# arielmission-space/PAOS

Measured on AMD Instinct MI355X. Metric: wavefronts/sec (4096^2 c128, 20-surface chain) + achieved HBM GB/s, higher is better.
Workload: dtype c128 (f64); 1 GPU; SYN20 20-surface chain (SURVEY 8d: 43 2-D FFTs per wavefront as the reference runs it), 4096x4096 fp64, walked 512-wavelength sweep, 32 wavefronts/GPU/step, PSFs stay in HBM; separable pass programs + ptp identities ([24] passes/wavefront, parity 1e-15..2e-14 vs oracle); grid=4096, batch_per_gpu=32, parallelism=wavefront-sharded x1, transport=none (single process), ranks_seen=1, launcher=none

## Files before the change

include/paos_hip.h:

```cpp
#ifndef PAOS_HIP_H
#define PAOS_HIP_H

#ifdef __cplusplus
extern "C" {
#endif

typedef struct paos_ctx paos_ctx;

enum { PAOS_OK = 0, PAOS_EINVAL = 1, PAOS_EHIP = 2, PAOS_EUNSUPPORTED = 3 };
enum { PAOS_F64 = 0, PAOS_F32 = 1 };
enum { PAOS_SHAPE_ELLIPSE = 0, PAOS_SHAPE_RECT = 1 };
enum { PAOS_KERNEL_PASS_ROWS = 0, PAOS_KERNEL_PASS_COLS = 1, PAOS_KERNEL_PASS_ANY = 2 };
enum { PAOS_PW_SIGN = 1, PAOS_PW_QPHASE_CENTRED = 2, PAOS_PW_QPHASE_NATURAL = 3, PAOS_PW_SCALE = 4,
       PAOS_PW_MASK = 5 };
enum { PAOS_PWF_MUL2PI = 1,
       PAOS_PWF_X_ONLY = 2, PAOS_PWF_Y_ONLY = 4 };
enum { PAOS_MAX_PW = 6 };
enum { PAOS_NORM_SLOTS = 64 };
enum { PAOS_WHAT_FIELD = 0, PAOS_WHAT_AMPLITUDE = 1, PAOS_WHAT_PHASE = 2, PAOS_WHAT_INTENSITY = 3 };

enum { PAOS_PHASE_STRIDE = 5 };
enum { PAOS_APERTURE_STRIDE = 8 };
enum { PAOS_ZERNIKE_HEAD = 8 };

// ... 16 lines not shown
int paos_ctx_create(int device, int n, int batch, int precision, paos_ctx** out);
int paos_ctx_destroy(paos_ctx* ctx);
const char* paos_last_error(const paos_ctx* ctx);
int paos_sync(paos_ctx* ctx);
const char* paos_build_info(void);
const char* paos_source_hash(void);
void* paos_stream(paos_ctx* ctx);

int paos_profile_begin(paos_ctx* ctx, int kernel_kind, int max_launches);
int paos_profile_end(paos_ctx* ctx, int* launches, double* total_ms);
int paos_profile_end_split(paos_ctx* ctx, int* launches, double* total_ms, int* pruned_launches, double* pruned_ms);
int paos_profile_end_launches(paos_ctx* ctx, int capacity, double* ms_out, int* tag_out, int* count);
int paos_profile_planned_bytes(paos_ctx* ctx, int capacity, double* bytes_out, int* count);
int paos_profile_line_transforms(paos_ctx* ctx, int capacity, double* lines_out, int* count);

int paos_fill(paos_ctx* ctx, double re, double im);
int paos_start(paos_ctx* ctx, double re, double im, int shape, const double* aperture, const double* stop);
int paos_start_rows(paos_ctx* ctx, double re, double im, int shape, const double* aperture, const double* stop,
                    const double* write_rows);
int paos_zero_outside_rows(paos_ctx* ctx, const double* live_rows);
int paos_start_box(paos_ctx* ctx, double re, double im, int shape, const double* aperture, const double* stop,
                   const double* write_rows, const double* write_cols);
int paos_start_zernike_box(paos_ctx* ctx, double re, double im, int shape, const double* aperture, const double* stop,
                           const double* write_rows, const double* write_cols, int nmax, int kdim, const double* table,
                           const double* params, int param_stride, int* power_ticket);
int paos_zero_outside_box(paos_ctx* ctx, const double* live_rows, const double* live_cols);
int paos_import(paos_ctx* ctx, int item, const void* host_c128);
int paos_export(paos_ctx* ctx, int item, int what, void* host_out);

int paos_psf_keep(paos_ctx* ctx);
int paos_psf_keep_power(paos_ctx* ctx, int* ticket);
int paos_psf_fetch(paos_ctx* ctx, int item, double* host_out);
int paos_host_alloc(unsigned long long bytes, void** out);
int paos_host_free(void* p);
int paos_export_pinned(paos_ctx* ctx, int item, int what, void* pinned_out);

int paos_aperture(paos_ctx* ctx, int shape, const double* params);
int paos_aperture_render(paos_ctx* ctx, int shape, const double* params1, double* host_mask);
int paos_make_stop(paos_ctx* ctx, const double* enable);
int paos_stop_scale_last_power(paos_ctx* ctx, const double* enable);
int paos_stop_defer_last_power(paos_ctx* ctx, const double* enable);
int paos_norm2(paos_ctx* ctx, double* host_out);
int paos_norm2_enqueue(paos_ctx* ctx, int* ticket);
int paos_norm2_enqueue_rows(paos_ctx* ctx, const double* live_rows, int* ticket);
int paos_norm2_enqueue_rows_like(paos_ctx* ctx, const double* live_rows, const double* same_as, int* ticket);
int paos_norm2_enqueue_box(paos_ctx* ctx, const double* live_rows, const double* live_cols, const double* same_as, int* ticket);
int paos_norm2_fetch(paos_ctx* ctx, int ticket, double* host_out);
int paos_norm2_release(paos_ctx* ctx, int ticket);
int paos_psf_metrics(paos_ctx* ctx, int nr, const double* radii_px, double cx_px, double cy_px,
                     double* host_out);
int paos_phase(paos_ctx* ctx, const double* params, int mul2pi);
int paos_phase_map(paos_ctx* ctx, int item, const double* host_wfe, double wl);
int paos_phase_map_items(paos_ctx* ctx, const double* host_wfe, unsigned long long key, int n_items, const double* items,
                         const double* wl);
int paos_psd_screen(paos_ctx* ctx, const double* host_noise, const double* host_rough, const double* params,
                    unsigned long long key, double* host_out);
int paos_ptp(paos_ctx* ctx, const double* params);
int paos_stw(paos_ctx* ctx, const double* params, int inverse);
int paos_wts(paos_ctx* ctx, const double* params, int inverse);
int paos_focus_begin(paos_ctx* ctx);
int paos_focus_plane(paos_ctx* ctx, const double* params);
int paos_focus_end(paos_ctx* ctx);
enum { PAOS_OTF_MTF = 0, PAOS_OTF_COMPLEX = 1 };
int paos_otf_compute(paos_ctx* ctx);
int paos_otf_fetch(paos_ctx* ctx, int item, int what, void* host_out);
int paos_otf_cuts(paos_ctx* ctx, double* host_out);
int paos_blur_table(int n, double d, double sigma, double pixel, double* t);
enum { PAOS_BLUR_ITEM = 6 };
int paos_blur_apply(paos_ctx* ctx, const double* per_item);
enum { PAOS_EE_GIVEN = 0, PAOS_EE_CENTROID = 1, PAOS_EE_PEAK = 2 };
enum { PAOS_EE_ITEM = 4 };
enum { PAOS_EE_SUMMARY = 9 };
int paos_ee_compute(paos_ctx* ctx, int bins, int square, int centre_mode, const double* per_item);
int paos_ee_fetch(paos_ctx* ctx, double* summary, double* curves);
int paos_zoom_weights(int n, int s, double frac, double* w, int* carry);
enum { PAOS_ZOOM_PSF = 0, PAOS_ZOOM_FIELD = 1 };
int paos_zoom_compute(paos_ctx* ctx, int m, int s, const double* centres, int want_field);
int paos_zoom_tiles(int n, int batch, int m, int* pt_y, int* pt_x);
int paos_zoom_fetch(paos_ctx* ctx, int item, int what, void* host_out);
int paos_run_passes(paos_ctx* ctx, const paos_pass* passes, int n_passes, const double* blocks,
                    int n_blocks);
int paos_copy_yardstick(paos_ctx* ctx, int reps, double* ms_per_launch, double* bytes_per_launch);
int paos_record_set_stats(paos_ctx* ctx, unsigned long long* found, unsigned long long* rendered);
int paos_central_half_stats(paos_ctx* ctx, unsigned long long* central, unsigned long long* plain);
int paos_narrow_window_stats(paos_ctx* ctx, unsigned long long* narrow, unsigned long long* other);
int paos_record_block_stats(paos_ctx* ctx, unsigned long long* out);
int paos_frugal_built(int precision, int n, const int* record);
int paos_pass_builds(paos_ctx* ctx, int* records, int capacity, int* count);
int paos_deferred_stop_stats(paos_ctx* ctx, unsigned long long* rode, unsigned long long* settled);
int paos_ctx_set_pruning(paos_ctx* ctx, int on);
int paos_run_passes_live(paos_ctx* ctx, const paos_pass* passes, int n_passes, const double* blocks,
                         int n_blocks, const double* live_rows);
int paos_run_program(paos_ctx* ctx, const paos_pass* passes, int n_passes, const double* blocks, int n_blocks,
                     const paos_program_opts* opts);
int paos_zernike(paos_ctx* ctx, int nmax, int kdim, const double* table, const double* params,
                 int param_stride, double* host_wfe);
int paos_zernike_like(paos_ctx* ctx, int nmax, int kdim, const double* table, const double* params,
                      int param_stride, const double* same_as, double* host_wfe);


int paos_pupil_aperture(paos_ctx* ctx, int shape, const double* params);
int paos_pupil_upload(paos_ctx* ctx, int item, const double* host_weights);
int paos_zernike_gram(paos_ctx* ctx, int nmax, int kdim, const double* table, const double* params,
                      int param_stride, int K, const double* poly, int use_pupil, double* host_out);
int paos_zernike_pupil(paos_ctx* ctx, int nmax, int kdim, const double* table, const double* params,
                       int param_stride, double* host_wfe);

enum { PAOS_WF_UNIFORM = 0, PAOS_WF_INTENSITY = 1 };
enum { PAOS_WF_SUMMARY = 10 };
int paos_wavefront_fit(paos_ctx* ctx, int nmax, int kdim, const double* table, const double* params, int param_stride,
                       int K, const double* poly, int weight_mode, int use_pupil, const double* min_intensity);
int paos_wavefront_fetch(paos_ctx* ctx, double* summary, double* sums);

enum { PAOS_DETECTOR_GEOM = 6 };
enum { PAOS_DETECTOR_ITEM = 3 };
enum { PAOS_DETECTOR_SCRATCH_MIB = 512 };
int paos_detector_begin(paos_ctx* ctx, const double* geom);
int paos_detector_add(paos_ctx* ctx, const double* per_item);
int paos_detector_images(paos_ctx* ctx, const double* per_item, double* host_out);
int paos_detector_fetch(paos_ctx* ctx, double* host_out);
enum { PAOS_DETECTOR_PLACED_ITEM = 5 };
int paos_detector_add_placed(paos_ctx* ctx, const double* per_item);
int paos_detector_images_placed(paos_ctx* ctx, const double* per_item, double* host_out);

#ifdef __cplusplus
}
#endif
#endif
```

paos_amd/_lib.py:

```python
import ctypes
import os
import threading
import weakref

import numpy as np

_HERE = os.path.dirname(os.path.abspath(__file__))
LIB_PATH = os.environ.get("PAOS_LIB") or os.path.join(_HERE, "libpaoship.so")

PAOS_F64, PAOS_F32 = 0, 1
SHAPE_ELLIPSE, SHAPE_RECT = 0, 1
WHAT_FIELD, WHAT_AMPLITUDE, WHAT_PHASE, WHAT_INTENSITY = 0, 1, 2, 3
KERNEL_PASS_ROWS, KERNEL_PASS_COLS, KERNEL_PASS_ANY = 0, 1, 2
PW_SIGN, PW_QPHASE_CENTRED, PW_QPHASE_NATURAL, PW_SCALE, PW_MASK = 1, 2, 3, 4, 5
PWF_MUL2PI = 1
PWF_X_ONLY, PWF_Y_ONLY = 2, 4
MAX_PW = 6
OTF_MTF, OTF_COMPLEX = 0, 1
EE_GIVEN, EE_CENTROID, EE_PEAK = 0, 1, 2
EE_ITEM, EE_SUMMARY, EE_MAX_BINS = 4, 9, 1024
WF_UNIFORM, WF_INTENSITY = 0, 1
WF_SUMMARY, WF_MAX_TERMS = 10, 63
ZOOM_PSF, ZOOM_FIELD = 0, 1
ZOOM_MAX_TABLES = 256
NORM_SLOTS = 64


class PwOp(ctypes.Structure):
    _fields_ = [("kind", ctypes.c_int), ("flags", ctypes.c_int), ("block", ctypes.c_int)]


class ProgramOpts(ctypes.Structure):
    _fields_ = [("live_rows", ctypes.POINTER(ctypes.c_double)), ("rows_stale", ctypes.c_int),
                ("final_intensity", ctypes.c_int), ("power_ticket", ctypes.POINTER(ctypes.c_int)),
                ("live_cols", ctypes.POINTER(ctypes.c_double))]


class Pass(ctypes.Structure):
    _fields_ = [("axis", ctypes.c_int), ("fft1", ctypes.c_int), ("fft2", ctypes.c_int),
                ("n_pre", ctypes.c_int), ("n_mid", ctypes.c_int), ("n_post", ctypes.c_int),
                ("pre", PwOp * MAX_PW), ("mid", PwOp * MAX_PW), ("post", PwOp * MAX_PW)]

PHASE_STRIDE = 5
APERTURE_STRIDE = 8
ZERNIKE_HEAD = 8

_c_ctx = ctypes.c_void_p
_dbl_p = ctypes.POINTER(ctypes.c_double)
SYMBOLS = {
    "paos_ctx_create": (ctypes.c_int, [ctypes.c_int, ctypes.c_int, ctypes.c_int, ctypes.c_int, ctypes.POINTER(_c_ctx)]),
    "paos_ctx_destroy": (ctypes.c_int, [_c_ctx]),
    "paos_last_error": (ctypes.c_char_p, [_c_ctx]),
    "paos_sync": (ctypes.c_int, [_c_ctx]),
    "paos_build_info": (ctypes.c_char_p, []),
    "paos_stream": (ctypes.c_void_p, [_c_ctx]),
    "paos_profile_begin": (ctypes.c_int, [_c_ctx, ctypes.c_int, ctypes.c_int]),
    "paos_profile_end": (ctypes.c_int, [_c_ctx, ctypes.POINTER(ctypes.c_int), _dbl_p]),
    "paos_profile_end_split": (ctypes.c_int, [_c_ctx, ctypes.POINTER(ctypes.c_int), _dbl_p, ctypes.POINTER(ctypes.c_int), _dbl_p]),
    "paos_source_hash": (ctypes.c_char_p, []),
    "paos_profile_planned_bytes": (ctypes.c_int, [_c_ctx, ctypes.c_int, _dbl_p, ctypes.POINTER(ctypes.c_int)]),
    "paos_profile_line_transforms": (ctypes.c_int, [_c_ctx, ctypes.c_int, _dbl_p, ctypes.POINTER(ctypes.c_int)]),
    "paos_profile_end_launches": (ctypes.c_int, [_c_ctx, ctypes.c_int, _dbl_p, ctypes.POINTER(ctypes.c_int),
                                                 ctypes.POINTER(ctypes.c_int)]),
    "paos_fill": (ctypes.c_int, [_c_ctx, ctypes.c_double, ctypes.c_double]),
    "paos_import": (ctypes.c_int, [_c_ctx, ctypes.c_int, ctypes.c_void_p]),
    "paos_export": (ctypes.c_int, [_c_ctx, ctypes.c_int, ctypes.c_int, ctypes.c_void_p]),
    "paos_aperture": (ctypes.c_int, [_c_ctx, ctypes.c_int, _dbl_p]),
    "paos_aperture_render": (ctypes.c_int, [_c_ctx, ctypes.c_int, _dbl_p, _dbl_p]),
    "paos_make_stop": (ctypes.c_int, [_c_ctx, _dbl_p]),
    "paos_stop_scale_last_power": (ctypes.c_int, [_c_ctx, _dbl_p]),
    "paos_stop_defer_last_power": (ctypes.c_int, [_c_ctx, _dbl_p]),
    "paos_norm2": (ctypes.c_int, [_c_ctx, _dbl_p]),
    "paos_norm2_enqueue": (ctypes.c_int, [_c_ctx, ctypes.POINTER(ctypes.c_int)]),
    "paos_norm2_fetch": (ctypes.c_int, [_c_ctx, ctypes.c_int, _dbl_p]),
    "paos_norm2_release": (ctypes.c_int, [_c_ctx, ctypes.c_int]),
    "paos_psf_metrics": (ctypes.c_int, [_c_ctx, ctypes.c_int, _dbl_p, ctypes.c_double, ctypes.c_double, _dbl_p]),
    "paos_phase": (ctypes.c_int, [_c_ctx, _dbl_p, ctypes.c_int]),
    "paos_phase_map": (ctypes.c_int, [_c_ctx, ctypes.c_int, _dbl_p, ctypes.c_double]),
    "paos_ptp": (ctypes.c_int, [_c_ctx, _dbl_p]),
    "paos_stw": (ctypes.c_int, [_c_ctx, _dbl_p, ctypes.c_int]),
    "paos_wts": (ctypes.c_int, [_c_ctx, _dbl_p, ctypes.c_int]),
    "paos_focus_begin": (ctypes.c_int, [_c_ctx]),
    "paos_focus_plane": (ctypes.c_int, [_c_ctx, _dbl_p]),
    "paos_focus_end": (ctypes.c_int, [_c_ctx]),
    "paos_otf_compute": (ctypes.c_int, [_c_ctx]),
    "paos_otf_fetch": (ctypes.c_int, [_c_ctx, ctypes.c_int, ctypes.c_int, ctypes.c_void_p]),
    "paos_otf_cuts": (ctypes.c_int, [_c_ctx, _dbl_p]),
    "paos_blur_table": (ctypes.c_int, [ctypes.c_int, ctypes.c_double, ctypes.c_double, ctypes.c_double, _dbl_p]),
    "paos_blur_apply": (ctypes.c_int, [_c_ctx, _dbl_p]),
    "paos_ee_compute": (ctypes.c_int, [_c_ctx, ctypes.c_int, ctypes.c_int, ctypes.c_int, _dbl_p]),
    "paos_ee_fetch": (ctypes.c_int, [_c_ctx, _dbl_p, _dbl_p]),
    "paos_wavefront_fit": (ctypes.c_int, [_c_ctx, ctypes.c_int, ctypes.c_int, _dbl_p, _dbl_p, ctypes.c_int, ctypes.c_int, _dbl_p,
                                          ctypes.c_int, ctypes.c_int, _dbl_p]),
    "paos_wavefront_fetch": (ctypes.c_int, [_c_ctx, _dbl_p, _dbl_p]),
    "paos_zoom_weights": (ctypes.c_int, [ctypes.c_int, ctypes.c_int, ctypes.c_double, _dbl_p, ctypes.POINTER(ctypes.c_int)]),
    "paos_zoom_compute": (ctypes.c_int, [_c_ctx, ctypes.c_int, ctypes.c_int, _dbl_p, ctypes.c_int]),
    "paos_zoom_fetch": (ctypes.c_int, [_c_ctx, ctypes.c_int, ctypes.c_int, ctypes.c_void_p]),
    "paos_zoom_tiles": (ctypes.c_int, [ctypes.c_int, ctypes.c_int, ctypes.c_int, ctypes.POINTER(ctypes.c_int),
                                       ctypes.POINTER(ctypes.c_int)]),
    "paos_run_passes": (ctypes.c_int, [_c_ctx, ctypes.POINTER(Pass), ctypes.c_int, _dbl_p, ctypes.c_int]),
    "paos_copy_yardstick": (ctypes.c_int, [_c_ctx, ctypes.c_int, _dbl_p, _dbl_p]),
    "paos_record_set_stats": (ctypes.c_int, [_c_ctx, ctypes.POINTER(ctypes.c_ulonglong), ctypes.POINTER(ctypes.c_ulonglong)]),
    "paos_central_half_stats": (ctypes.c_int, [_c_ctx, ctypes.POINTER(ctypes.c_ulonglong), ctypes.POINTER(ctypes.c_ulonglong)]),
    "paos_narrow_window_stats": (ctypes.c_int, [_c_ctx, ctypes.POINTER(ctypes.c_ulonglong), ctypes.POINTER(ctypes.c_ulonglong)]),
    "paos_record_block_stats": (ctypes.c_int, [_c_ctx, ctypes.POINTER(ctypes.c_ulonglong)]),
    "paos_frugal_built": (ctypes.c_int, [ctypes.c_int, ctypes.c_int, ctypes.POINTER(ctypes.c_int)]),
    "paos_pass_builds": (ctypes.c_int, [_c_ctx, ctypes.POINTER(ctypes.c_int), ctypes.c_int, ctypes.POINTER(ctypes.c_int)]),
    "paos_deferred_stop_stats": (ctypes.c_int, [_c_ctx, ctypes.POINTER(ctypes.c_ulonglong), ctypes.POINTER(ctypes.c_ulonglong)]),
    "paos_ctx_set_pruning": (ctypes.c_int, [_c_ctx, ctypes.c_int]),
    "paos_run_passes_live": (ctypes.c_int, [_c_ctx, ctypes.POINTER(Pass), ctypes.c_int, _dbl_p, ctypes.c_int, _dbl_p]),
    "paos_zernike": (ctypes.c_int, [_c_ctx, ctypes.c_int, ctypes.c_int, _dbl_p, _dbl_p, ctypes.c_int, _dbl_p]),
    "paos_psf_keep": (ctypes.c_int, [_c_ctx]),
    "paos_psf_keep_power": (ctypes.c_int, [_c_ctx, ctypes.POINTER(ctypes.c_int)]),
    "paos_psf_fetch": (ctypes.c_int, [_c_ctx, ctypes.c_int, _dbl_p]),
    "paos_host_alloc": (ctypes.c_int, [ctypes.c_ulonglong, ctypes.POINTER(ctypes.c_void_p)]),
    "paos_host_free": (ctypes.c_int, [ctypes.c_void_p]),
    "paos_export_pinned": (ctypes.c_int, [_c_ctx, ctypes.c_int, ctypes.c_int, ctypes.c_void_p]),
    "paos_start": (ctypes.c_int, [_c_ctx, ctypes.c_double, ctypes.c_double, ctypes.c_int, _dbl_p, _dbl_p]),
    "paos_pupil_aperture": (ctypes.c_int, [_c_ctx, ctypes.c_int, _dbl_p]),
    "paos_pupil_upload": (ctypes.c_int, [_c_ctx, ctypes.c_int, _dbl_p]),
    "paos_zernike_like": (ctypes.c_int, [_c_ctx, ctypes.c_int, ctypes.c_int, _dbl_p, _dbl_p, ctypes.c_int, _dbl_p, _dbl_p]),
    "paos_zernike_gram": (ctypes.c_int, [_c_ctx, ctypes.c_int, ctypes.c_int, _dbl_p, _dbl_p, ctypes.c_int,
                                         ctypes.c_int, _dbl_p, ctypes.c_int, _dbl_p]),
    "paos_zernike_pupil": (ctypes.c_int, [_c_ctx, ctypes.c_int, ctypes.c_int, _dbl_p, _dbl_p, ctypes.c_int, _dbl_p]),
    "paos_start_rows": (ctypes.c_int, [_c_ctx, ctypes.c_double, ctypes.c_double, ctypes.c_int, _dbl_p, _dbl_p, _dbl_p]),
    "paos_zero_outside_rows": (ctypes.c_int, [_c_ctx, _dbl_p]),
    "paos_phase_map_items": (ctypes.c_int, [_c_ctx, _dbl_p, ctypes.c_ulonglong, ctypes.c_int, _dbl_p, _dbl_p]),
    "paos_psd_screen": (ctypes.c_int, [_c_ctx, _dbl_p, _dbl_p, _dbl_p, ctypes.c_ulonglong, _dbl_p]),
    "paos_start_box": (ctypes.c_int, [_c_ctx, ctypes.c_double, ctypes.c_double, ctypes.c_int, _dbl_p, _dbl_p, _dbl_p, _dbl_p]),
    "paos_start_zernike_box": (ctypes.c_int, [_c_ctx, ctypes.c_double, ctypes.c_double, ctypes.c_int, _dbl_p, _dbl_p, _dbl_p, _dbl_p,
                                              ctypes.c_int, ctypes.c_int, _dbl_p, _dbl_p, ctypes.c_int, ctypes.POINTER(ctypes.c_int)]),
    "paos_zero_outside_box": (ctypes.c_int, [_c_ctx, _dbl_p, _dbl_p]),
    "paos_norm2_enqueue_box": (ctypes.c_int, [_c_ctx, _dbl_p, _dbl_p, _dbl_p, ctypes.POINTER(ctypes.c_int)]),
    "paos_norm2_enqueue_rows": (ctypes.c_int, [_c_ctx, _dbl_p, ctypes.POINTER(ctypes.c_int)]),
    "paos_norm2_enqueue_rows_like": (ctypes.c_int, [_c_ctx, _dbl_p, _dbl_p, ctypes.POINTER(ctypes.c_int)]),
    "paos_run_program": (ctypes.c_int, [_c_ctx, ctypes.POINTER(Pass), ctypes.c_int, _dbl_p, ctypes.c_int,
                                        ctypes.POINTER(ProgramOpts)]),
    "paos_detector_begin": (ctypes.c_int, [_c_ctx, _dbl_p]),
    "paos_detector_add": (ctypes.c_int, [_c_ctx, _dbl_p]),
    "paos_detector_images": (ctypes.c_int, [_c_ctx, _dbl_p, _dbl_p]),
    "paos_detector_fetch": (ctypes.c_int, [_c_ctx, _dbl_p]),
    "paos_detector_add_placed": (ctypes.c_int, [_c_ctx, _dbl_p]),
    "paos_detector_images_placed": (ctypes.c_int, [_c_ctx, _dbl_p, _dbl_p]),
}

_lib = None


class PaosHipError(RuntimeError):
    pass


def load():
    global _lib
    if _lib is not None:
        return _lib
    if not os.path.exists(LIB_PATH):
        raise PaosHipError(
            f"{LIB_PATH} not found: build it with `make` or "
            "`python -c 'import __graft_entry__ as g; g.build()'` (there is no CPU fallback)"
        )
    lib = ctypes.CDLL(LIB_PATH)
    if os.environ.get("PAOS_LIB"):
        import sys

        print(f"paos_amd: using the library variant {LIB_PATH} (PAOS_LIB)", file=sys.stderr)
    for name, (res, args) in SYMBOLS.items():
        fn = getattr(lib, name)
        fn.restype = res
        fn.argtypes = args
    _lib = lib
    return lib


def _dptr(arr):
    return arr.ctypes.data_as(_dbl_p)


def as_blocks(blocks, batch, stride):
    arr = np.ascontiguousarray(blocks, dtype=np.float64)
    if arr.shape != (batch, stride):
        raise ValueError(f"expected parameter blocks of shape {(batch, stride)}, got {arr.shape}")
    return arr


BUILD_FIELDS = ("axis", "kpre", "kmid", "nfft", "store", "tab", "fuse", "one_line", "central")


def frugal_built(precision, n, record):
    if len(record) != len(BUILD_FIELDS):
        raise ValueError("a build record has nine fields")
    rec = (ctypes.c_int * 9)(*[int(v) for v in record])
    code = {"fp64": PAOS_F64, "fp32": PAOS_F32}.get(precision, -1)
    rc = load().paos_frugal_built(code, int(n), rec)
    if rc < 0:
        raise ValueError(f"no family of pass-kernel builds for {precision} at n = {n}")
    return bool(rc)


def zoom_check(size, oversample, n):
    if isinstance(size, bool) or not isinstance(size, (int, np.integer)) or size < 16 or size > 1024 or size % 16:
        raise ValueError(f"a zoomed window's size must be an integer multiple of 16 in 16 .. 1024, got {size!r}")
    if isinstance(oversample, bool) or not isinstance(oversample, (int, np.integer)) or not 1 <= oversample <= 64:
        raise ValueError(f"a zoomed window's oversampling must be an integer in 1 .. 64, got {oversample!r}")
    if size > oversample * n:
        raise ValueError(f"a zoomed window of {size} samples at oversampling {oversample} is wider than the {n}-pixel grid")


def zoom_tiles(n, batch, size):
    pty, ptx = ctypes.c_int(0), ctypes.c_int(0)
    if load().paos_zoom_tiles(int(n), int(batch), int(size), ctypes.byref(pty), ctypes.byref(ptx)) != 0:
        raise ValueError(f"paos_zoom_tiles refused n={n!r}, batch={batch!r}, size={size!r}")
    return pty.value, ptx.value


def blur_table(n, d, sigma, pixel=0.0):
    if isinstance(n, bool) or not isinstance(n, (int, np.integer)) or n < 2:
        raise ValueError(f"paos_blur_table refused n={n!r}")
    out = np.empty(int(n) // 2 + 1, dtype=np.float64)
    if load().paos_blur_table(int(n), float(d), float(sigma), float(pixel), _dptr(out)) != 0:
# ... 425 lines not shown
    def energy_compute(self, bins, deltas, aspects, centre_mode, centres=None, square=False):
        per_item = np.empty((self.batch, EE_ITEM), dtype=np.float64)
        try:
            per_item[:, 0] = np.broadcast_to(np.asarray(deltas, dtype=np.float64), (self.batch,))
            per_item[:, 1] = np.broadcast_to(np.asarray(aspects, dtype=np.float64), (self.batch,))
            per_item[:, 2:] = self.n / 2 if centres is None else np.asarray(centres, dtype=np.float64)
        except ValueError:
            raise ValueError(f"energy_compute takes scalars or one value per item ({self.batch}) and (batch, 2) centres") from None
        self._check(self._lib.paos_ee_compute(self._ctx, int(bins), int(bool(square)), int(centre_mode), _dptr(per_item)),
                    "paos_ee_compute")
        self._ee_shape = (self.batch, 2 if square else 1, int(bins))

    def energy_fetch(self, curves=True):
        shape = getattr(self, "_ee_shape", None)
        if shape is None:
            raise PaosHipError("paos_ee_fetch failed (1): no energy profiles computed (paos_ee_compute)")
        summary = np.empty((self.batch, EE_SUMMARY), dtype=np.float64)
        out = np.empty(shape, dtype=np.float64) if curves else None
        self._check(self._lib.paos_ee_fetch(self._ctx, _dptr(summary), _dptr(out) if curves else None), "paos_ee_fetch")
        return summary, out

    def wavefront_fit(self, nmax, kdim, table, blocks, poly, weight=WF_UNIFORM, min_intensity=None, pupil=False):
        t = np.ascontiguousarray(table, dtype=np.float64).reshape(-1)
        b = np.ascontiguousarray(blocks, dtype=np.float64)
        q = np.ascontiguousarray(poly, dtype=np.float64)
        if b.ndim != 2 or b.shape[0] != self.batch:
            raise ValueError("zernike blocks must be [batch][stride]")
        if q.ndim != 2 or q.shape[1] != 4:
            raise ValueError("poly must be [K][4]")
        floors = None
        if min_intensity is not None:
            try:
                floors = np.ascontiguousarray(np.broadcast_to(np.asarray(min_intensity, dtype=np.float64), (self.batch,)))
            except ValueError:
                raise ValueError(f"wavefront_fit takes a scalar floor or one per item ({self.batch})") from None
        self._check(self._lib.paos_wavefront_fit(self._ctx, int(nmax), int(kdim), _dptr(t), _dptr(b), int(b.shape[1]), int(q.shape[0]),
                                                 _dptr(q), int(weight), 1 if pupil else 0,
                                                 _dptr(floors) if floors is not None else None), "paos_wavefront_fit")
        self._wf_terms = int(q.shape[0])

    def wavefront_fetch(self):
        k = getattr(self, "_wf_terms", None)
        if k is None:
            raise PaosHipError("paos_wavefront_fetch failed (1): no wavefront fit computed (paos_wavefront_fit)")
        summary = np.empty((self.batch, WF_SUMMARY), dtype=np.float64)
        sums = np.empty((self.batch, (k + 1) * (k + 2) // 2), dtype=np.float64)
        self._check(self._lib.paos_wavefront_fetch(self._ctx, _dptr(summary), _dptr(sums)), "paos_wavefront_fetch")
        return summary, sums

    def zoom_compute(self, size, oversample, centres=None, field=False):
        ctr = None if centres is None else zoom_centres(centres, self.batch, self.n)
        zoom_check(size, oversample, self.n)
        self._check(self._lib.paos_zoom_compute(self._ctx, int(size), int(oversample), _dptr(ctr) if ctr is not None else None,
                                                1 if field else 0), "paos_zoom_compute")
        self._zoom_size = int(size)

    def zoom_fetch(self, item=0, what="psf"):
        if what not in ("psf", "field"):
            raise ValueError(f"what must be 'psf' or 'field', got {what!r}")
        m = getattr(self, "_zoom_size", 1)
        out = np.empty((m, m), dtype=np.float64 if what == "psf" else np.complex128)
        self._check(self._lib.paos_zoom_fetch(self._ctx, int(item), ZOOM_PSF if what == "psf" else ZOOM_FIELD,
                                              out.ctypes.data_as(ctypes.c_void_p)), "paos_zoom_fetch")
        return out

    def copy_yardstick(self, reps=10):
        ms, nbytes = ctypes.c_double(0.0), ctypes.c_double(0.0)
        self._check(self._lib.paos_copy_yardstick(self._ctx, int(reps), ctypes.byref(ms), ctypes.byref(nbytes)),
                    "paos_copy_yardstick")
        return ms.value, nbytes.value

    def record_set_stats(self):
        found, rendered = ctypes.c_ulonglong(0), ctypes.c_ulonglong(0)
        self._check(self._lib.paos_record_set_stats(self._ctx, ctypes.byref(found), ctypes.byref(rendered)),
                    "paos_record_set_stats")
        return int(found.value), int(rendered.value)

    def central_half_stats(self):
        central, plain = ctypes.c_ulonglong(0), ctypes.c_ulonglong(0)
        self._check(self._lib.paos_central_half_stats(self._ctx, ctypes.byref(central), ctypes.byref(plain)),
                    "paos_central_half_stats")
        return int(central.value), int(plain.value)

    def record_block_stats(self):
        out = (ctypes.c_ulonglong * 3)()
        self._check(self._lib.paos_record_block_stats(self._ctx, out), "paos_record_block_stats")
        return int(out[0]), int(out[1]), int(out[2])

    def pass_builds(self, capacity=64):
        count = ctypes.c_int(0)
        buf = (ctypes.c_int * (9 * capacity))()
        self._check(self._lib.paos_pass_builds(self._ctx, buf, capacity, ctypes.byref(count)), "paos_pass_builds")
        if count.value > capacity:
            return self.pass_builds(count.value)
        return [tuple(buf[9 * i:9 * i + 9]) for i in range(count.value)]

    def deferred_stop_stats(self):
        rode, settled = ctypes.c_ulonglong(0), ctypes.c_ulonglong(0)
        self._check(self._lib.paos_deferred_stop_stats(self._ctx, ctypes.byref(rode), ctypes.byref(settled)),
                    "paos_deferred_stop_stats")
        return int(rode.value), int(settled.value)

    def set_pruning(self, on):
        self._check(self._lib.paos_ctx_set_pruning(self._ctx, 1 if on else 0), "paos_ctx_set_pruning")

    def run_passes(self, passes, blocks, live_rows=None, rows_stale=False, final_intensity=False, live_cols=None):
        b = np.ascontiguousarray(blocks, dtype=np.float64)
        if b.ndim != 3 or b.shape[1:] != (self.batch, PHASE_STRIDE):
            raise ValueError("blocks must be [n_blocks][batch][5]")
        arr = (Pass * len(passes))()
        for dst, src in zip(arr, passes):
            dst.axis, dst.fft1, dst.fft2 = src["axis"], src.get("fft1", -1), src.get("fft2", -1)
            for name in ("pre", "mid", "post"):
                ops = src.get(name, ())
                if len(ops) > MAX_PW:
                    raise ValueError("too many operators in one pass slot")
                setattr(dst, "n_" + name, len(ops))
                lst = getattr(dst, name)
                for i, (kind, flags, block) in enumerate(ops):
                    lst[i].kind, lst[i].flags, lst[i].block = kind, flags, block
        if rows_stale or final_intensity:
            lr = self._rows(live_rows) if live_rows is not None else None
            lc = self._rows(live_cols) if (live_cols is not None and rows_stale and lr is not None) else None
            ticket = ctypes.c_int(-1)
            opts = ProgramOpts(_dptr(lr) if lr is not None else None, 1 if (rows_stale and lr is not None) else 0,
                               int(final_intensity), ctypes.pointer(ticket), _dptr(lc) if lc is not None else None)
            self._check(self._lib.paos_run_program(self._ctx, arr, len(passes), _dptr(b), b.shape[0], ctypes.byref(opts)),
                        "paos_run_program")
            return ticket.value if final_intensity else None
        if live_rows is not None:
            lr = self._rows(live_rows)
            self._check(self._lib.paos_run_passes_live(self._ctx, arr, len(passes), _dptr(b), b.shape[0], _dptr(lr)),
                        "paos_run_passes_live")
            return None
        self._check(self._lib.paos_run_passes(self._ctx, arr, len(passes), _dptr(b), b.shape[0]),
                    "paos_run_passes")
        return None

    def zernike(self, nmax, kdim, table, blocks, want_wfe=False, pupil=False, same_as=None):
        t = np.ascontiguousarray(table, dtype=np.float64).reshape(-1)
        b = np.ascontiguousarray(blocks, dtype=np.float64)
        if b.ndim != 2 or b.shape[0] != self.batch:
            raise ValueError("zernike blocks must be [batch][stride]")
        out = np.empty((self.n, self.n), dtype=np.float64) if want_wfe else None
        if same_as is not None and not pupil:
            like = np.ascontiguousarray(same_as, dtype=np.float64).reshape(-1)
            if like.size != self.batch:
                raise ValueError("same_as must name an item per item")
            self._check(self._lib.paos_zernike_like(self._ctx, int(nmax), int(kdim), _dptr(t), _dptr(b), int(b.shape[1]),
                                                    _dptr(like), _dptr(out) if want_wfe else None), "paos_zernike_like")
            return out
        fn = self._lib.paos_zernike_pupil if pupil else self._lib.paos_zernike
        self._check(fn(self._ctx, int(nmax), int(kdim), _dptr(t), _dptr(b), int(b.shape[1]),
                       _dptr(out) if want_wfe else None),
                    "paos_zernike_pupil" if pupil else "paos_zernike")
        return out

    def start(self, value, shape, blocks, stop=None, write_rows=None, write_cols=None):
        b = np.ascontiguousarray(blocks, dtype=np.float64)
        if b.shape != (self.batch, APERTURE_STRIDE):
            raise ValueError("aperture blocks must be [batch][8]")
        st = None if stop is None else np.ascontiguousarray(stop, dtype=np.float64)
        if st is not None and st.shape != (self.batch,):
            raise ValueError("stop flags must be [batch]")
        v = complex(value)
        if write_rows is not None and write_cols is not None:
            self._check(self._lib.paos_start_box(self._ctx, v.real, v.imag, int(shape), _dptr(b),
                                                 _dptr(st) if st is not None else None, _dptr(self._rows(write_rows)),
                                                 _dptr(self._rows(write_cols))), "paos_start_box")
            return
        if write_rows is not None:
            self._check(self._lib.paos_start_rows(self._ctx, v.real, v.imag, int(shape), _dptr(b),
                                                  _dptr(st) if st is not None else None, _dptr(self._rows(write_rows))),
                        "paos_start_rows")
            return
        self._check(self._lib.paos_start(self._ctx, v.real, v.imag, int(shape), _dptr(b),
                                         _dptr(st) if st is not None else None), "paos_start")

    def start_zernike(self, value, shape, blocks, stop, write_rows, write_cols, nmax, kdim, table, zblocks, power=False):
        b = np.ascontiguousarray(blocks, dtype=np.float64)
        if b.shape != (self.batch, APERTURE_STRIDE):
            raise ValueError("aperture blocks must be [batch][8]")
        st = None if stop is None else np.ascontiguousarray(stop, dtype=np.float64)
        if st is not None and st.shape != (self.batch,):
            raise ValueError("stop flags must be [batch]")
        t = np.ascontiguousarray(table, dtype=np.float64).reshape(-1)
        zb = np.ascontiguousarray(zblocks, dtype=np.float64)
        if zb.ndim != 2 or zb.shape[0] != self.batch:
            raise ValueError("zernike blocks must be [batch][stride]")
        v = complex(value)
        ticket = ctypes.c_int(-1)
        self._check(self._lib.paos_start_zernike_box(self._ctx, v.real, v.imag, int(shape), _dptr(b),
                                                     _dptr(st) if st is not None else None, _dptr(self._rows(write_rows)),
                                                     _dptr(self._rows(write_cols)), int(nmax), int(kdim), _dptr(t), _dptr(zb),
                                                     int(zb.shape[1]), ctypes.byref(ticket) if power else None),
                    "paos_start_zernike_box")
        return ticket.value if power else None

    def pupil_aperture(self, shape, blocks):
        b = np.ascontiguousarray(blocks, dtype=np.float64)
        if b.shape != (self.batch, APERTURE_STRIDE):
            raise ValueError("aperture blocks must be [batch][8]")
        self._check(self._lib.paos_pupil_aperture(self._ctx, int(shape), _dptr(b)), "paos_pupil_aperture")

    def pupil_upload(self, item, weights):
        w = np.ascontiguousarray(weights, dtype=np.float64)
        if w.shape != (self.n, self.n):
            raise ValueError("pupil weights must be [n][n]")
        self._check(self._lib.paos_pupil_upload(self._ctx, int(item), _dptr(w)), "paos_pupil_upload")

    def zernike_gram(self, nmax, kdim, table, blocks, poly, pupil=True):
        t = np.ascontiguousarray(table, dtype=np.float64).reshape(-1)
        b = np.ascontiguousarray(blocks, dtype=np.float64)
        q = np.ascontiguousarray(poly, dtype=np.float64)
        if b.ndim != 2 or b.shape[0] != self.batch:
            raise ValueError("zernike blocks must be [batch][stride]")
        if q.ndim != 2 or q.shape[1] != 4:
            raise ValueError("poly must be [K][4]")
        k = q.shape[0]
        out = np.empty((self.batch, k * (k + 1) // 2 + 1), dtype=np.float64)
        self._check(self._lib.paos_zernike_gram(self._ctx, int(nmax), int(kdim), _dptr(t), _dptr(b),
                                                int(b.shape[1]), int(k), _dptr(q), 1 if pupil else 0, _dptr(out)),
                    "paos_zernike_gram")
        return out[:, :-1], out[:, -1]
```

paos_amd/csrc/arena_layout.h:

```cpp
#pragma once
#include <cstddef>

#pragma GCC visibility push(hidden)

constexpr size_t kArenaAlign = 16;
inline size_t arena_rounded(size_t count) { return (count + kArenaAlign - 1) & ~(kArenaAlign - 1); }
constexpr size_t kArenaSlack = 64;

enum ArenaRoom {
  ARENA_FITS,
  ARENA_SWITCH,
  ARENA_GROW
};

struct ArenaLayout {
  size_t cap = 0;
  size_t head = 0;
  size_t sent = 0;

  ArenaRoom room(size_t total) const {
    total += kArenaSlack;
    if (total > cap) return ARENA_GROW;
    return head + total > cap ? ARENA_SWITCH : ARENA_FITS;
  }
  size_t grown(size_t total) const {
    size_t c = cap ? cap : kArenaAlign;
    while (c < total + kArenaSlack) c *= 2;
    return c;
  }
  bool fits(size_t count) const { return count <= cap && head + count <= cap; }
  size_t place(size_t count) {
    const size_t at = head;
    head += arena_rounded(count);
    return at;
  }
  bool pending() const { return sent < head; }
  bool take(size_t* first, size_t* count) {
    if (!pending()) return false;
    *first = sent;
    *count = head - sent;
    sent = head;
    return true;
  }
  void drop() { sent = head; }
  void rewind() { head = sent = 0; }
};

struct ArenaBatchState {
  bool reserved = false, closed = false;
  bool may_add() const { return !closed; }
  bool may_switch() const { return !reserved; }
};

#pragma GCC visibility pop
```

paos_amd/csrc/context.hip:

```cpp
#include "host.h"

#include <cmath>
#include <complex>
#include <cstdio>
#include <cstring>
#include <mutex>
#include <set>
#include <utility>

namespace {

thread_local std::string g_err;

}

int fail(paos_ctx* c, int code, const std::string& msg) {
  if (c) c->err = msg;
  g_err = msg;
  return code;
}

namespace {

bool dump_arena() {
// ... 198 lines not shown
  return out;
}

namespace {

template <typename T>
std::vector<std::complex<T>> twiddles(int n) {
  std::vector<std::complex<T>> tw(n);
  const long double two_pi = 6.283185307179586476925286766559005768L;
  for (int m = 0; m < n; ++m) {
    const long double a = two_pi * (long double)m / (long double)n;
    tw[m] = std::complex<T>((T)cosl(a), (T)-sinl(a));
  }
  return tw;
}


int profile_end(paos_ctx* c, int* launches, double* total_ms, int* pruned_launches, double* pruned_ms) {
  if (c) (void)hipSetDevice(c->device);
  if (!c || !launches || !total_ms) return fail(c, PAOS_EINVAL, "null argument");
  HIPCHK(c, hipStreamSynchronize(c->stream));
  double sum = 0.0, psum = 0.0;
  int pcount = 0;
  for (size_t i = 0; i + 1 < c->prof_used; i += 2) {
    float ms = 0.f;
    HIPCHK(c, hipEventElapsedTime(&ms, c->prof_events[i], c->prof_events[i + 1]));
    sum += ms;
    if (i / 2 < c->prof_tags.size() && c->prof_tags[i / 2]) { psum += ms; ++pcount; }
  }
  *launches = (int)(c->prof_used / 2);
  *total_ms = sum;
  if (pruned_launches) *pruned_launches = pcount;
  if (pruned_ms) *pruned_ms = psum;
  c->prof_kind = -1;
  c->prof_used = 0;
  return PAOS_OK;
}

}

extern "C" {

const char* paos_last_error(const paos_ctx* ctx) { return ctx ? ctx->err.c_str() : g_err.c_str(); }

const char* paos_build_info(void) {
  static const std::string info = std::string("libpaoship gfx950 layout=") + std::to_string(BR) + "(c64 at N>=2048: " + std::to_string(PAOS_F32_BR) + ")x(" +
                                  std::to_string(Lay<double>::BC) + "|" + std::to_string(Lay<float>::BC) +
                                  ") pad_blocks=" + std::to_string(PAOS_PAD_BLOCKS);
  return info.c_str();
}

void* paos_stream(paos_ctx* ctx) { return ctx ? (void*)ctx->stream : nullptr; }

int paos_ctx_create(int device, int n, int batch, int precision, paos_ctx** out) {
  if (!out) return fail(nullptr, PAOS_EINVAL, "out is null");
  *out = nullptr;
  if (n < 64 || n > 4096 || (n & (n - 1))) return fail(nullptr, PAOS_EUNSUPPORTED, "grid size must be a power of two in 64..4096");
  if (batch < 1) return fail(nullptr, PAOS_EINVAL, "batch must be >= 1");
  if (precision != PAOS_F64 && precision != PAOS_F32) return fail(nullptr, PAOS_EINVAL, "precision must be PAOS_F64 or PAOS_F32");
  int ndev = 0;
  if (hipGetDeviceCount(&ndev) != hipSuccess || ndev == 0)
    return fail(nullptr, PAOS_EHIP, "no HIP device available: libpaoship has no CPU fallback");
  if (device < 0 || device >= ndev) return fail(nullptr, PAOS_EINVAL, "device index out of range");
  paos_ctx* c = new paos_ctx();
  c->device = device; c->n = n; c->batch = batch; c->precision = precision;
  const int bc = precision == PAOS_F64 ? Lay<double>::BC : Lay<float>::BC;
  c->br = (precision == PAOS_F32 && n >= 2048) ? PAOS_F32_BR : PAOS_BR;
  c->pitch = (unsigned)n * c->br + (unsigned)PAOS_PAD_BLOCKS * c->br * bc;
  c->item_stride = c->pitch * (unsigned)(n / c->br);
  const size_t eb = elem_bytes(c);
  auto bail = [&](hipError_t e, const char* what) {
    std::string msg = std::string(what) + ": " + hipGetErrorString(e);
    paos_ctx_destroy(c);
    return fail(nullptr, PAOS_EHIP, msg);
  };
  hipError_t e;
  if ((e = hipSetDevice(device)) != hipSuccess) return bail(e, "hipSetDevice");
  if ((e = hipStreamCreateWithFlags(&c->stream, hipStreamNonBlocking)) != hipSuccess) return bail(e, "hipStreamCreate");
  if (const char* pad = getenv("PAOS_LDS_PAD")) c->lds_pad = (size_t)std::max(0, std::atoi(pad));
  if (env_is("PAOS_CENTRAL_HALF", '0')) c->central_half = false;
  if (env_is("PAOS_CENTRAL_HALF", '1')) c->central_half = true;
  if (env_is("PAOS_NARROW_WINDOWS", '0')) c->narrow_windows = false;
  if (env_is("PAOS_NARROW_WINDOWS", '1')) c->narrow_windows = true;
  if ((e = hipMalloc(&c->dyn_scale, (size_t)batch * sizeof(double))) != hipSuccess) return bail(e, "hipMalloc(dyn_scale)");
  {
    std::vector<double> ones((size_t)batch, 1.0);
    if ((e = hipMemcpy(c->dyn_scale, ones.data(), ones.size() * sizeof(double), hipMemcpyHostToDevice)) != hipSuccess) return bail(e, "hipMemcpy(dyn_scale)");
  }
  if ((e = hipMalloc(&c->field, (size_t)c->item_stride * batch * eb)) != hipSuccess) return bail(e, "hipMalloc(field)");
  if ((e = hipMemsetAsync(c->field, 0, (size_t)c->item_stride * batch * eb, c->stream)) != hipSuccess) return bail(e, "hipMemset(field)");
  if ((e = hipMalloc(&c->tw, (size_t)n * eb)) != hipSuccess) return bail(e, "hipMalloc(tw)");
  if ((e = hipMalloc(&c->staging, (size_t)n * n * 16)) != hipSuccess) return bail(e, "hipMalloc(staging)");
  c->nparts = 1024;
  if ((e = hipMalloc(&c->partial, (size_t)batch * c->nparts * sizeof(double))) != hipSuccess) return bail(e, "hipMalloc(partial)");
  if ((e = hipMalloc(&c->norm2, (size_t)batch * sizeof(double))) != hipSuccess) return bail(e, "hipMalloc(norm2)");
  if ((e = hipHostMalloc(&c->norm2_host, (size_t)kNormSlots * batch * sizeof(double))) != hipSuccess) return bail(e, "hipHostMalloc(norm2)");
  c->arena.lay.cap = (size_t)1 << 18;
  if (c->arena.lay.cap < (size_t)batch * 2048) c->arena.lay.cap = (size_t)batch * 2048;
  if (const char* cap = getenv("PAOS_ARENA_DOUBLES")) c->arena.lay.cap = arena_rounded((size_t)std::max(1LL, std::atoll(cap)));
  if ((e = hipHostMalloc(&c->arena.host, kArenaSlabs * c->arena.lay.cap * sizeof(double))) != hipSuccess) return bail(e, "hipHostMalloc(arena)");
  if ((e = hipMalloc(&c->arena.dev, kArenaSlabs * c->arena.lay.cap * sizeof(double))) != hipSuccess) return bail(e, "hipMalloc(arena)");
  for (int k = 0; k < kArenaSlabs; ++k)
    if ((e = hipEventCreateWithFlags(&c->arena.fence[k], hipEventDisableTiming)) != hipSuccess) return bail(e, "hipEventCreate(arena fence)");
  c->arena.used[0] = true;
  e = dispatch_layout(c, [&](auto t, auto) {
    auto tw = twiddles<decltype(t)>(n);
    return hipMemcpy(c->tw, tw.data(), (size_t)n * eb, hipMemcpyHostToDevice);
  });
  if (e != hipSuccess) return bail(e, "hipMemcpy(tw)");
  *out = c;
  return PAOS_OK;
}

int paos_profile_begin(paos_ctx* c, int kernel_kind, int max_launches) {
  if (c) (void)hipSetDevice(c->device);
  if (!c || max_launches < 0) return fail(c, PAOS_EINVAL, "bad profile request");
  HIPCHK(c, hipStreamSynchronize(c->stream));
  while (c->prof_events.size() < (size_t)2 * max_launches) {
    hipEvent_t e;
    HIPCHK(c, hipEventCreate(&e));
    c->prof_events.push_back(e);
  }
  c->prof_kind = kernel_kind;
  c->prof_used = 0;
  c->prof_tags.clear();
  c->prof_bytes.clear();
  c->prof_lines.clear();
  return PAOS_OK;
}

int paos_profile_end_launches(paos_ctx* c, int capacity, double* ms_out, int* tag_out, int* count) {
  if (c) (void)hipSetDevice(c->device);
  if (!c || !ms_out || !tag_out || !count || capacity < 0) return fail(c, PAOS_EINVAL, "null argument");
  HIPCHK(c, hipStreamSynchronize(c->stream));
  const int n = (int)(c->prof_used / 2);
  if (n > capacity) return fail(c, PAOS_EINVAL, "more launches were timed than the caller's arrays hold");
  for (int i = 0; i < n; ++i) {
    float ms = 0.f;
    HIPCHK(c, hipEventElapsedTime(&ms, c->prof_events[2 * i], c->prof_events[2 * i + 1]));
    ms_out[i] = ms;
    tag_out[i] = (size_t)i < c->prof_tags.size() ? c->prof_tags[i] : 0;
  }
  *count = n;
  c->prof_kind = -1;
  c->prof_used = 0;
  return PAOS_OK;
}

int paos_profile_planned_bytes(paos_ctx* c, int capacity, double* bytes_out, int* count) {
  if (!c || !bytes_out || !count || capacity < 0) return fail(c, PAOS_EINVAL, "null argument");
  const int n = (int)(c->prof_used / 2);
  if (n > capacity) return fail(c, PAOS_EINVAL, "more launches were timed than the caller's array holds");
  for (int i = 0; i < n; ++i) bytes_out[i] = (size_t)i < c->prof_bytes.size() ? c->prof_bytes[i] : 0.0;
  *count = n;
  return PAOS_OK;
}

int paos_profile_line_transforms(paos_ctx* c, int capacity, double* lines_out, int* count) {
  if (!c || !lines_out || !count || capacity < 0) return fail(c, PAOS_EINVAL, "bad profile request");
  const int n = (int)(c->prof_used / 2);
  if (n > capacity) return fail(c, PAOS_EINVAL, "profile buffer too small");
  for (int i = 0; i < n; ++i) lines_out[i] = (size_t)i < c->prof_lines.size() ? c->prof_lines[i] : 0.0;
  *count = n;
  return PAOS_OK;
}

int paos_profile_end(paos_ctx* c, int* launches, double* total_ms) {
  return profile_end(c, launches, total_ms, nullptr, nullptr);
}

int paos_profile_end_split(paos_ctx* c, int* launches, double* total_ms, int* pruned_launches, double* pruned_ms) {
  if (!pruned_launches || !pruned_ms) return fail(c, PAOS_EINVAL, "null argument");
  return profile_end(c, launches, total_ms, pruned_launches, pruned_ms);
}

int paos_ctx_destroy(paos_ctx* c) {
  if (!c) return PAOS_OK;
  (void)hipSetDevice(c->device);
  if (c->stream) (void)hipStreamSynchronize(c->stream);
  for (hipEvent_t e : c->prof_events) (void)hipEventDestroy(e);
  if (c->field) (void)hipFree(c->field);
  if (c->tw) (void)hipFree(c->tw);
  if (c->staging) (void)hipFree(c->staging);
  if (c->tables) (void)hipFree(c->tables);
  if (c->mask) (void)hipFree(c->mask);
  if (c->metric_partial) (void)hipFree(c->metric_partial);
  if (c->metric_out) (void)hipFree(c->metric_out);
  if (c->metric_host) (void)hipHostFree(c->metric_host);
  for (auto& ms : c->mask_sets) {
    if (ms.lines) (void)hipFree(ms.lines);
    if (ms.vals) (void)hipFree(ms.vals);
  }
  if (c->mask_overflow) (void)hipFree(c->mask_overflow);
  if (c->block_stats) (void)hipFree(c->block_stats);
  if (c->partial) (void)hipFree(c->partial);
  if (c->norm2) (void)hipFree(c->norm2);
  if (c->norm2_host) (void)hipHostFree(c->norm2_host);
  if (c->psf) (void)hipFree(c->psf);
  if (c->focus_spec) (void)hipFree(c->focus_spec);
  if (c->otf_spec) (void)hipFree(c->otf_spec);
  if (c->otf_cuts) (void)hipFree(c->otf_cuts);
  if (c->zoom_t) (void)hipFree(c->zoom_t);
  if (c->zoom_psf) (void)hipFree(c->zoom_psf);
  if (c->zoom_field) (void)hipFree(c->zoom_field);
  if (c->zoom_tabs) (void)hipFree(c->zoom_tabs);
  if (c->map_dev) (void)hipFree(c->map_dev);
  if (c->psd_scratch) (void)hipFree(c->psd_scratch);
  if (c->start_norm2) (void)hipFree(c->start_norm2);
  if (c->start_partial) (void)hipFree(c->start_partial);
  if (c->psd_bad) (void)hipFree(c->psd_bad);
  if (c->pow_partial) (void)hipFree(c->pow_partial);
  if (c->dyn_scale) (void)hipFree(c->dyn_scale);
  if (c->ptab) (void)hipFree(c->ptab);
  if (c->psf_partial) (void)hipFree(c->psf_partial);
  if (c->det_img) (void)hipFree(c->det_img);
  if (c->det_rows) (void)hipFree(c->det_rows);
  if (c->det_out) (void)hipFree(c->det_out);
  if (c->ee_buf) (void)hipFree(c->ee_buf);
  if (c->wf_buf) (void)hipFree(c->wf_buf);
  for (int i = 0; i < 2; ++i) {
    if (c->bounce[i]) (void)hipHostFree(c->bounce[i]);
    if (c->bounce_ev[i]) (void)hipEventDestroy(c->bounce_ev[i]);
  }
  if (c->arena.host) (void)hipHostFree(c->arena.host);
  if (c->arena.dev) (void)hipFree(c->arena.dev);
  for (int k = 0; k < kArenaSlabs; ++k)
    if (c->arena.fence[k]) (void)hipEventDestroy(c->arena.fence[k]);
  if (c->stream) (void)hipStreamDestroy(c->stream);
  delete c;
  return PAOS_OK;
}

int paos_sync(paos_ctx* c) {
  if (c) (void)hipSetDevice(c->device);
  if (!c) return fail(c, PAOS_EINVAL, "null context");
  HIPCHK(c, hipStreamSynchronize(c->stream));
  return check_mask_overflow(c);
}

int paos_host_alloc(unsigned long long bytes, void** out) {
  if (!out || bytes == 0) return fail(nullptr, PAOS_EINVAL, "null argument");
  *out = nullptr;
  const hipError_t e = hipHostMalloc(out, (size_t)bytes);
  if (e != hipSuccess) {
    *out = nullptr;
    return fail(nullptr, PAOS_EHIP, std::string("hipHostMalloc: ") + hipGetErrorString(e));
  }
  return PAOS_OK;
}

int paos_host_free(void* p) {
  if (!p) return PAOS_OK;
  const hipError_t e = hipHostFree(p);
  if (e != hipSuccess) return fail(nullptr, PAOS_EHIP, std::string("hipHostFree: ") + hipGetErrorString(e));
  return PAOS_OK;
}

int paos_norm2_fetch(paos_ctx* c, int ticket, double* host_out) {
  if (c) (void)hipSetDevice(c->device);
  if (!c || !host_out || ticket < 0 || ticket >= kNormSlots) return fail(c, PAOS_EINVAL, "bad ticket");
  if (!c->norm_busy[ticket]) return fail(c, PAOS_EINVAL, "ticket is not outstanding (already fetched, or never issued)");
  HIPCHK(c, hipStreamSynchronize(c->stream));
  c->norm_busy[ticket] = false;
  std::memcpy(host_out, c->norm2_host + (size_t)ticket * c->batch, (size_t)c->batch * sizeof(double));
  return check_mask_overflow(c);
}

int paos_norm2_release(paos_ctx* c, int ticket) {
  if (!c || ticket < 0 || ticket >= kNormSlots) return fail(c, PAOS_EINVAL, "bad ticket");
  c->norm_busy[ticket] = false;
  return PAOS_OK;
}

int paos_record_set_stats(paos_ctx* c, unsigned long long* found, unsigned long long* rendered) {
  if (!c || !found || !rendered) return fail(c, PAOS_EINVAL, "bad record-set request");
  *found = c->mask_hits;
  *rendered = c->mask_rendered;
  return PAOS_OK;
}

int paos_central_half_stats(paos_ctx* c, unsigned long long* central, unsigned long long* plain) {
  if (!c || !central || !plain) return fail(c, PAOS_EINVAL, "bad central-half request");
  *central = c->central_launches;
  *plain = c->plain_launches;
  return PAOS_OK;
}

int paos_narrow_window_stats(paos_ctx* c, unsigned long long* narrow, unsigned long long* other) {
  if (!c || !narrow || !other) return fail(c, PAOS_EINVAL, "bad narrow-window request");
  *narrow = c->narrow_launches;
  *other = c->other_launches;
  return PAOS_OK;
}

int paos_record_block_stats(paos_ctx* c, unsigned long long* out) {
  if (!c || !out) return fail(c, PAOS_EINVAL, "bad record-block request");
  out[0] = out[1] = out[2] = 0ull;
  if (!c->block_stats) return PAOS_OK;
  HIPCHK(c, hipStreamSynchronize(c->stream));
  HIPCHK(c, hipMemcpy(out, c->block_stats, 3 * sizeof(unsigned long long), hipMemcpyDeviceToHost));
  return PAOS_OK;
}

int paos_deferred_stop_stats(paos_ctx* c, unsigned long long* rode, unsigned long long* settled) {
  if (!c || !rode || !settled) return fail(c, PAOS_EINVAL, "bad deferred-stop request");
  *rode = c->deferred_rode;
  *settled = c->deferred_settled;
  return PAOS_OK;
}

int paos_ctx_set_pruning(paos_ctx* c, int on) {
  if (!c) return fail(c, PAOS_EINVAL, "null context");
  c->prune = on != 0;
  return PAOS_OK;
}

}
```

paos_amd/csrc/host.h:

```cpp
#pragma once
#include "../../include/paos_hip.h"

#include <hip/hip_runtime.h>

#include <cstdlib>
#include <string>
#include <type_traits>
#include <vector>

#include "arena_layout.h"
#include "frugal_pass.h"
#include "pass_records.h"

using namespace paos;

#ifndef PAOS_BR
#define PAOS_BR 4
#endif
#ifndef PAOS_PAD_BLOCKS
#define PAOS_PAD_BLOCKS 3
#endif
inline constexpr int BR = PAOS_BR;
#ifndef PAOS_F32_BR
#define PAOS_F32_BR 8
#endif
template <typename T, int N>
constexpr int block_rows() { return (sizeof(T) == 4 && N >= 2048) ? PAOS_F32_BR : PAOS_BR; }
inline constexpr int kNormSlots = PAOS_NORM_SLOTS;
template <typename T>
struct Lay {
  static constexpr int BC = 2;
};

constexpr int kArenaSlabs = 4;
struct Arena {
  double* host = nullptr;
  double* dev = nullptr;
  ArenaLayout lay;
  int cur = 0;
  int left = -1;
  hipEvent_t fence[kArenaSlabs] = {};
  bool fenced[kArenaSlabs] = {};
  bool used[kArenaSlabs] = {};
};

struct paos_ctx {
  int device = 0, n = 0, batch = 0, precision = 0;
  int br = PAOS_BR;
  unsigned pitch = 0, item_stride = 0;
  hipStream_t stream = nullptr;
  double* psf = nullptr;
  void* focus_spec = nullptr;
  bool focus_open = false;
  void* otf_spec = nullptr;
  bool otf_computed = false, otf_valid = false;
  double* otf_cuts = nullptr;
  std::vector<double> blur_tabs, blur_key;
  cx<double>* zoom_t = nullptr;
  double* zoom_psf = nullptr;
  cx<double>* zoom_field = nullptr;
  int zoom_m = 0;
  bool zoom_done = false, zoom_has_field = false;
  double* zoom_tabs = nullptr;
  int zoom_s = 0, zoom_cap = 0;
  std::vector<double> zoom_fracs;
  std::vector<std::vector<int>> zoom_carry;
  double* map_dev = nullptr;
  unsigned long long map_key = 0;
  double map_max = 0.0;
  std::vector<double> start_key;
  double* start_norm2 = nullptr;
  std::vector<double> start_partial_key;
  double* start_partial = nullptr;
  cx<double>* psd_scratch = nullptr;
  int* psd_bad = nullptr;
  double* psf_partial = nullptr;
  int psf_nparts = 0;
  double* pow_partial = nullptr;
  int pow_nparts = 0;
  cx<double>* ptab = nullptr;
  int ptab_slots = 0;
  double* dyn_scale = nullptr;
  bool dyn_pending = false;
  unsigned long long deferred_rode = 0, deferred_settled = 0;
  bool norm2_of_field = false;
  int psf_zero_axis = -1;
  std::vector<double> psf_zero_lo, psf_zero_hi;
  bool det_set = false;
  int det_nx = 0, det_ny = 0;
  double det_geom[4] = {};
  double* det_img = nullptr;
  double* det_rows = nullptr;
  size_t det_rows_bytes = 0;
  double* det_out = nullptr;
  size_t det_out_bytes = 0;
  double* ee_buf = nullptr;
  size_t ee_bytes = 0;
  int ee_bins = 0, ee_curves = 0;
  bool ee_computed = false, ee_valid = false;
  double* wf_buf = nullptr;
  size_t wf_bytes = 0;
  int wf_pairs = 0;
  bool wf_fitted = false;
  void* bounce[2] = {nullptr, nullptr};
  hipEvent_t bounce_ev[2] = {nullptr, nullptr};
  void* field = nullptr;
  void* tw = nullptr;
  void* staging = nullptr;
  cx<double>* tables = nullptr;
  double* mask = nullptr;
  double* metric_partial = nullptr;
  double* metric_out = nullptr;
  double* metric_host = nullptr;
  struct MaskSet {
    MaskLine* lines = nullptr;
    double* vals = nullptr;
    std::vector<double> key;
    unsigned long long used = 0;
    int line_lo = 0, line_hi = 0;
  };
  static constexpr int kMaskSets = 8;
  MaskSet mask_sets[kMaskSets];
  unsigned long long mask_clock = 0;
  unsigned long long mask_hits = 0, mask_rendered = 0;
  size_t lds_pad = 0;
  bool central_half = true;
  unsigned long long central_launches = 0, plain_launches = 0;
  bool narrow_windows = true;
  unsigned long long narrow_launches = 0, other_launches = 0;
  std::vector<int> pass_builds;
  int* mask_overflow = nullptr;
  unsigned long long* block_stats = nullptr;
  double* partial = nullptr;
// ... 46 lines not shown
  static constexpr int COL_LINES = BC;
  static constexpr int ROW_THREADS = ROW_LINES * N / E, COL_THREADS = COL_LINES * N / E;
  static constexpr int ROW_TILES = (ROW_THREADS >= 128) ? 1 : 128 / ROW_THREADS;
  static constexpr int COL_TILES = (COL_THREADS >= 128) ? 1 : 128 / COL_THREADS;
  static constexpr bool ROW_SPLIT = (size_t)ROW_LINES * ROW_TILES * line_lds_bytes<T, N, false>() > 144 * 1024;
  static constexpr bool COL_SPLIT = (size_t)COL_LINES * COL_TILES * line_lds_bytes<T, N, false>() > 144 * 1024;
  static constexpr int MINW = 1;
};
inline int frugal_tile_lines(const paos_ctx* c, int axis) { return axis == 0 ? (c->n >= 2048 ? c->br / 2 : c->br) : 2; }

int arena_reserve(paos_ctx* c, size_t total);
int arena_push(paos_ctx* c, const double* src, size_t count, const double** dev);
class ArenaBatch {
 public:
  explicit ArenaBatch(paos_ctx* c) : c_(c) {}
  int begin(size_t total);
  int add(const double* src, size_t count, const double** dev);
  int commit();

 private:
  paos_ctx* c_;
  ArenaBatchState st_;
};
int arena_settled(paos_ctx* c, int rc);
int copy_to_host(paos_ctx* c, void* host, const void* dev, size_t bytes);
int next_norm_slot(paos_ctx* c);
int check_mask_overflow(paos_ctx* c);
int check_rows(paos_ctx* c, const double* rows);
std::vector<double> rounded_cols(const paos_ctx* c, const double* cols);
int opt_in_lds(paos_ctx* c, const void* kern, size_t lds);
bool timed_launch_begin(paos_ctx* c, int kind);
hipError_t timed_launch_end(paos_ctx* c, int tag);

int launch_failed(paos_ctx* c, const char* call, hipError_t e, const char* file, int line);
#define TIMED_LAUNCH(c, ...) timed_launch(__FILE__, __LINE__, (c), __VA_ARGS__)
template <typename Kern, typename... Args>
int timed_launch(const char* file, int line, paos_ctx* c, Kern kern, dim3 grid, dim3 block, size_t lds, size_t lds_opt_in, int kind,
                 int tag, Args... args) {
  if (lds_opt_in) {
    int rc = opt_in_lds(c, (const void*)kern, lds_opt_in);
    if (rc) return rc;
  }
  const bool timed = timed_launch_begin(c, kind);
  hipLaunchKernelGGL(kern, grid, block, lds, c->stream, args...);
  hipError_t e = hipGetLastError();
  if (e != hipSuccess) return launch_failed(c, "hipGetLastError()", e, file, line);
  if (timed && (e = timed_launch_end(c, tag)) != hipSuccess) return launch_failed(c, "timed_launch_end(c, tag)", e, file, line);
  return PAOS_OK;
}
inline size_t generic_lds_opt_in(size_t lds) { return lds > 48 * 1024 ? lds : 0; }

template <typename F>
int dispatch_n(paos_ctx* c, F&& f) {
  switch (c->n) {
#define PAOS_N_CASE(N) case N: return f(std::integral_constant<int, N>{})
    PAOS_N_CASE(64);
    PAOS_N_CASE(128);
    PAOS_N_CASE(256);
    PAOS_N_CASE(512);
    PAOS_N_CASE(1024);
    PAOS_N_CASE(2048);
    PAOS_N_CASE(4096);
#undef PAOS_N_CASE
  }
  return fail(c, PAOS_EUNSUPPORTED, "grid size must be a power of two in 64..4096");
}

template <typename F>
auto dispatch_block_rows(const paos_ctx* c, F&& f) {
  if (c->br == PAOS_F32_BR) return f(std::integral_constant<int, PAOS_F32_BR>{});
  return f(std::integral_constant<int, PAOS_BR>{});
}
template <typename F>
auto dispatch_layout(const paos_ctx* c, F&& f) {
  if (c->precision == PAOS_F64) return f(double{}, std::integral_constant<int, PAOS_BR>{});
  return dispatch_block_rows(c, [&](auto br) { return f(float{}, br); });
}
template <int A, int B, typename F>
auto dispatch_either(bool first, F&& f) {
  if (first) return f(std::integral_constant<int, A>{});
  return f(std::integral_constant<int, B>{});
}

int run_passes(paos_ctx* c, const paos_pass* passes, int n_passes, const double* blocks, int n_blocks,
               const double* entry_rows = nullptr, bool entry_stale = false, int* final_ticket = nullptr, int final_mode = 1,
               const double* entry_cols = nullptr);
int mask_render_mode();
bool mask_rect_blocks();

int generic_pass(paos_ctx* c, int axis, const PassArgs& a, int feat);

template <typename T, int N>
int frugal_family(paos_ctx* c, const FrugalBuild& b, const FrugalArgs& a, bool narrow);

int settle_scale(paos_ctx* c, bool field_is_overwritten = false);
int dyn_scale_reset(paos_ctx* c);
int zero_outside_rows(paos_ctx* c, const double* live_rows);
int zero_outside_box(paos_ctx* c, const double* live_rows, const double* live_cols);
int power_ring_full(paos_ctx* c);
int take_power_ticket(paos_ctx* c, const double* partial, int nparts, const double* source, int* ticket);
int psf_keep_power_impl(paos_ctx* c, int* ticket);
struct MaskRender {
  const double *params, *shared;
  int set, axis, line0, line_end, shapes;
};
constexpr int kMaskRenders = 8;
int render_mask_records(paos_ctx* c, const MaskRender* jobs, int count);
int render_mask_weights(paos_ctx* c, const double* ap);
int pointwise_pass(paos_ctx* c, const PassArgs& a);

#define SETTLE_SCALE(c) do { if (c) { (c)->norm2_of_field = false; if ((c)->dyn_pending) { int rc_ = settle_scale(c); if (rc_) return rc_; } } } while (0)
#define DROP_SCALE(c) do { if (c) { (c)->norm2_of_field = false; if ((c)->dyn_pending) { int rc_ = settle_scale(c, true); if (rc_) return rc_; } } } while (0)

#pragma GCC visibility pop
```

paos_amd/csrc/paos_hip.hip:

```cpp
#include "host.h"

#include <algorithm>
#include <cmath>
#include <cstring>

#include "item_groups.h"
#include "pointwise.h"

namespace {

int pw_blocks(const paos_ctx* c) {
  const size_t total = (size_t)c->item_stride;
  size_t b = (total + kPwThreads - 1) / kPwThreads;
  return (int)(b < 2048 ? b : 2048);
}

__global__ void dyn_scale_set_kernel(double* dyn, const double* norm2, const double* enable, int batch) {
  const int i = blockIdx.x * blockDim.x + threadIdx.x;
  if (i < batch) dyn[i] = (!enable || enable[i] != 0.0) ? 1.0 / sqrt(norm2[i]) : 1.0;
}
__global__ void dyn_scale_reset_kernel(double* dyn, int batch) {
  const int i = blockIdx.x * blockDim.x + threadIdx.x;
  if (i < batch) dyn[i] = 1.0;
}
// ... 31 lines not shown

static_assert(kMaskRenders == kMaskJobs, "a call's renderings go out in one launch per shape");
int render_mask_records(paos_ctx* c, const MaskRender* renders, int count) {
  MaskJobs jobs{};
  for (int j = 0; j < count; ++j) {
    const MaskRender& r = renders[j];
    const paos_ctx::MaskSet& ms = c->mask_sets[r.set];
    jobs.job[j] = MaskJob{r.params, r.shared, ms.lines, ms.vals, r.axis, r.line0, r.line_end, r.shapes};
  }
  jobs.batch_stride = c->batch * (int)FP_STRIDE; jobs.param_stride = (int)FP_STRIDE; jobs.n = c->n; jobs.overflow = c->mask_overflow;
  const int mode = mask_render_mode();
  jobs.windows = mode != 0 ? 1 : 0;
  jobs.pairs = mode >= 2 ? std::min(mode, 3) - 1 : 0;
  jobs.rect_blocks = mask_rect_blocks() ? 1 : 0;
  int widest = 0, shapes = 0;
  for (int j = 0; j < count; ++j) {
    widest = std::max(widest, jobs.job[j].line_end - jobs.job[j].line0);
    shapes |= jobs.job[j].shapes;
  }
  const dim3 block(256);
  const int per_wg = 4 * (jobs.pairs >= 2 ? 4 : (jobs.pairs ? 2 : 1));
  constexpr int block_per_wg = kMaskBlockLines * kMaskWaves;
  if ((shapes & 1) && mode == 4)
    hipLaunchKernelGGL(mask_blocks_kernel, dim3((widest + block_per_wg - 1) / block_per_wg, c->batch, count), block, 0, c->stream, jobs, c->block_stats);
  else if (shapes & 1)
    hipLaunchKernelGGL(mask_lines_kernel<0>, dim3((widest + per_wg - 1) / per_wg, c->batch, count), block, 0, c->stream, jobs);
  const int rect_per_wg = 4 * (jobs.rect_blocks ? 64 : 1);
  if (shapes & 2) hipLaunchKernelGGL(mask_lines_kernel<1>, dim3((widest + rect_per_wg - 1) / rect_per_wg, c->batch, count), block, 0, c->stream, jobs);
  HIPCHK(c, hipGetLastError());
  return PAOS_OK;
}

int render_mask_weights(paos_ctx* c, const double* ap) {
  if (!c->mask) HIPCHK(c, hipMalloc(&c->mask, (size_t)c->batch * c->item_stride * sizeof(double)));
  const dim3 grid(pw_blocks(c), c->batch), block(kPwThreads);
  const double* ap2 = ap + (size_t)c->batch * FP_STRIDE;
  dispatch_layout(c, [&](auto t, auto br) {
    using T = decltype(t);
    constexpr int BRV = decltype(br)::value;
    hipLaunchKernelGGL((aperture_kernel<T, BRV, Lay<T>::BC, 0>), grid, block, 0, c->stream, (cx<T>*)nullptr, ap, ap2, FP_STRIDE, c->n, c->pitch, c->item_stride, c->mask, 1);
    hipLaunchKernelGGL((aperture_kernel<T, BRV, Lay<T>::BC, 1>), grid, block, 0, c->stream, (cx<T>*)nullptr, ap, ap2, FP_STRIDE, c->n, c->pitch, c->item_stride, c->mask, 1);
  });
  HIPCHK(c, hipGetLastError());
  return PAOS_OK;
}

int pointwise_pass(paos_ctx* c, const PassArgs& a) {
  const dim3 grid(pw_blocks(c), c->batch), block(kPwThreads);
  dispatch_layout(c, [&](auto t, auto br) {
    hipLaunchKernelGGL((pointwise_kernel<decltype(t), decltype(br)::value, Lay<decltype(t)>::BC>), grid, block, 0, c->stream, a, c->n);
  });
  HIPCHK(c, hipGetLastError());
  return PAOS_OK;
}

namespace {

const char* const kPhaseMapOverflow = "the phase argument 2 pi w / wl of the map's largest value is not finite";
bool phase_map_argument_finite(double wmax, double wl) { return std::isfinite((6.283185307179586 * wmax) / wl); }

bool share_wfe_maps() {
  static const bool on = !env_is("PAOS_SHARE_WFE", '0');
  return on;
}

void norm2_partial_launch(paos_ctx* c, const double* enable, const double* rows = nullptr, const double* cols = nullptr) {
  dispatch_layout(c, [&](auto t, auto br) {
    using T = decltype(t);
    hipLaunchKernelGGL((norm2_partial_kernel<T, decltype(br)::value, Lay<T>::BC>), dim3(c->nparts, c->batch), dim3(kPwThreads), 0, c->stream,
                       (const cx<T>*)c->field, c->partial, c->n, c->pitch, c->item_stride, enable, 1, rows, cols);
  });
}

void stop_scale_launch(paos_ctx* c, const double* enable) {
  dispatch_layout(c, [&](auto t, auto) {
    using T = decltype(t);
    hipLaunchKernelGGL(stop_scale_kernel<T>, dim3(pw_blocks(c), c->batch), dim3(kPwThreads), 0, c->stream, (cx<T>*)c->field, c->norm2,
                       c->item_stride, enable, 1);
  });
}

}

int power_ring_full(paos_ctx* c) {
  if (c->norm_busy[next_norm_slot(c)])
    return fail(c, PAOS_EINVAL, "64 power reductions outstanding: fetch earlier tickets (paos_norm2_fetch) first");
  return PAOS_OK;
}

int take_power_ticket(paos_ctx* c, const double* partial, int nparts, const double* source, int* ticket) {
  if (int rc = power_ring_full(c)) return rc;
  const int slot = next_norm_slot(c);
  hipLaunchKernelGGL(norm2_final_kernel, dim3(c->batch), dim3(kPwThreads), 0, c->stream, partial, c->norm2, nparts, (const double*)nullptr, 1, source);
  HIPCHK(c, hipGetLastError());
  c->norm_busy[slot] = true;
  c->norm_slot = (slot + 1) % kNormSlots;
  HIPCHK(c, hipMemcpyAsync(c->norm2_host + (size_t)slot * c->batch, c->norm2, (size_t)c->batch * sizeof(double),
                           hipMemcpyDeviceToHost, c->stream));
  *ticket = slot;
  return PAOS_OK;
}

extern "C" {

int paos_fill(paos_ctx* c, double re, double im) {
  DROP_SCALE(c);
  if (c) (void)hipSetDevice(c->device);
  if (!c) return fail(c, PAOS_EINVAL, "null context");
  const size_t total = (size_t)c->item_stride * c->batch;
  dispatch_layout(c, [&](auto t, auto) {
    using T = decltype(t);
    hipLaunchKernelGGL(fill_kernel<T>, dim3(2048), dim3(kPwThreads), 0, c->stream, (cx<T>*)c->field, total, (T)re, (T)im);
  });
  HIPCHK(c, hipGetLastError());
  return PAOS_OK;
}

struct StartZernike {
  int nmax, kdim, param_stride;
  const double *table, *params;
  int* power_ticket;
};
static int zernike_check(paos_ctx* c, int nmax, int kdim, const double* table, const double* params, int param_stride);

static bool start_memo_on() {
  static const bool memo = !env_is("PAOS_START_POWER_MEMO", '0');
  return memo;
}
static bool same_key(const std::vector<double>& a, const std::vector<double>& b) {
  return a.size() == b.size() && !std::memcmp(a.data(), b.data(), a.size() * sizeof(double));
}
static void start_forget(paos_ctx* c) {
  c->start_key.clear();
  c->start_partial_key.clear();
}

static int start_body(paos_ctx* c, double re, double im, int shape, const double* aperture, const double* stop,
                      const double* write_rows, const double* write_cols, const StartZernike* zk) {
  if (c) (void)hipSetDevice(c->device);
  if (!c || !aperture) return fail(c, PAOS_EINVAL, "null argument");
  if (shape != PAOS_SHAPE_ELLIPSE && shape != PAOS_SHAPE_RECT) return fail(c, PAOS_EINVAL, "unknown aperture shape");
  int rc;
  if (zk) {
    if ((rc = zernike_check(c, zk->nmax, zk->kdim, zk->table, zk->params, zk->param_stride))) return rc;
    if (zk->power_ticket && (rc = power_ring_full(c))) return rc;
  }
  const int batch = c->batch;
  std::vector<double> flags(batch, 0.0);
  bool any_stop = false;
  if (stop)
    for (int i = 0; i < batch; ++i) { flags[i] = stop[i] != 0.0 ? 1.0 : 0.0; any_stop |= flags[i] != 0.0; }
  std::vector<double> power_of, compute;
  power_representatives(batch, aperture, AP_STRIDE, flags.data(), power_of, compute);
  if (write_rows && (rc = check_rows(c, write_rows))) return rc;
  std::vector<double> wc;
  if (write_cols) {
    if (!write_rows) return fail(c, PAOS_EINVAL, "a column window needs a row window");
    if ((rc = check_rows(c, write_cols))) return rc;
    wc = rounded_cols(c, write_cols);
  }
  static const bool share_start = !env_is("PAOS_SHARE_START", '0');
  ItemGroups groups = group_items(
      batch,
      [&](int j, int i) {
        return share_start && flags[j] == flags[i] && same_record(aperture + (size_t)j * AP_STRIDE, aperture + (size_t)i * AP_STRIDE, AP_STRIDE) &&
               (!write_rows || same_record(write_rows + 2 * j, write_rows + 2 * i, 2)) &&
               (!write_cols || same_record(write_cols + 2 * j, write_cols + 2 * i, 2));
      },
      [](int) { return true; });
  std::vector<double> lead, same, subs;
  const bool want_power = zk && zk->power_ticket;
  if (zk) {
    group_leaders(groups, lead, same);
    subs = split_by_map(groups, zk->params, zk->param_stride, ZP_ENABLE, ZP_INV_WL, share_wfe_maps());
  }
  const size_t zt_count = zk ? (size_t)(zk->nmax + 1) * zk->kdim * 3 : 0, zp_count = zk ? (size_t)batch * zk->param_stride : 0;
  size_t total = arena_rounded((size_t)batch * AP_STRIDE) + 3 * arena_rounded(batch) + arena_rounded(groups.goff.size()) +
                 arena_rounded(groups.glen.size()) + arena_rounded(groups.members.size());
  if (write_rows) total += arena_rounded((size_t)2 * batch);
  if (write_cols) total += arena_rounded(wc.size());
  if (zk) total += arena_rounded(zt_count) + arena_rounded(zp_count) + arena_rounded(subs.size());
  if (want_power) total += 2 * arena_rounded(batch);
  ArenaBatch ab(c);
  if ((rc = ab.begin(total))) return rc;
  const double *dp = nullptr, *ds = nullptr, *dcompute = nullptr, *dpower_of = nullptr, *drows = nullptr, *dcols = nullptr;
  if ((rc = ab.add(aperture, (size_t)batch * AP_STRIDE, &dp))) return rc;
  if ((rc = ab.add(flags.data(), flags.size(), &ds))) return rc;
  if ((rc = ab.add(compute.data(), compute.size(), &dcompute))) return rc;
  if ((rc = ab.add(power_of.data(), power_of.size(), &dpower_of))) return rc;
  if (write_rows && (rc = ab.add(write_rows, (size_t)2 * batch, &drows))) return rc;
  if (write_cols && (rc = ab.add(wc.data(), wc.size(), &dcols))) return rc;
  const double *dzt = nullptr, *dzp = nullptr, *dsubs = nullptr, *dlead = nullptr, *dsame = nullptr;
  if (zk) {
    if ((rc = ab.add(zk->table, zt_count, &dzt))) return rc;
    if ((rc = ab.add(zk->params, zp_count, &dzp))) return rc;
    if ((rc = ab.add(subs.data(), subs.size(), &dsubs))) return rc;
    if (want_power) {
      if ((rc = ab.add(lead.data(), lead.size(), &dlead))) return rc;
      if ((rc = ab.add(same.data(), same.size(), &dsame))) return rc;
    }
  }
  const double *dgoff = nullptr, *dglen = nullptr, *dmembers = nullptr;
  if ((rc = ab.add(groups.goff.data(), groups.goff.size(), &dgoff))) return rc;
  if ((rc = ab.add(groups.glen.data(), groups.glen.size(), &dglen))) return rc;
  if ((rc = ab.add(groups.members.data(), groups.members.size(), &dmembers))) return rc;
  if ((rc = ab.commit())) return rc;
  const bool memo = start_memo_on();
  std::vector<double> key, pkey;
  if (memo && (any_stop || want_power)) {
    key.reserve(3 + (size_t)batch * (AP_STRIDE + 1));
    key.push_back((double)shape); key.push_back(re); key.push_back(im);
    key.insert(key.end(), aperture, aperture + (size_t)batch * AP_STRIDE);
    key.insert(key.end(), flags.begin(), flags.end());
  }
  bool power_found = false;
  if (any_stop) {
    power_found = memo && c->start_norm2 && same_key(key, c->start_key);
    if (power_found) HIPCHK(c, hipMemcpyAsync(c->norm2, c->start_norm2, (size_t)batch * sizeof(double), hipMemcpyDeviceToDevice, c->stream));
    else c->start_key.clear();
  }
  bool partial_found = false;
  double* partial = c->partial;
  if (want_power && memo) {
    pkey = key;
    pkey.insert(pkey.end(), write_rows, write_rows + (size_t)2 * batch);
    pkey.insert(pkey.end(), wc.begin(), wc.end());
    pkey.insert(pkey.end(), lead.begin(), lead.end());
    pkey.insert(pkey.end(), same.begin(), same.end());
    partial_found = c->start_partial && same_key(pkey, c->start_partial_key);
    if (!partial_found) c->start_partial_key.clear();
    if (!c->start_partial) HIPCHK(c, hipMalloc(&c->start_partial, (size_t)batch * c->nparts * sizeof(double)));
    partial = c->start_partial;
  }
  const dim3 block(kPwThreads), sweep(pw_blocks(c), batch), parts(c->nparts, batch);
  dispatch_layout(c, [&](auto t, auto br) {
    using T = decltype(t);
    constexpr int BRV = decltype(br)::value, BC = Lay<T>::BC;
    dispatch_either<0, 1>(shape == PAOS_SHAPE_ELLIPSE, [&](auto s) {
      constexpr int S = decltype(s)::value;
      if (any_stop && !power_found) {
        hipLaunchKernelGGL((start_power_kernel<T, BRV, BC, S>), parts, block, 0, c->stream, dp, c->n, c->pitch, c->item_stride, re, im,
                           c->partial, dcompute);
        hipLaunchKernelGGL(norm2_final_kernel, dim3(batch), block, 0, c->stream, c->partial, c->norm2, c->nparts, ds, 1, dpower_of);
      }
      if (!zk) {
        hipLaunchKernelGGL((start_write_kernel<T, BRV, BC, S>), sweep, block, 0, c->stream, (cx<T>*)c->field, dp, c->n, c->pitch,
                           c->item_stride, re, im, (const double*)c->norm2, ds, drows, dgoff, dglen, dmembers, dcols);
        return;
      }
      dispatch_either<8, 0>(zk->nmax <= 8, [&](auto nc) {
        hipLaunchKernelGGL((zernike_start_write_kernel<T, BRV, BC, S, decltype(nc)::value>), sweep, block, 0, c->stream, (cx<T>*)c->field,
                           dp, c->n, c->pitch, c->item_stride, re, im, (const double*)c->norm2, ds, drows, dcols, dgoff, dglen, dsubs,
                           dmembers, dzt, dzp, zk->param_stride, zk->nmax, zk->kdim);
      });
      if (want_power && !partial_found)
        hipLaunchKernelGGL((start_norm2_partial_kernel<T, BRV, BC, S>), parts, block, 0, c->stream, partial, dp, c->n, c->pitch,
                           c->item_stride, re, im, (const double*)c->norm2, ds, dlead, drows, dcols);
    });
  });
  HIPCHK(c, hipGetLastError());
  if (any_stop && !power_found && memo) {
    if (!c->start_norm2) HIPCHK(c, hipMalloc(&c->start_norm2, (size_t)batch * sizeof(double)));
    HIPCHK(c, hipMemcpyAsync(c->start_norm2, c->norm2, (size_t)batch * sizeof(double), hipMemcpyDeviceToDevice, c->stream));
    c->start_key = std::move(key);
  }
  if (want_power && !partial_found && memo) c->start_partial_key = std::move(pkey);
  if (want_power) return take_power_ticket(c, partial, c->nparts, dsame, zk->power_ticket);
  return PAOS_OK;
}

static int start_impl(paos_ctx* c, double re, double im, int shape, const double* aperture, const double* stop,
                      const double* write_rows, const double* write_cols = nullptr, const StartZernike* zk = nullptr) {
  const int rc = arena_settled(c, start_body(c, re, im, shape, aperture, stop, write_rows, write_cols, zk));
  if (rc != PAOS_OK && c) start_forget(c);
  return rc;
}

int paos_start(paos_ctx* c, double re, double im, int shape, const double* aperture, const double* stop) {
  return paos_start_box(c, re, im, shape, aperture, stop, nullptr, nullptr);
}

int paos_start_rows(paos_ctx* c, double re, double im, int shape, const double* aperture, const double* stop,
                    const double* write_rows) {
  return paos_start_box(c, re, im, shape, aperture, stop, write_rows, nullptr);
}

int paos_start_box(paos_ctx* c, double re, double im, int shape, const double* aperture, const double* stop,
                   const double* write_rows, const double* write_cols) {
  DROP_SCALE(c);
  return start_impl(c, re, im, shape, aperture, stop, write_rows, write_cols);
}

int paos_start_zernike_box(paos_ctx* c, double re, double im, int shape, const double* aperture, const double* stop,
                           const double* write_rows, const double* write_cols, int nmax, int kdim, const double* table,
                           const double* params, int param_stride, int* power_ticket) {
  DROP_SCALE(c);
  if (c && (!write_rows || !write_cols)) return fail(c, PAOS_EINVAL, "paos_start_zernike_box: null window");
  const StartZernike zk{nmax, kdim, param_stride, table, params, power_ticket};
  return start_impl(c, re, im, shape, aperture, stop, write_rows, write_cols, &zk);
}

int paos_zero_outside_box(paos_ctx* c, const double* live_rows, const double* live_cols) {
  SETTLE_SCALE(c);
  if (c) (void)hipSetDevice(c->device);
  if (!c || !live_rows) return fail(c, PAOS_EINVAL, "null argument");
  int rc = check_rows(c, live_rows);
  if (rc) return rc;
  if (live_cols && (rc = check_rows(c, live_cols))) return rc;
  return arena_settled(c, zero_outside_box(c, live_rows, live_cols));
}

int paos_zero_outside_rows(paos_ctx* c, const double* live_rows) { return paos_zero_outside_box(c, live_rows, nullptr); }

int paos_import(paos_ctx* c, int item, const void* host) {
  SETTLE_SCALE(c);
  if (c) (void)hipSetDevice(c->device);
  if (!c || !host || item < 0 || item >= c->batch) return fail(c, PAOS_EINVAL, "bad item or null buffer");
  const size_t bytes = (size_t)c->n * c->n * 16;
  HIPCHK(c, hipMemcpyAsync(c->staging, host, bytes, hipMemcpyHostToDevice, c->stream));
  dispatch_layout(c, [&](auto t, auto br) {
    using T = decltype(t);
    hipLaunchKernelGGL((import_kernel<T, decltype(br)::value, Lay<T>::BC>), dim3(pw_blocks(c)), dim3(kPwThreads), 0, c->stream,
                       (cx<T>*)c->field + (size_t)item * c->item_stride, (const cx<double>*)c->staging, c->n, c->pitch);
  });
  HIPCHK(c, hipGetLastError());
  HIPCHK(c, hipStreamSynchronize(c->stream));
  return PAOS_OK;
}

static int export_impl(paos_ctx* c, int item, int what, void* host_out, bool pinned) {
  if (!c || !host_out || item < 0 || item >= c->batch || what < 0 || what > 3)
    return fail(c, PAOS_EINVAL, "bad item/what or null buffer");
  dispatch_layout(c, [&](auto t, auto br) {
    using T = decltype(t);
    hipLaunchKernelGGL((export_kernel<T, decltype(br)::value, Lay<T>::BC>), dim3(pw_blocks(c)), dim3(kPwThreads), 0, c->stream,
                       (const cx<T>*)c->field + (size_t)item * c->item_stride, (double*)c->staging, c->n, c->pitch, what);
  });
  HIPCHK(c, hipGetLastError());
  const size_t bytes = (size_t)c->n * c->n * (what == PAOS_WHAT_FIELD ? 16 : 8);
  if (pinned) {
    HIPCHK(c, hipMemcpyAsync(host_out, c->staging, bytes, hipMemcpyDeviceToHost, c->stream));
    HIPCHK(c, hipStreamSynchronize(c->stream));
  } else {
    int rc = copy_to_host(c, host_out, c->staging, bytes);
    if (rc) return rc;
  }
  return check_mask_overflow(c);
}

int paos_export(paos_ctx* c, int item, int what, void* host_out) {
  SETTLE_SCALE(c);
  if (c) (void)hipSetDevice(c->device);
  return export_impl(c, item, what, host_out, false);
}

int paos_export_pinned(paos_ctx* c, int item, int what, void* pinned_out) {
  SETTLE_SCALE(c);
  if (c) (void)hipSetDevice(c->device);
  return export_impl(c, item, what, pinned_out, true);
}

int paos_psf_keep(paos_ctx* c) {
  SETTLE_SCALE(c);
  if (c) (void)hipSetDevice(c->device);
  if (!c) return fail(c, PAOS_EINVAL, "null context");
  if (!c->psf) HIPCHK(c, hipMalloc(&c->psf, (size_t)c->batch * c->item_stride * sizeof(double)));
  c->psf_zero_axis = -1;
  c->otf_valid = c->ee_valid = false;
  const dim3 grid(pw_blocks(c), c->batch), block(kPwThreads);
  dispatch_layout(c, [&](auto t, auto br) {
    using T = decltype(t);
    hipLaunchKernelGGL((intensity_kernel<T, decltype(br)::value, Lay<T>::BC>), grid, block, 0, c->stream, (const cx<T>*)c->field,
                       c->psf, c->n, c->pitch, c->item_stride);
  });
  HIPCHK(c, hipGetLastError());
  return PAOS_OK;
}

int paos_psf_fetch(paos_ctx* c, int item, double* host_out) {
  if (c) (void)hipSetDevice(c->device);
  if (!c || !host_out || item < 0 || item >= c->batch) return fail(c, PAOS_EINVAL, "bad item or null buffer");
// ... 629 lines not shown
```

paos_amd/csrc/passes.hip:

```cpp
#include "frugal_launch.h"

#include <algorithm>
#include <cmath>
#include <cstdio>
#include <cstring>

#include "pass_program.h"
#include "phase_tables.h"

namespace {

int check_ops(paos_ctx* c, const paos_pw_op* ops, int count, int n_blocks) {
  if (count < 0 || count > PAOS_MAX_PW) return fail(c, PAOS_EINVAL, "too many pointwise operators in a pass");
  for (int o = 0; o < count; ++o) {
    if (ops[o].kind < PAOS_PW_SIGN || ops[o].kind > PAOS_PW_MASK) return fail(c, PAOS_EINVAL, "unknown pointwise operator");
    if (ops[o].block < 0 || ops[o].block >= n_blocks) return fail(c, PAOS_EINVAL, "operator block index out of range");
    if (ops[o].kind == PAOS_PW_MASK && ops[o].block + 1 >= n_blocks) return fail(c, PAOS_EINVAL, "an aperture operator needs two parameter blocks");
  }
  return PAOS_OK;
}

bool use_tables() {
  static const bool on = env_is("PAOS_PHASE_TABLES", '1');
  return on;
// ... 173 lines not shown
  c->prof_next_lines = g.lines;
  const FrugalBuild& b = g.build;
  {
    int rec[kBuildFields];
    build_to_ints(b, rec);
    c->pass_builds.insert(c->pass_builds.end(), rec, rec + kBuildFields);
  }
  static const bool dump = env_is("PAOS_DUMP_PASSES", '1');
  if (dump) {
    std::fprintf(stderr, "build axis %d kpre %d kmid %d nfft %d store %d tab %d fuse %d one_line %d central %d n %d %s\n", b.axis, b.kpre, b.kmid,
                 b.nfft, b.store, b.tab, b.fuse, b.one_line, b.central, c->n, c->precision == PAOS_F64 ? "fp64" : "fp32");
    for (int k = 0; k < g.count; ++k) {
      const LoweredPass* l = g.lp[k];
      if (l->items.empty()) continue;
      const FrugalItem& f = l->items[0];
      std::fprintf(stderr, "%spass axis %d kpre %d kmid %d nfft %d | pre: sign %g scale %g mask %g | fft1 on %g inv %g | mid: sign %g scale %g mask %g | "
                   "fft2 on %g inv %g | lines [%g, %g) fill %g loads [%g, %g) stores [%g, %g)\n", k == 0 ? "" : "+", g.axis, l->kpre, l->kmid, l->nfft,
                   f.pre.sign_on, f.pre.scale, f.pre.mask_on, f.fft1_on, f.fft1_inv, f.mid.sign_on, f.mid.scale, f.mid.mask_on, f.fft2_on, f.fft2_inv,
                   f.line_lo, f.line_hi, f.line_fill, f.pos_lo, f.pos_hi, f.spos_lo, f.spos_hi);
    }
  }
  return dispatch_family(c->precision, c->n, (int)PAOS_EUNSUPPORTED,
                         [&](auto t, auto n) { return frugal_family<decltype(t), decltype(n)::value>(c, b, a, g.narrow != 0); });
}

int launch_one_pass(paos_ctx* c, const paos_pass& p, const double* dblocks, int n_blocks,
                    const int* table_of_op ) {
  int rc;
  for (int l = 0; l < 3; ++l)
    if ((rc = check_ops(c, op_list(p, l).ops, op_list(p, l).count, n_blocks))) return rc;
  if (p.fft1 >= n_blocks || p.fft2 >= n_blocks) return fail(c, PAOS_EINVAL, "transform control block out of range");
  int nmask = 0;
  for (int l = 0; l < 3; ++l) {
    const OpList ol = op_list(p, l);
    for (int o = 0; o < ol.count; ++o)
      if (ol.ops[o].kind == PAOS_PW_MASK) {
        if (++nmask > 1) return fail(c, PAOS_EINVAL, "one aperture operator per pass");
        int rcm = render_mask_weights(c, dblocks + (size_t)ol.ops[o].block * c->batch * FP_STRIDE);
        if (rcm) return rcm;
      }
  }
  PassArgs a{};
  a.field = c->field; a.tw = c->tw; a.blocks = dblocks; a.tables = c->tables; a.mask = c->mask; a.batch = c->batch;
  a.fft1 = p.fft1; a.fft2 = p.fft2; a.n_pre = p.n_pre; a.n_mid = p.n_mid; a.n_post = p.n_post;
  static_assert(sizeof(PwOp) == sizeof(paos_pw_op), "ABI op layout");
  std::memcpy(a.pre, p.pre, sizeof(a.pre));
  std::memcpy(a.mid, p.mid, sizeof(a.mid));
  std::memcpy(a.post, p.post, sizeof(a.post));
  PwOp* lists[3] = {a.pre, a.mid, a.post};
  int feat = 0;
  for (int l = 0; l < 3; ++l)
    for (int o = 0; o < PAOS_MAX_PW; ++o) {
      lists[l][o].flags &= (1 << kTableShift) - 1;
      const int t = table_of_op[l * PAOS_MAX_PW + o];
      if (t >= 0) { lists[l][o].flags |= (t + 1) << kTableShift; feat = 3; }
      if (o < op_list(p, l).count && lists[l][o].kind == PWK_MASK) feat = 3;
    }
  a.pitch = c->pitch; a.item_stride = c->item_stride;
  if (p.axis == 0 || p.axis == 1) return generic_pass(c, p.axis, a, feat);
  if (p.axis != -1) return fail(c, PAOS_EINVAL, "pass axis must be 0, 1 or -1");
  if (p.fft1 >= 0 || p.fft2 >= 0 || p.n_mid || p.n_post)
    return fail(c, PAOS_EINVAL, "a transform-free pass carries its operators in the pre list");
  return pointwise_pass(c, a);
}

struct ProgramRun {
  paos_ctx* c;
  const paos_pass* passes;
  int n_passes;
  const double* blocks;
  int n_blocks;
  PlanDims d;
  PlanSwitches sw;
  ArenaBatch ab;
  const double* dblocks = nullptr;
  std::vector<LoweredPass> low;
  bool all_frugal = false, pruned = false;
  int store = 0;
  int power_groups = 0;
  std::vector<MaskRender> renderings;
  std::vector<Launch> launches;
  std::vector<int> launch_of;
  StagedTables staged;
  ProgramRun(paos_ctx* c_, const paos_pass* passes_, int n_passes_, const double* blocks_, int n_blocks_)
      : c(c_), passes(passes_), n_passes(n_passes_), blocks(blocks_), n_blocks(n_blocks_), d(plan_dims(c_)), sw(plan_switches(c_)), ab(c_) {}
};

int validate_program(paos_ctx* c, const paos_pass* passes, int n_passes, const double* blocks, int n_blocks, const int* final_ticket) {
  if (c) c->pass_builds.clear();
  if (!c || !passes || !blocks || n_passes < 0 || n_blocks < 1) return fail(c, PAOS_EINVAL, "bad pass program");
  c->norm2_of_field = false;
  if (int rcr = final_ticket ? power_ring_full(c) : PAOS_OK) return rcr;
  switch (check_phase_args(plan_dims(c), passes, n_passes, blocks, n_blocks)) {
    case PHASE_BLOCK_OUT_OF_RANGE: return fail(c, PAOS_EINVAL, "operator block index out of range");
    case PHASE_TOO_LARGE: return fail(c, PAOS_EUNSUPPORTED, "quadratic phase exceeds 1e12 rad at the grid corner (or is not finite)");
    default: return PAOS_OK;
  }
}

int open_batch(ProgramRun& r) {
  paos_ctx* c = r.c;
  const size_t per_pass = (((size_t)c->batch * sizeof(FrugalItem) / sizeof(double) + 15) & ~size_t(15)) +
                          (((size_t)c->batch + 15) & ~size_t(15)) + 16;
  int rc = r.ab.begin((size_t)r.n_blocks * c->batch * FP_STRIDE + 16 + (size_t)r.n_passes * per_pass + 2 * arena_rounded((size_t)2 * c->batch));
  if (rc) return rc;
  return r.ab.add(r.blocks, (size_t)r.n_blocks * c->batch * FP_STRIDE, &r.dblocks);
}

int lower_and_assign_sets(ProgramRun& r) {
  paos_ctx* c = r.c;
  r.low.resize(r.n_passes);
  r.all_frugal = !use_tables() && frugal_sizes(c) && r.n_passes > 0;
  if (use_tables() || !frugal_sizes(c)) return PAOS_OK;
  int rc = ensure_mask_store(c);
  if (rc) return rc;
  for (int q = 0; q < r.n_passes; ++q) {
    LoweredPass& lp = r.low[q];
    lp.ok = lower_frugal(r.d, r.passes[q], r.blocks, lp);
    if (lp.ok && lp.mask_block >= 0 && (rc = assign_mask_set(c, r.passes[q], lp, r.blocks))) return rc;
    r.all_frugal = r.all_frugal && lp.ok;
  }
  return PAOS_OK;
}

int settle_stop(ProgramRun& r) {
  paos_ctx* c = r.c;
  if (!c->dyn_pending) return PAOS_OK;
  bool ride = r.n_passes > 0 && r.low[0].ok;
  if (ride)
    for (const FrugalItem& fi : r.low[0].items) ride = ride && fi.active != 0.0;
  if (ride) ++c->deferred_rode;
  return ride ? PAOS_OK : settle_scale(c);
}

void plan_lines(ProgramRun& r, const double* entry_rows, bool entry_stale, const double* entry_cols) {
  paos_ctx* c = r.c;
  r.pruned = r.all_frugal && r.sw.env_prune && r.sw.ctx_prune;
  if (r.pruned) plan_pruning(r.d, r.passes, r.n_passes, r.blocks, r.low, entry_rows, entry_stale, entry_cols);
  for (LoweredPass& lp : r.low) {
    if (!lp.ok || lp.mask_block < 0) continue;
    record_window(r.d, lp);
    paos_ctx::MaskSet& ms = c->mask_sets[lp.mask_set];
    if (!lp.mask_render && !(ms.line_lo <= lp.mask_lo && ms.line_hi >= lp.mask_hi)) {
      lp.mask_render = true;
      --c->mask_hits; ++c->mask_rendered;
    }
    if (lp.mask_render) { ms.line_lo = lp.mask_lo; ms.line_hi = lp.mask_hi; }
  }
}

int prepare_store(ProgramRun& r, int final_mode) {
  paos_ctx* c = r.c;
  r.store = last_pass_store(r.low, final_mode);
  if (final_mode == 2 && r.store == 2) {
    r.power_groups = c->n / frugal_tile_lines(c, r.passes[r.n_passes - 1].axis);
    if (c->pow_nparts < c->n / 2) {
      if (c->pow_partial) (void)hipFree(c->pow_partial);
      c->pow_partial = nullptr; c->pow_nparts = 0;
      HIPCHK(c, hipMalloc(&c->pow_partial, (size_t)c->batch * (c->n / 2) * sizeof(double)));
      c->pow_nparts = c->n / 2;
    }
    HIPCHK(c, hipMemsetAsync(c->pow_partial, 0, (size_t)c->batch * r.power_groups * sizeof(double), c->stream));
  }
  if (final_mode != 1) return PAOS_OK;
  if (!c->psf) HIPCHK(c, hipMalloc(&c->psf, (size_t)c->batch * c->item_stride * sizeof(double)));
  c->otf_valid = c->ee_valid = false;
  if (r.store != 1) return PAOS_OK;
  const int axis = r.passes[r.n_passes - 1].axis, groups = c->n / frugal_tile_lines(c, axis);
  if (c->psf_nparts < groups) {
    if (c->psf_partial) (void)hipFree(c->psf_partial);
    c->psf_partial = nullptr; c->psf_nparts = 0;
    c->psf_zero_axis = -1;
    HIPCHK(c, hipMalloc(&c->psf_partial, (size_t)c->batch * groups * sizeof(double)));
    c->psf_nparts = groups;
  }
  psf_zero_fill(r.d, r.sw, axis, r.low[r.n_passes - 1].items, c->psf_zero_axis, c->psf_zero_lo, c->psf_zero_hi);
  c->psf_zero_axis = -1;
  return PAOS_OK;
}

int batch_renderings(ProgramRun& r) {
  for (int q : batched_renderings(r.sw, r.all_frugal, r.low)) {
    LoweredPass& lp = r.low[q];
    const double* dshared = nullptr;
    int rc = r.ab.add(lp.mask_shared.data(), lp.mask_shared.size(), &dshared);
    if (rc) return rc;
    r.renderings.push_back(mask_job(r.c, r.passes[q].axis, lp, r.dblocks + (size_t)lp.mask_block * r.c->batch * FP_STRIDE, dshared));
    lp.mask_render = false;
// ... 2 lines not shown
}

int plan_and_stage_launches(ProgramRun& r) {
  r.launches = form_launches(r.d, r.sw, r.passes, r.n_passes, r.low, r.all_frugal && r.pruned, r.launch_of);
  for (Launch& g : r.launches) {
    if (!g.lp[0]->ok) continue;
    decide_tables(r.d, r.sw, g);
    finish_launch(r.d, r.sw, g, g.q + g.count == r.n_passes ? r.store : 0);
  }
  if (!stage_whole_program(r.d, r.sw, r.all_frugal, r.n_passes)) return PAOS_OK;
  return stage_groups(r.c, r.ab, r.launches, &r.staged);
}

int launch_chunks(ProgramRun& r) {
  paos_ctx* c = r.c;
  int rc;
  int i = 0;
  while (i < r.n_passes) {
    TableArgs ta{};
    ta.blocks = r.dblocks; ta.tables = c->tables; ta.batch = c->batch; ta.n = c->n; ta.count = 0;
    std::vector<int> assign;
    int j = i;
    for (; j < r.n_passes; ++j) {
      const paos_pass& p = r.passes[j];
      int need = 0;
      for (int l = 0; l < 3; ++l)
        for (int o = 0; o < op_list(p, l).count && o < PAOS_MAX_PW; ++o) need += is_phase(op_list(p, l).ops[o]);
      if (use_tables() && ta.count + need > kMaxTables) {
        if (j == i) return fail(c, PAOS_EINVAL, "one pass needs more phase tables than the store holds");
        break;
      }
      const size_t base = assign.size();
      assign.resize(base + 3 * PAOS_MAX_PW, -1);
      if (!use_tables()) continue;
      for (int l = 0; l < 3; ++l)
        for (int o = 0; o < op_list(p, l).count && o < PAOS_MAX_PW; ++o) {
          const paos_pw_op& op = op_list(p, l).ops[o];
          if (!is_phase(op)) continue;
          if (op.block < 0 || op.block >= r.n_blocks) return fail(c, PAOS_EINVAL, "operator block index out of range");
          ta.jobs[ta.count] = {op.block, op.kind, op.flags & PAOS_PWF_MUL2PI};
          assign[base + l * PAOS_MAX_PW + o] = ta.count++;
        }
    }
    if (ta.count > 0) {
      if (!c->tables) {
        HIPCHK(c, hipMalloc(&c->tables, (size_t)kMaxTables * c->batch * 2 * c->n * sizeof(cx<double>)));
        ta.tables = c->tables;
      }
      const dim3 grid((2 * c->n + 255) / 256, c->batch, ta.count);
      hipLaunchKernelGGL(phase_table_kernel, grid, dim3(256), 0, c->stream, ta);
      HIPCHK(c, hipGetLastError());
    }
    for (int q = i; q < j; ++q) {
      if (!r.low[q].ok) {
        if ((rc = launch_one_pass(c, r.passes[q], r.dblocks, r.n_blocks, &assign[(size_t)(q - i) * 3 * PAOS_MAX_PW]))) return rc;
        continue;
      }
      const Launch& g = r.launches[r.launch_of[q]];
      const int last = q + g.count - 1;
      if (last >= j) return fail(c, PAOS_EINVAL, "a fused group crosses a table chunk");
      if ((rc = launch_lowered(c, g, r.dblocks, r.staged.items ? r.staged.items + g.item_base : nullptr))) return rc;
      q = last;
      if (c->dyn_pending) {
        if ((rc = dyn_scale_reset(c))) return rc;
      }
    }
    i = j;
  }
  return PAOS_OK;
}

int hand_out_ticket(ProgramRun& r, int final_mode, int* final_ticket) {
  paos_ctx* c = r.c;
  if (final_mode == 2) {
    const int rcp = r.store == 2 ? take_power_ticket(c, c->pow_partial, r.power_groups, nullptr, final_ticket) : paos_norm2_enqueue(c, final_ticket);
    if (rcp == PAOS_OK) c->norm2_of_field = true;
    return rcp;
  }
  if (r.store != 1) return psf_keep_power_impl(c, final_ticket);
  c->psf_zero_axis = r.passes[r.n_passes - 1].axis;
  return take_power_ticket(c, c->psf_partial, c->n / frugal_tile_lines(c, r.passes[r.n_passes - 1].axis), nullptr, final_ticket);
}

int run_passes_impl(paos_ctx* c, const paos_pass* passes, int n_passes, const double* blocks, int n_blocks,
                    const double* entry_rows, bool entry_stale, int* final_ticket, int final_mode, const double* entry_cols) {
  int rc = validate_program(c, passes, n_passes, blocks, n_blocks, final_ticket);
  if (rc) return rc;
  final_mode = final_ticket ? (final_mode == 2 ? 2 : 1) : 0;
  ProgramRun r(c, passes, n_passes, blocks, n_blocks);
  if ((rc = open_batch(r)) || (rc = lower_and_assign_sets(r)) || (rc = settle_stop(r))) return rc;
  plan_lines(r, entry_rows, entry_stale, entry_cols);
  if (entry_stale && entry_rows && entry_zero_first(r.d, r.pruned, r.low, entry_rows, entry_cols)) {
    if ((rc = entry_cols ? zero_outside_box(c, entry_rows, entry_cols) : zero_outside_rows(c, entry_rows))) return rc;
  }
  if ((rc = prepare_store(r, final_mode)) || (rc = batch_renderings(r)) || (rc = plan_and_stage_launches(r))) return rc;
  if ((rc = r.ab.commit())) return rc;
  for (size_t at = 0; at < r.renderings.size(); at += kMaskRenders)
    if ((rc = render_mask_records(c, r.renderings.data() + at, (int)std::min<size_t>(kMaskRenders, r.renderings.size() - at)))) return rc;
  if ((rc = launch_staged_tables(c, r.staged)) || (rc = launch_chunks(r))) return rc;
  return final_mode ? hand_out_ticket(r, final_mode, final_ticket) : PAOS_OK;
}

}

int run_passes(paos_ctx* c, const paos_pass* passes, int n_passes, const double* blocks, int n_blocks, const double* entry_rows,
               bool entry_stale, int* final_ticket, int final_mode, const double* entry_cols) {
  const int rc = arena_settled(c, run_passes_impl(c, passes, n_passes, blocks, n_blocks, entry_rows, entry_stale, final_ticket, final_mode, entry_cols));
  if (rc != PAOS_OK && c) forget_mask_sets(c);
  return rc;
}

int mask_render_mode() {
  if (env_is("PAOS_MASK_SCAN", '1')) return 0;
  if (env_is("PAOS_MASK_PAIRS", '0')) return 1;
  if (env_is("PAOS_MASK_PAIRS", '1')) return 2;
  return env_is("PAOS_MASK_BLOCKS", '0') ? 3 : 4;
}
bool mask_rect_blocks() {
  return !env_is("PAOS_MASK_RECT_BLOCKS", '0');
}

namespace {

struct Program {
  std::vector<paos_pass> passes;
  std::vector<double> blocks;
  int batch;
  explicit Program(int b) : batch(b) {}
  int add_block(const double* src, double v1, double v2, double v3, double v4, bool copy) {
    const int id = (int)(blocks.size() / ((size_t)batch * FP_STRIDE));
    for (int i = 0; i < batch; ++i) {
      const double* s = src + (size_t)i * FP_STRIDE;
      if (copy) blocks.insert(blocks.end(), s, s + FP_STRIDE);
      else blocks.insert(blocks.end(), {s[FP_ENABLE], v1, v2, v3, v4});
    }
    return id;
  }
  paos_pass& add_pass(int axis, int fft1, int fft2) {
    paos_pass p{};
    p.axis = axis; p.fft1 = fft1; p.fft2 = fft2;
    passes.push_back(p);
    return passes.back();
  }
};
void push(paos_pw_op* list, int& count, int kind, int block, int flags = 0) { list[count++] = {kind, flags, block}; }

enum FftOp { OP_PTP, OP_STW, OP_WTS };

int fft_op(paos_ctx* c, FftOp op, const double* params, int inverse) {
  if (!c || !params) return fail(c, PAOS_EINVAL, "null argument");
  Program g(c->batch);
  const double inv_n = 1.0 / c->n;
  const int par = g.add_block(params, 0, 0, 0, 0, true);
  const int scl = g.add_block(params, 0, 0, inv_n, 0, false);
  if (op == OP_PTP) {
    const int fwd = g.add_block(params, 0, 0, 0, 0, false), inv = g.add_block(params, 1, 0, 0, 0, false);
    g.add_pass(0, fwd, -1);
    { paos_pass& p = g.add_pass(1, fwd, inv); push(p.mid, p.n_mid, PAOS_PW_QPHASE_NATURAL, par); push(p.mid, p.n_mid, PAOS_PW_SCALE, scl); }
    { paos_pass& p = g.add_pass(0, inv, -1); push(p.mid, p.n_mid, PAOS_PW_SCALE, scl); }
  } else {
    const int ctl = g.add_block(params, inverse ? 1.0 : 0.0, 0, 0, 0, false);
    paos_pass& r = g.add_pass(0, ctl, -1);
    push(r.pre, r.n_pre, PAOS_PW_SIGN, par);
    if (op == OP_WTS) push(r.pre, r.n_pre, PAOS_PW_QPHASE_CENTRED, par);
    paos_pass& q = g.add_pass(1, ctl, -1);
    push(q.mid, q.n_mid, PAOS_PW_SIGN, par);
    if (op == OP_STW) push(q.mid, q.n_mid, PAOS_PW_QPHASE_CENTRED, par);
    push(q.mid, q.n_mid, PAOS_PW_SCALE, scl);
  }
  return run_passes(c, g.passes.data(), (int)g.passes.size(), g.blocks.data(),
                    (int)(g.blocks.size() / ((size_t)c->batch * FP_STRIDE)));
}

}

extern "C" {

int paos_run_program(paos_ctx* c, const paos_pass* passes, int n_passes, const double* blocks, int n_blocks,
                     const paos_program_opts* opts) {
  if (c) (void)hipSetDevice(c->device);
  if (!opts) return run_passes(c, passes, n_passes, blocks, n_blocks);
  if (c && opts->live_rows) {
    int rc = check_rows(c, opts->live_rows);
    if (rc) return rc;
  }
  if (opts->final_intensity && !opts->power_ticket) return fail(c, PAOS_EINVAL, "final_intensity needs a place for the power ticket");
  if (opts->final_intensity < 0 || opts->final_intensity > 2) return fail(c, PAOS_EINVAL, "final_intensity: 0, 1 (PSF instead of the field) or 2 (field + its power)");
  const bool stale = opts->live_rows && opts->rows_stale != 0;
  if (c && opts->live_cols && stale) {
    int rc = check_rows(c, opts->live_cols);
    if (rc) return rc;
  }
  return run_passes(c, passes, n_passes, blocks, n_blocks, opts->live_rows, stale,
                    opts->final_intensity ? opts->power_ticket : nullptr, opts->final_intensity == 2 ? 2 : 1,
                    stale ? opts->live_cols : nullptr);
}

int paos_frugal_built(int precision, int n, const int* record) {
  if (!record) return -PAOS_EINVAL;
  const FrugalBuild b = build_from_ints(record);
  return dispatch_family(precision, n, -(int)PAOS_EINVAL, [&](auto t, auto size) { return frugal_built<decltype(t), decltype(size)::value>(b) ? 1 : 0; });
}

int paos_pass_builds(paos_ctx* c, int* records, int capacity, int* count) {
  if (!c || !count || capacity < 0 || (capacity > 0 && !records)) return fail(c, PAOS_EINVAL, "bad pass-builds request");
  const int have = (int)(c->pass_builds.size() / kBuildFields);
  *count = have;
  if (have > 0 && capacity > 0) std::memcpy(records, c->pass_builds.data(), (size_t)(have < capacity ? have : capacity) * kBuildFields * sizeof(int));
  return PAOS_OK;
}

int paos_phase(paos_ctx* c, const double* params, int mul2pi) {
  SETTLE_SCALE(c);
  if (c) (void)hipSetDevice(c->device);
  if (!c || !params) return fail(c, PAOS_EINVAL, "null argument");
  Program g(c->batch);
  const int par = g.add_block(params, 0, 0, 0, 0, true);
  paos_pass& p = g.add_pass(-1, -1, -1);
  push(p.pre, p.n_pre, PAOS_PW_QPHASE_CENTRED, par, mul2pi ? PAOS_PWF_MUL2PI : 0);
  return run_passes(c, g.passes.data(), 1, g.blocks.data(), 1);
}

int paos_run_passes(paos_ctx* c, const paos_pass* passes, int n_passes, const double* blocks, int n_blocks) {
  if (c) (void)hipSetDevice(c->device);
  return run_passes(c, passes, n_passes, blocks, n_blocks);
}

int paos_run_passes_live(paos_ctx* c, const paos_pass* passes, int n_passes, const double* blocks, int n_blocks,
                         const double* live_rows) {
  if (c) (void)hipSetDevice(c->device);
  if (c && live_rows)
    for (int i = 0; i < c->batch; ++i)
      if (!(live_rows[2 * i] >= 0.0) || !(live_rows[2 * i + 1] <= (double)c->n) || !(live_rows[2 * i] <= live_rows[2 * i + 1]))
        return fail(c, PAOS_EINVAL, "live row range must satisfy 0 <= lo <= hi <= n");
  return run_passes(c, passes, n_passes, blocks, n_blocks, live_rows);
}

int paos_ptp(paos_ctx* c, const double* params) {
  if (c) (void)hipSetDevice(c->device);
  return fft_op(c, OP_PTP, params, 0);
}
int paos_stw(paos_ctx* c, const double* params, int inverse) {
  if (c) (void)hipSetDevice(c->device);
  return fft_op(c, OP_STW, params, inverse);
}
int paos_wts(paos_ctx* c, const double* params, int inverse) {
  if (c) (void)hipSetDevice(c->device);
  return fft_op(c, OP_WTS, params, inverse);
}

}
```

paos_amd/passes.py:

```python
import numpy as np

from . import _lib

import os

_OFF = [0.0, 0.0, 0.0, 0.0, 0.0]
MAX_MERGED_PTP = 3
PTP_ALGEBRA = os.environ.get("PAOS_PTP_ALGEBRA", "1") != "0"
PARITY_GATE = 1.0e-10
UNDO_MAX_RESIDUAL = 1.0e-11
UNDO_COMPENSATE_MAX = 1.0e-6
FIRST_AXIS = 1 if os.environ.get("PAOS_FIRST_AXIS", "0") == "1" else 0


def _rows(rows, batch):
    if isinstance(rows, np.ndarray):
        if rows.shape != (batch, 5):
            raise ValueError(f"expected blocks of shape {(batch, 5)}, got {rows.shape}")
        return rows
    if len(rows) != batch:
        raise ValueError("one block (or None) per batch item is required")
    return np.array([r if r is not None else _OFF for r in rows], dtype=np.float64).reshape(batch, 5)


# ... 159 lines not shown
        else:
            zero = np.zeros_like(rx)
            out.append(np.stack([on.astype(float), np.sqrt(np.abs(rx)), zero, np.ones_like(rx), np.where(rx < 0.0, -1.0, 1.0)], axis=1))
            out.append(np.stack([on.astype(float), zero, np.sqrt(np.abs(ry)), np.ones_like(rx), np.where(ry < 0.0, -1.0, 1.0)], axis=1))
        return [b for b in out if np.any(b[:, 0] != 0.0) and np.any((b[:, 1] != 0.0) | (b[:, 2] != 0.0))]

    def stw(self, rows, inverse):
        self._single(rows, inverse, "stw")

    def wts(self, rows, inverse):
        self._single(rows, inverse, "wts")

    def ptp(self, rows):
        arr = _rows(rows, self.batch)
        if not arr[:, 0].any():
            return
        lp = self.last_ptp if PTP_ALGEBRA else None
        if (lp is not None and self.open is lp["tail"] and not self.tail and lp["tail"]["mid"] == lp["tail_mid"] and
                sum(op[0] == _lib.PW_QPHASE_NATURAL for op in lp["middle"]["mid"]) < MAX_MERGED_PTP):
            first = self.blocks[lp["par"]]
            on = arr[:, 0] != 0.0
            if (lp["single"] and np.array_equal(first[:, 0] != 0.0, on) and
                    np.array_equal(first[on, 1:3], arr[on, 1:3]) and np.array_equal(first[on, 3], -arr[on, 3]) and
                    np.array_equal(first[on, 4], arr[on, 4])):
                self._restore(lp["undo"])
                return
            par = self._block(arr)
            for blk, col, val in ((lp["fwd"], 1, 0.0), (lp["inv"], 1, 1.0), (lp["scl"], 3, 1.0 / self.n)):
                b = self.blocks[blk]
                new = on & (b[:, 0] == 0.0)
                b[new, :] = 0.0
                b[new, 0] = 1.0
                b[new, col] = val
            mid = lp["middle"]["mid"]
            mid.insert(len(mid) - 1, (_lib.PW_QPHASE_NATURAL, 0, par))
            lp["single"] = False
            return
        undo = self._snapshot()
        par = self._block(arr)
        fwd = self._derived(arr, v1=0.0)
        inv = self._derived(arr, v1=1.0)
        scl = self._derived(arr, v3=1.0 / self.n)
        axis = self._first_pass([], fwd)
        middle = {"axis": 1 - axis, "fft1": fwd, "fft2": inv, "pre": [], "post": [],
                  "mid": [(_lib.PW_QPHASE_NATURAL, 0, par), (_lib.PW_SCALE, 0, scl)]}
        self.passes.append(middle)
        self.open = None
        self._open_pass(axis, inv, [(_lib.PW_SCALE, 0, scl)])
        self.last_ptp = {"middle": middle, "tail": self.open, "tail_mid": list(self.open["mid"]), "fwd": fwd, "inv": inv,
                         "scl": scl, "par": par, "single": True, "undo": undo}

    def _snapshot(self):
        o = self.open
        return {"n_blocks": len(self.blocks), "n_passes": len(self.passes), "open": o, "tail": list(self.tail),
                "open_state": None if o is None else (list(o["mid"]), o.get("fft2", -1)), "last_ptp": self.last_ptp,
                "last_single": self.last_single}

    def _restore(self, snap):
        del self.blocks[snap["n_blocks"]:]
        del self.passes[snap["n_passes"]:]
        self.open, self.tail, self.last_ptp = snap["open"], list(snap["tail"]), snap["last_ptp"]
        self.last_single = snap["last_single"]
        if self.open is not None:
            self.open["mid"], self.open["fft2"] = list(snap["open_state"][0]), snap["open_state"][1]

    def open_takes_mask(self):
        o = self.open
        if o is None or self.tail:
            return False
        if any(op[0] == _lib.PW_MASK for op in o["mid"]):
            return False
        return len(o["mid"]) + 1 <= _lib.MAX_PW

    def pending(self):
        return bool(self.passes or self.tail or self.open)

    def program(self):
        self._close_open()
        passes = self.passes
        blocks = np.stack(self.blocks) if self.blocks else np.zeros((0, self.batch, 5), dtype=np.float64)
        self._reset()
        return passes, blocks

    def flush(self, dev, live_rows=None, rows_stale=False, final_intensity=False, live_cols=None):
        if not self.pending():
            return (0, None) if final_intensity else 0
        passes, blocks = self.program()
        ticket = None
        if passes:
            if rows_stale and live_cols is not None:
                ticket = dev.run_passes(passes, blocks, live_rows=live_rows, rows_stale=True, final_intensity=final_intensity,
                                        live_cols=live_cols)
            elif rows_stale or final_intensity:
                ticket = dev.run_passes(passes, blocks, live_rows=live_rows, rows_stale=rows_stale,
                                        final_intensity=final_intensity)
            elif live_rows is None:
                dev.run_passes(passes, blocks)
            else:
                dev.run_passes(passes, blocks, live_rows=live_rows)
        elif final_intensity and final_intensity != 2:
            raise RuntimeError("a program without passes cannot store the PSF")
        return (len(passes), ticket) if final_intensity else len(passes)


SEPARABLE = os.environ.get("PAOS_SEPARABLE", "1") != "0"


class SeparableCompiler(PassCompiler):

    def _reset(self):
        super()._reset()
        self.ops = []

    def aperture(self, records):
        rows = _aperture_rows(records, self.batch)
        if rows is None:
            return
        self.ops.append({"k": "mask", "first": rows[0], "second": rows[1]})

    def lens(self, rows):
        arr = _rows(rows, self.batch)
        if arr[:, 0].any():
            self.ops.append({"k": "diag", "kind": _lib.PW_QPHASE_CENTRED, "flags": _lib.PWF_MUL2PI, "arr": arr.copy()})

    def _single(self, rows, inverse, kind):
        arr = _rows(rows, self.batch)
        if not arr[:, 0].any():
            return
        inv = np.where(np.asarray(inverse, dtype=bool), 1.0, 0.0) * np.ones(self.batch)
        last = self.ops[-1] if self.ops else None
        if PTP_ALGEBRA and kind == "stw" and last is not None and last["k"] == "single" and last["kind"] == "wts":
            if self._undoes(last["arr"], last["inv"], arr, inv):
                self.ops.pop()
                return
            if self._undoes(last["arr"], last["inv"], arr, inv, max_residual=UNDO_COMPENSATE_MAX):
                leftovers = self._residual_phase(last["arr"], arr)
                self.ops.pop()
                for blk in leftovers:
                    self.ops.append({"k": "diag", "kind": _lib.PW_QPHASE_CENTRED, "flags": 0, "arr": blk})
                return
        self.ops.append({"k": "single", "kind": kind, "arr": arr.copy(), "inv": inv})

    def ptp(self, rows):
        arr = _rows(rows, self.batch)
        if not arr[:, 0].any():
            return
        on = arr[:, 0] != 0.0
        last = self.ops[-1] if self.ops else None
        if PTP_ALGEBRA and last is not None and last["k"] == "ptp" and len(last["H"]) < MAX_MERGED_PTP:
            first = last["H"][0]
            if (len(last["H"]) == 1 and np.array_equal(first[:, 0] != 0.0, on) and
                    np.array_equal(first[on, 1:3], arr[on, 1:3]) and np.array_equal(first[on, 3], -arr[on, 3]) and
                    np.array_equal(first[on, 4], arr[on, 4])):
                self.ops.pop()
                return
            last["H"].append(arr.copy())
            last["on"] = last["on"] | on
            return
        self.ops.append({"k": "ptp", "H": [arr.copy()], "on": on.copy()})

    def open_takes_mask(self):
        count = 0
        for op in reversed(self.ops):
            if op["k"] == "mask":
                return False if count == 0 else count % 2 == 1
            count += {"ptp": 2, "single": 1}.get(op["k"], 0)
        return count % 2 == 1

    def pending(self):
        return bool(self.ops)

    def _axis_block(self, arr, axis):
# ... 126 lines not shown
```

paos_amd/run.py:

```python
import atexit
import gc
import math
import threading
from collections.abc import Mapping, Sequence
from copy import deepcopy
from numbers import Real

import numpy as np

from . import _lib
from . import abcd as _abcd
from .abcd import ABCD
from .aperture import EllipticalAperture, RectangularAperture, make_aperture
from .coordinate_break import coordinate_break
from . import passes as _passes
from .passes import PassCompiler, SeparableCompiler
from . import phase_maps as _phase_maps
from .phase_maps import MAP_SERIAL as _MAP_SERIAL, PsdScreen, grid_sag_map
from .planner import (BeamBatch, gram_polynomials, jacobi_recurrence, orthonorm_matrix,
                      zernike_block)
from .zernike import zernike_tables

import os as _os

FUSE_APERTURES = {"0": False, "1": True}.get(_os.environ.get("PAOS_FUSE_APERTURES", "auto"), "auto")
POWER_ON_STORE = _os.environ.get("PAOS_POWER_ON_STORE", "1") != "0"
STOP_FROM_PROGRAM = _os.environ.get("PAOS_STOP_FROM_PROGRAM", "1") != "0"
INERT_TAIL = _os.environ.get("PAOS_INERT_TAIL", "1") != "0"
STOP_DEFERRED = _os.environ.get("PAOS_STOP_DEFERRED", "1") != "0"
START_BOX = _os.environ.get("PAOS_START_BOX", "1") != "0"
TWIN_FIELDS = _os.environ.get("PAOS_TWIN_FIELDS", "1") != "0"
FUSE_START = _os.environ.get("PAOS_FUSE_START", "1") != "0"
_MASK_RUN = 192




class _Reduction:

    __slots__ = ("dev", "slot", "raw", "released")

    def __init__(self, dev, slot):
        self.dev, self.slot, self.raw, self.released = dev, int(slot), None, False

    def values(self):
        if self.raw is None:
            if self.released:
                raise RuntimeError("this power was given back unread (PowerTicket.release)")
            self.raw = self.dev.norm2_fetch(self.slot)
        return self.raw

    def release(self):
        if self.raw is None and not self.released:
            self.dev.norm2_release(self.slot)
            self.released = True


class PowerTicket:

    __slots__ = ("_red", "_post")

    def __init__(self, reduction, post=None):
        self._red, self._post = reduction, post

    def fetch(self):
        v = self._red.values()
        return self._post(v) if self._post is not None else v

    def release(self):
        self._red.release()

    def __int__(self):
        return self._red.slot

    def __repr__(self):
        state = "fetched" if self._red.raw is not None else ("released" if self._red.released else "outstanding")
        return f"PowerTicket(slot {self._red.slot}, {state}{', derived' if self._post is not None else ''})"


class _PowerLedger:

    def __init__(self, dev):
        self.dev, self.entries, self.drained, self._final, self.offered = dev, [], 0, {}, None

    def final(self, ticket):
        return self._final.setdefault(ticket, _Reduction(self.dev, ticket))

    def record(self, ticket, pending, post=None, final=False):
        red = self.final(ticket) if final else _Reduction(self.dev, ticket)
        self.entries.append((red, pending, post))
        return red

    def offer(self, ticket, post=None):
        self.offered = (ticket, post)

    def claim(self, pending):
        (ticket, post), self.offered = self.offered, None
        self.record(ticket, pending, post)

    def decline(self):
        if self.offered is not None:
            self.dev.norm2_release(self.offered[0])
            self.offered = None

    def outstanding(self):
        return sum(1 for e in self.entries[self.drained:] if e[0].raw is None and not e[0].released)

    def drain(self):
        for red, pending, post in self.entries[self.drained:]:
            values = red.values()
            if post is not None:
                values = post(values)
            for i, rec in pending:
                rec["power"] = float(values[i])
        self.drained = len(self.entries)
# ... 472 lines not shown
            groups.setdefault(id(m), (m, [], []))
            groups[id(m)][1].append(i)
            groups[id(m)][2].append(wl)
            if len(plans) == 1:
                wfe = m.copy() if any(hit[2] is m for hit in _SAG_MAPS.values()) else m
    for m, idx, wls in groups.values():
        if len(idx) > 1 and hasattr(dev, "phase_map_items"):
            filled = _FILLED_MAPS.get(id(m))
            if filled is None or filled[0] is not m:
                if len(_FILLED_MAPS) >= 2:
                    _FILLED_MAPS.pop(next(iter(_FILLED_MAPS)))
                filled = _FILLED_MAPS[id(m)] = (m, np.ascontiguousarray(np.ma.filled(m, 0.0), dtype=np.float64), next(_MAP_SERIAL))
            dev.phase_map_items(filled[1], idx, wls, key=filled[2])
        else:
            for i, wl in zip(idx, wls):
                dev.phase_map(i, np.ma.filled(m, 0.0), wl)
    return wfe


_FILLED_MAPS = {}


def _queue_apertures(comp, plans):
    if plans.ap is not None:
        comp.aperture(plans.ap.blocks())


def _queue_steps(comp, lens, stw, ptp, wts, inv_stw, inv_wts):
    comp.lens(lens)
    comp.stw(stw, inv_stw != 0.0)
    comp.ptp(ptp)
    comp.wts(wts, inv_wts != 0.0)


def _given(**kw):
    return {k: v for k, v in kw.items() if v is not None}


def _enqueue_power(dev, rows=None, like=None, cols=None):
    if rows is None:
        return dev.norm2_enqueue()
    if cols is not None:
        return dev.norm2_enqueue(rows, same_as=like, live_cols=cols)
    return dev.norm2_enqueue(rows, **_given(same_as=like))


def _start_field(dev, fs, plans, value, lean, may_defer):
    code = plans.ap.start_shape() if plans.ap is not None else None
    if code is None:
        dev.fill(value)
        return False, None
    rows = cols = None
    if lean is not None and hasattr(dev, "zero_outside_rows"):
        trial = [[0, dev.n] for _ in plans]
        plans.ap.narrow_rows(trial, dev.n)
        if all(r[0] > 0 or r[1] < dev.n for r in trial) and all(r[0] < r[1] for r in trial):
            rows = trial
            if START_BOX:
                cols = plans.ap.live_cols(dev.n)
    blocks = plans.ap.blocks()[0].tolist()
    stops = [1.0 if p["stop"] else 0.0 for p in plans]
    seen, same_as = {}, []
    for i, (b, st) in enumerate(zip(blocks, stops)):
        key = (tuple(float(x) for x in b), st, tuple(rows[i]) if rows is not None else None,
               tuple(cols[i]) if cols is not None else None)
        same_as.append(seen.setdefault(key, i))
    copies = same_as if len(set(same_as)) < len(same_as) else None
    if may_defer and cols is not None:
        lean.deferred_start = dict(value=value, code=code, blocks=blocks, stops=stops, rows=rows, cols=cols, like=copies)
    else:
        dev.start(value, code, blocks, stops, **_given(write_rows=rows, write_cols=cols))
    _live_rows_after(plans, fs.live, dev.n)
    fs.stale, fs.stale_cols = rows is not None, cols if rows is not None else None
    return True, copies


class _WalkState:

    def __init__(self):
        self.rows, self.psf_ticket, self.same_as = None, None, None
        self.cols = None
        self.final_ticket = None
        self.deferred_start = None


class _FieldState:

    def __init__(self, n, batch):
        self.n, self.live = n, [[0, n] for _ in range(batch)]
        self.stale, self.stale_cols, self.dead, self.twins, self.power = False, None, False, None, None

    def known_rows(self):
        return [list(r) for r in self.live] if any(r[0] > 0 or r[1] < self.n for r in self.live) else None

    def stale_cols_for(self, rows):
        return self.stale_cols if (self.stale and rows is not None) else None

    def settle(self, dev):
        if self.stale:
            if self.stale_cols is not None:
                dev.zero_outside_rows(self.live, self.stale_cols)
            else:
                dev.zero_outside_rows(self.live)
            self.stale, self.stale_cols = False, None

    def flush(self, dev, comp, lean, ledger, final_intensity=False, final_power=False):
        if self.dead:
            comp.program()
            return 0
        rows = self.known_rows()
        if not comp.pending():
            return 0
        store = True if final_intensity else (2 if final_power else False)
        if store == 2 and ledger is not None:
            ledger.make_room()
        out = comp.flush(dev, live_rows=rows, rows_stale=self.stale and rows is not None, final_intensity=store,
                         live_cols=self.stale_cols_for(rows))
        done, ticket = out if store else (out, None)
        if final_intensity:
            lean.psf_ticket = lean.final_ticket = ticket
            self.dead = True
        elif final_power:
            self.power = ticket if done else None
        if done:
            self.stale, self.stale_cols = False, None
            for r in self.live:
                r[0], r[1] = 0, self.n
        return done


def _zernike_rides(d, plans, items, n, pending):
    any_stop, any_zern, _, any_ap = plans.summary()
    if not any_zern or any_stop or any_ap or pending or (len(plans) == 1 and bool(items[0]["save"])):
        return False
    for p, rows, cols in zip(plans, d["rows"], d["cols"]):
        z = p["zernike"]
        if z is None or z["pupil"] is not None or not (z["radius"] > 0 and z["dx"] > 0 and z["dy"] > 0):
            return False
        hx, hy = z["radius"] / z["dx"], z["radius"] / z["dy"]
        if not (cols[0] <= n // 2 - hx and n // 2 + hx <= cols[1] - 1 and
                rows[0] <= n // 2 - hy and n // 2 + hy <= rows[1] - 1):
            return False
    return True


def _launch_start(dev, lean, plans=None, items=None, pending=True):
    d, lean.deferred_start = lean.deferred_start, None
    power = d.get("power")
    if plans is not None and _zernike_rides(d, plans, items, dev.n, pending):
        zs, nmax, kdim, table, build = _zernike_tables(plans)
        slot = dev.start_zernike(d["value"], d["code"], d["blocks"], d["stops"], d["rows"], d["cols"], nmax, kdim, table,
                                 build([z["Z"] for z in zs]), power=power is not None)
        if power is not None:
            power.slot = int(slot)
        return True
    dev.start(d["value"], d["code"], d["blocks"], d["stops"], write_rows=d["rows"], write_cols=d["cols"])
    if power is not None:
        power.slot = int(_enqueue_power(dev, d["rows"], d["like"], d["cols"]))
    return False


def _walk(dev, states, chains, on_saved, stats=None, fresh=None, lean=None, psf_at=None, ledger=None):
    _SAG_SEEN.clear()
    keys = [list(c.keys()) for c in chains]
    if any(k != keys[0] for k in keys[1:]):
        raise ValueError("batched chains must list the same surfaces (same keys, same order)")
    st0 = states[0]
    if any((st.pupil_diameter, st.gridsize, st.zoom) != (st0.pupil_diameter, st0.gridsize, st0.zoom) for st in states):
        raise ValueError("the wavefronts of a batch share beam diameter, grid and zoom")
    beams = BeamBatch(st0.pupil_diameter, [st.wavelength for st in states], st0.gridsize, st0.zoom)
    state, n = beams.state, beams.n
    comp = (SeparableCompiler if _passes.SEPARABLE else PassCompiler)(len(states), dev.n)
    fs = _FieldState(dev.n, len(states))
    npass = fused_start = 0
    factor_cols_t, factor_cols_s = [], []
    rays = _Rays([st.field for st in states])

    order = keys[0]
    inert_from = len(order)
    while inert_from > 0 and all(_inert(c[order[inert_from - 1]]) for c in chains):
        inert_from -= 1
    for pos, key in enumerate(order):
        items = [c[key] for c in chains]
        if ledger is not None:
            ledger.decline()
        dxs, dys, wls = state[:, beams.DX].tolist(), state[:, beams.DY].tolist(), state[:, beams.WL].tolist()
        readout = []

        def wz_dtf():
            if not readout:
                readout.extend(beams.readout())
            return readout

        plans = _plan_surface(items, n, dxs, dys, wls, lambda i: wz_dtf()[0][i], rays)
        col_t, col_s = [it["ABCDt"] for it in items], [it["ABCDs"] for it in items]
        factor_cols_t.append(col_t)
        factor_cols_s.append(col_s)
        saved = any(it["save"] for it in items)
        if saved:
            plans.chief_ray = rays.chief()
            wz, dtf = wz_dtf()
            fr, props, ext = state[:, beams.FRATIO].tolist(), beams.propagators(), beams.extents()
            for i, (it, p) in enumerate(zip(items, plans)):
                if it["save"]:
                    p["scalars"] = {"wz": float(wz[i]), "distancetofocus": float(dtf[i]), "fratio": fr[i],
                                    "dx": dxs[i], "dy": dys[i], "wl": wls[i], "extent": ext[i],
                                    "propagator": props[i]}
                    p["ABCDt"] = ABCDProduct(tuple(col[i] for col in factor_cols_t))
                    p["ABCDs"] = ABCDProduct(tuple(col[i] for col in factor_cols_s))
        lens, stw, ptp, wts, inv_stw, inv_wts = beams.surface(*_gate_arrays(col_t, col_s))
        rays.advance(col_t, col_s)
        zernike_done = (lean is not None and lean.deferred_start is not None
                        and _launch_start(dev, lean, plans, items, comp.pending()))
        fused_start += zernike_done
        if fresh is not None and not saved and all(_inert(it) for it in items):
            continue
        any_stop, any_zern, any_map, any_ap = plans.summary()
        started, like = False, None
        if fresh is not None:
            value, fresh = fresh, None
            untouched = not (any_zern or any_map)
            may_defer = (FUSE_START and untouched and hasattr(dev, "start_zernike") and pos + 1 < len(order)
                         and not (psf_at is not None and key == psf_at) and all(_identity_gates(it) for it in items))
            started, copies = _start_field(dev, fs, plans, value, lean, may_defer)
            if started:
                like, fs.twins = (copies if untouched else None), (copies if TWIN_FIELDS else None)
        if not started:
            fuse_ap = FUSE_APERTURES
            own_breaker = saved or any_stop or any_zern or any_map
            if fuse_ap == "auto":
                fuse_ap = (plans.ap is not None and (not own_breaker or comp.open_takes_mask()) and
                           plans.ap.fits_line_records(dev.n, dev.precision))
            if fuse_ap:
                _queue_apertures(comp, plans)
            breaker = own_breaker or (any_ap and not fuse_ap)
            if breaker:
                only_saved = (saved and all(it["save"] for it in items) and
                              not (any_stop or any_zern or any_map or (any_ap and not fuse_ap)))
                ends_here = key == psf_at or (INERT_TAIL and pos + 1 >= inert_from and psf_at == order[-1] and
                                              all(_identity_gates(it) for it in items))
                as_psf = (lean is not None and psf_at is not None and ends_here and only_saved and comp.pending()
                          and not fs.dead)
                stop_rides = (STOP_FROM_PROGRAM and any_stop and comp.pending() and not fs.dead and
                              not (any_ap and not fuse_ap))
                npass += fs.flush(dev, comp, lean, ledger, final_intensity=as_psf,
                                  final_power=(not as_psf and comp.pending() and not fs.dead and
                                               (stop_rides or (ledger is not None and only_saved))))
            if not fuse_ap and any_ap:
                _launch_apertures(dev, plans)
                if not comp.pending():
                    _live_rows_after(plans, fs.live, dev.n)
            post = None
            if any_stop:
                fs.settle(dev)
                flags = [1.0 if p["stop"] else 0.0 for p in plans]
                if fs.power is not None:
                    dev.make_stop(flags, power_known=True, defer=STOP_DEFERRED)
                    post = lambda v, f=np.array(flags): np.where(f != 0.0, v * (1.0 / np.sqrt(v)) ** 2, v)
                else:
                    dev.make_stop(flags)
            if fs.power is not None:
                if ledger is not None:
                    ledger.offer(fs.power, post)
                else:
                    dev.norm2_release(fs.power)
                fs.power = None
            if fs.twins is not None and (comp.pending() or fuse_ap or any_ap or any_stop):
                fs.twins = None
        wfe = None if zernike_done else _launch_zernike(dev, plans, want_wfe=len(plans) == 1 and bool(items[0]["save"]),
                                                        same_as=fs.twins)
        if any_zern or any_map:
            fs.twins = None
        wfe = _launch_phase_maps(dev, plans, wfe)
        if saved:
            if lean is None:
                fs.settle(dev)
            else:
                if psf_at is not None and key == psf_at and lean.psf_ticket is None:
                    fs.settle(dev)
                lean.rows = fs.known_rows() if not comp.pending() else None
                lean.cols, lean.same_as = fs.stale_cols_for(lean.rows), like
            on_saved(key, items, plans, wfe)
            if lean is not None:
                lean.rows, lean.psf_ticket, lean.cols, lean.same_as = None, None, None, None
        _queue_steps(comp, lens, stw, ptp, wts, inv_stw, inv_wts)
        if comp.pending():
            fs.twins = None
            if lean is not None and lean.deferred_start is not None:
                _launch_start(dev, lean)
    if ledger is not None:
        ledger.decline()
    if lean is not None and lean.deferred_start is not None:
        _launch_start(dev, lean)
    if fresh is not None:
        dev.fill(fresh)
    npass += fs.flush(dev, comp, lean, ledger)
    fs.settle(dev)
    if stats is not None:
        stats["fused_passes"] = npass
        stats["fused_start"] = fused_start


_IDLE_CONTEXTS = {}
_IDLE_LOCK = threading.Lock()


def _borrow_context(n, precision, device):
    with _IDLE_LOCK:
        dev = _IDLE_CONTEXTS.pop((n, precision, device), None)
    return dev if dev is not None else _lib.DeviceFields(n, 1, precision, device)


def _return_context(dev, n, precision, device):
    with _IDLE_LOCK:
        if (n, precision, device) not in _IDLE_CONTEXTS:
            _IDLE_CONTEXTS[(n, precision, device)] = dev
            return
    dev.close()


def release_contexts():
    with _IDLE_LOCK:
        devs = list(_IDLE_CONTEXTS.values())
        _IDLE_CONTEXTS.clear()
    for dev in devs:
        dev.close()


atexit.register(release_contexts)


def run(pupil_diameter, wavelength, gridsize, zoom, field, opt_chain, precision="fp64", device=0):
    assert isinstance(opt_chain, dict), "opt_chain must be a dict"
    retval = {}
    state = _Item(pupil_diameter, wavelength, gridsize, zoom, field)
    dev = _borrow_context(int(gridsize), precision, device)

    def on_saved(key, items, plans, wfe):
        item, plan = items[0], plans[0]
        rec = {"aperture": plans.aperture(0)}
        if isinstance(wfe, np.ma.MaskedArray):
            rec["wfe"] = wfe
        elif wfe is not None:
            outside = np.isnan(wfe)
            rec["wfe"] = np.ma.MaskedArray(data=np.where(outside, 0.0, wfe), mask=outside,
                                           fill_value=0.0)
        s = plan["scalars"]
        rec.update({
            "amplitude": dev.download(0, _lib.WHAT_AMPLITUDE),
            "wz": s["wz"], "distancetofocus": s["distancetofocus"], "fratio": s["fratio"],
            "phase": dev.download(0, _lib.WHAT_PHASE),
            "dx": s["dx"], "dy": s["dy"],
            "wfo": dev.download(0, _lib.WHAT_FIELD),
            "wl": s["wl"], "extent": s["extent"], "propagator": s["propagator"],
        })
        rec["_plan"] = plan
        retval[item["num"]] = rec

    try:
        _walk(dev, [state], [opt_chain], on_saved, fresh=1.0 + 0.0j)
        dev.sync()
    except BaseException:
        dev.close()
        raise
    _return_context(dev, int(gridsize), precision, device)
    for rec in retval.values():
        plan = rec.pop("_plan")
        rec["ABCDt"] = deepcopy(plan["ABCDt"])
        rec["ABCDs"] = deepcopy(plan["ABCDs"])
    return retval


def _need_saved_last(chains, last_key, who):
    if last_key is None or not all(chain[last_key]["save"] for chain in chains):
        raise ValueError(f"{who} the last surface of the chain to be saved")


def _plan_wavefront(wavefront, chains, nb, sync):
    if wavefront is None:
# ... 335 lines not shown
```

Before: 2529 wavefronts/s.

## Hold the Zernike start and launch it fused with the next pass program

Adds a combined entry point that runs the start-of-chain aperture/Zernike setup inside the same native call as the following pass program. The Python driver holds the deferred start and releases it either into that program or standalone when a stop, aperture, map or save needs it first. It also adds a side stream with fork/join events for a front fork, which is off by default. The aim is to cut host round trips, per-launch overhead and arena uploads at the start of each chain, at the cost of more complex ordering logic and a multi-ticket power-ring check.

```diff
diff --git a/include/paos_hip.h b/include/paos_hip.h
--- a/include/paos_hip.h
+++ b/include/paos_hip.h
@@ -122,6 +122,8 @@
                     int n_blocks);
 int paos_copy_yardstick(paos_ctx* ctx, int reps, double* ms_per_launch, double* bytes_per_launch);
 int paos_record_set_stats(paos_ctx* ctx, unsigned long long* found, unsigned long long* rendered);
+int paos_record_sets_poison(paos_ctx* ctx);
+int paos_record_set_fetch(paos_ctx* ctx, int set, void* lines_out, double* vals_out, unsigned long long* bytes);
 int paos_central_half_stats(paos_ctx* ctx, unsigned long long* central, unsigned long long* plain);
 int paos_narrow_window_stats(paos_ctx* ctx, unsigned long long* narrow, unsigned long long* other);
 int paos_record_block_stats(paos_ctx* ctx, unsigned long long* out);
@@ -133,6 +135,18 @@
                          int n_blocks, const double* live_rows);
 int paos_run_program(paos_ctx* ctx, const paos_pass* passes, int n_passes, const double* blocks, int n_blocks,
                      const paos_program_opts* opts);
+typedef struct {
+  double re, im;
+  int shape;
+  const double *aperture, *stop, *write_rows, *write_cols;
+  int nmax, kdim;
+  const double *table, *params;
+  int param_stride;
+  int* power_ticket;
+} paos_start_desc;
+int paos_run_started_program(paos_ctx* ctx, const paos_start_desc* start, const paos_pass* passes, int n_passes,
+                             const double* blocks, int n_blocks, const paos_program_opts* opts);
+int paos_front_fork_stats(paos_ctx* ctx, unsigned long long* forked, unsigned long long* in_line);
 int paos_zernike(paos_ctx* ctx, int nmax, int kdim, const double* table, const double* params,
                  int param_stride, double* host_wfe);
 int paos_zernike_like(paos_ctx* ctx, int nmax, int kdim, const double* table, const double* params,
diff --git a/paos_amd/_lib.py b/paos_amd/_lib.py
--- a/paos_amd/_lib.py
+++ b/paos_amd/_lib.py
@@ -34,6 +34,15 @@
     _fields_ = [("live_rows", ctypes.POINTER(ctypes.c_double)), ("rows_stale", ctypes.c_int),
                 ("final_intensity", ctypes.c_int), ("power_ticket", ctypes.POINTER(ctypes.c_int)),
                 ("live_cols", ctypes.POINTER(ctypes.c_double))]
+
+
+class StartDesc(ctypes.Structure):
+    _fields_ = [("re", ctypes.c_double), ("im", ctypes.c_double), ("shape", ctypes.c_int),
+                ("aperture", ctypes.POINTER(ctypes.c_double)), ("stop", ctypes.POINTER(ctypes.c_double)),
+                ("write_rows", ctypes.POINTER(ctypes.c_double)), ("write_cols", ctypes.POINTER(ctypes.c_double)),
+                ("nmax", ctypes.c_int), ("kdim", ctypes.c_int),
+                ("table", ctypes.POINTER(ctypes.c_double)), ("params", ctypes.POINTER(ctypes.c_double)),
+                ("param_stride", ctypes.c_int), ("power_ticket", ctypes.POINTER(ctypes.c_int))]
 
 
 class Pass(ctypes.Structure):
@@ -136,6 +145,11 @@
     "paos_norm2_enqueue_rows_like": (ctypes.c_int, [_c_ctx, _dbl_p, _dbl_p, ctypes.POINTER(ctypes.c_int)]),
     "paos_run_program": (ctypes.c_int, [_c_ctx, ctypes.POINTER(Pass), ctypes.c_int, _dbl_p, ctypes.c_int,
                                         ctypes.POINTER(ProgramOpts)]),
+    "paos_run_started_program": (ctypes.c_int, [_c_ctx, ctypes.POINTER(StartDesc), ctypes.POINTER(Pass), ctypes.c_int, _dbl_p, ctypes.c_int,
+                                                ctypes.POINTER(ProgramOpts)]),
+    "paos_record_sets_poison": (ctypes.c_int, [_c_ctx]),
+    "paos_record_set_fetch": (ctypes.c_int, [_c_ctx, ctypes.c_int, ctypes.c_void_p, _dbl_p, ctypes.POINTER(ctypes.c_ulonglong)]),
+    "paos_front_fork_stats": (ctypes.c_int, [_c_ctx, ctypes.POINTER(ctypes.c_ulonglong), ctypes.POINTER(ctypes.c_ulonglong)]),
     "paos_detector_begin": (ctypes.c_int, [_c_ctx, _dbl_p]),
     "paos_detector_add": (ctypes.c_int, [_c_ctx, _dbl_p]),
     "paos_detector_images": (ctypes.c_int, [_c_ctx, _dbl_p, _dbl_p]),
@@ -727,6 +741,25 @@
                     "paos_central_half_stats")
         return int(central.value), int(plain.value)
 
+    def record_sets_poison(self):
+        self._check(self._lib.paos_record_sets_poison(self._ctx), "paos_record_sets_poison")
+
+    def record_set_fetch(self, k):
+        size = (ctypes.c_ulonglong * 2)()
+        self._check(self._lib.paos_record_set_fetch(self._ctx, int(k), None, None, size), "paos_record_set_fetch")
+        if not size[0]:
+            return None
+        lines, vals = np.empty(int(size[0]), dtype=np.uint8), np.empty(int(size[1]) // 8, dtype=np.float64)
+        self._check(self._lib.paos_record_set_fetch(self._ctx, int(k), lines.ctypes.data_as(ctypes.c_void_p), _dptr(vals), size),
+                    "paos_record_set_fetch")
+        return lines, vals
+
+    def front_fork_stats(self):
+        forked, in_line = ctypes.c_ulonglong(0), ctypes.c_ulonglong(0)
+        self._check(self._lib.paos_front_fork_stats(self._ctx, ctypes.byref(forked), ctypes.byref(in_line)),
+                    "paos_front_fork_stats")
+        return int(forked.value), int(in_line.value)
+
     def record_block_stats(self):
         out = (ctypes.c_ulonglong * 3)()
         self._check(self._lib.paos_record_block_stats(self._ctx, out), "paos_record_block_stats")
@@ -749,10 +782,7 @@
     def set_pruning(self, on):
         self._check(self._lib.paos_ctx_set_pruning(self._ctx, 1 if on else 0), "paos_ctx_set_pruning")
 
-    def run_passes(self, passes, blocks, live_rows=None, rows_stale=False, final_intensity=False, live_cols=None):
-        b = np.ascontiguousarray(blocks, dtype=np.float64)
-        if b.ndim != 3 or b.shape[1:] != (self.batch, PHASE_STRIDE):
-            raise ValueError("blocks must be [n_blocks][batch][5]")
+    def _pass_array(self, passes):
         arr = (Pass * len(passes))()
         for dst, src in zip(arr, passes):
             dst.axis, dst.fft1, dst.fft2 = src["axis"], src.get("fft1", -1), src.get("fft2", -1)
@@ -764,6 +794,13 @@
                 lst = getattr(dst, name)
                 for i, (kind, flags, block) in enumerate(ops):
                     lst[i].kind, lst[i].flags, lst[i].block = kind, flags, block
+        return arr
+
+    def run_passes(self, passes, blocks, live_rows=None, rows_stale=False, final_intensity=False, live_cols=None):
+        b = np.ascontiguousarray(blocks, dtype=np.float64)
+        if b.ndim != 3 or b.shape[1:] != (self.batch, PHASE_STRIDE):
+            raise ValueError("blocks must be [n_blocks][batch][5]")
+        arr = self._pass_array(passes)
         if rows_stale or final_intensity:
             lr = self._rows(live_rows) if live_rows is not None else None
             lc = self._rows(live_cols) if (live_cols is not None and rows_stale and lr is not None) else None
@@ -781,6 +818,27 @@
         self._check(self._lib.paos_run_passes(self._ctx, arr, len(passes), _dptr(b), b.shape[0]),
                     "paos_run_passes")
         return None
+
+    def run_started_program(self, start, passes, blocks, live_rows=None, rows_stale=False, final_intensity=False, live_cols=None):
+        value, shape, blocks0, stop, write_rows, write_cols, nmax, kdim, table, zblocks, power = start
+        ap, st, t, zb = self._start_arrays(blocks0, stop, table, zblocks)
+        wr, wcols = self._rows(write_rows), self._rows(write_cols)
+        v = complex(value)
+        start_ticket = ctypes.c_int(-1)
+        desc = StartDesc(v.real, v.imag, int(shape), _dptr(ap), _dptr(st) if st is not None else None, _dptr(wr), _dptr(wcols),
+                         int(nmax), int(kdim), _dptr(t), _dptr(zb), int(zb.shape[1]), ctypes.pointer(start_ticket) if power else None)
+        b = np.ascontiguousarray(blocks, dtype=np.float64)
+        if b.ndim != 3 or b.shape[1:] != (self.batch, PHASE_STRIDE):
+            raise ValueError("blocks must be [n_blocks][batch][5]")
+        arr = self._pass_array(passes)
+        lr = self._rows(live_rows) if live_rows is not None else None
+        lc = self._rows(live_cols) if (live_cols is not None and rows_stale and lr is not None) else None
+        ticket = ctypes.c_int(-1)
+        opts = ProgramOpts(_dptr(lr) if lr is not None else None, 1 if (rows_stale and lr is not None) else 0,
+                           int(final_intensity), ctypes.pointer(ticket), _dptr(lc) if lc is not None else None)
+        self._check(self._lib.paos_run_started_program(self._ctx, ctypes.byref(desc), arr, len(passes), _dptr(b), b.shape[0],
+                                                       ctypes.byref(opts)), "paos_run_started_program")
+        return (start_ticket.value if power else None), (ticket.value if final_intensity else None)
 
     def zernike(self, nmax, kdim, table, blocks, want_wfe=False, pupil=False, same_as=None):
         t = np.ascontiguousarray(table, dtype=np.float64).reshape(-1)
@@ -822,7 +880,7 @@
         self._check(self._lib.paos_start(self._ctx, v.real, v.imag, int(shape), _dptr(b),
                                          _dptr(st) if st is not None else None), "paos_start")
 
-    def start_zernike(self, value, shape, blocks, stop, write_rows, write_cols, nmax, kdim, table, zblocks, power=False):
+    def _start_arrays(self, blocks, stop, table, zblocks):
         b = np.ascontiguousarray(blocks, dtype=np.float64)
         if b.shape != (self.batch, APERTURE_STRIDE):
             raise ValueError("aperture blocks must be [batch][8]")
@@ -833,6 +891,10 @@
         zb = np.ascontiguousarray(zblocks, dtype=np.float64)
         if zb.ndim != 2 or zb.shape[0] != self.batch:
             raise ValueError("zernike blocks must be [batch][stride]")
+        return b, st, t, zb
+
+    def start_zernike(self, value, shape, blocks, stop, write_rows, write_cols, nmax, kdim, table, zblocks, power=False):
+        b, st, t, zb = self._start_arrays(blocks, stop, table, zblocks)
         v = complex(value)
         ticket = ctypes.c_int(-1)
         self._check(self._lib.paos_start_zernike_box(self._ctx, v.real, v.imag, int(shape), _dptr(b),
diff --git a/paos_amd/csrc/arena_layout.h b/paos_amd/csrc/arena_layout.h
--- a/paos_amd/csrc/arena_layout.h
+++ b/paos_amd/csrc/arena_layout.h
@@ -6,6 +6,17 @@
 constexpr size_t kArenaAlign = 16;
 inline size_t arena_rounded(size_t count) { return (count + kArenaAlign - 1) & ~(kArenaAlign - 1); }
 constexpr size_t kArenaSlack = 64;
+
+inline size_t arena_blocks_total(const size_t* counts, size_t n) {
+  size_t total = 0;
+  for (size_t k = 0; k < n; ++k) total += arena_rounded(counts[k]);
+  return total;
+}
+inline size_t arena_program_total(size_t n_blocks, size_t n_passes, size_t batch, size_t block_stride, size_t item_doubles,
+                                  size_t start_total = 0) {
+  const size_t per_pass = arena_rounded(batch * item_doubles) + arena_rounded(batch) + kArenaAlign;
+  return n_blocks * batch * block_stride + kArenaAlign + n_passes * per_pass + 2 * arena_rounded(2 * batch) + start_total;
+}
 
 enum ArenaRoom {
   ARENA_FITS,
diff --git a/paos_amd/csrc/context.hip b/paos_amd/csrc/context.hip
--- a/paos_amd/csrc/context.hip
+++ b/paos_amd/csrc/context.hip
@@ -304,6 +304,11 @@
   if (env_is("PAOS_CENTRAL_HALF", '1')) c->central_half = true;
   if (env_is("PAOS_NARROW_WINDOWS", '0')) c->narrow_windows = false;
   if (env_is("PAOS_NARROW_WINDOWS", '1')) c->narrow_windows = true;
+  if (env_is("PAOS_FRONT_FORK", '0')) c->front_fork = false;
+  if (env_is("PAOS_FRONT_FORK", '1')) c->front_fork = true;
+  if ((e = hipStreamCreateWithFlags(&c->side, hipStreamNonBlocking)) != hipSuccess) return bail(e, "hipStreamCreate(side)");
+  if ((e = hipEventCreateWithFlags(&c->fork_ev, hipEventDisableTiming)) != hipSuccess) return bail(e, "hipEventCreate(fork)");
+  if ((e = hipEventCreateWithFlags(&c->join_ev, hipEventDisableTiming)) != hipSuccess) return bail(e, "hipEventCreate(join)");
   if ((e = hipMalloc(&c->dyn_scale, (size_t)batch * sizeof(double))) != hipSuccess) return bail(e, "hipMalloc(dyn_scale)");
   {
     std::vector<double> ones((size_t)batch, 1.0);
@@ -400,6 +405,10 @@
   if (!c) return PAOS_OK;
   (void)hipSetDevice(c->device);
   if (c->stream) (void)hipStreamSynchronize(c->stream);
+  if (c->side) (void)hipStreamSynchronize(c->side);
+  if (c->fork_ev) (void)hipEventDestroy(c->fork_ev);
+  if (c->join_ev) (void)hipEventDestroy(c->join_ev);
+  if (c->side) (void)hipStreamDestroy(c->side);
   for (hipEvent_t e : c->prof_events) (void)hipEventDestroy(e);
   if (c->field) (void)hipFree(c->field);
   if (c->tw) (void)hipFree(c->tw);
@@ -515,6 +524,13 @@
   return PAOS_OK;
 }
 
+int paos_front_fork_stats(paos_ctx* c, unsigned long long* forked, unsigned long long* in_line) {
+  if (!c || !forked || !in_line) return fail(c, PAOS_EINVAL, "bad front-fork request");
+  *forked = c->front_forked;
+  *in_line = c->front_inline;
+  return PAOS_OK;
+}
+
 int paos_record_block_stats(paos_ctx* c, unsigned long long* out) {
   if (!c || !out) return fail(c, PAOS_EINVAL, "bad record-block request");
   out[0] = out[1] = out[2] = 0ull;
diff --git a/paos_amd/csrc/host.h b/paos_amd/csrc/host.h
--- a/paos_amd/csrc/host.h
+++ b/paos_amd/csrc/host.h
@@ -10,6 +10,7 @@
 
 #include "arena_layout.h"
 #include "frugal_pass.h"
+#include "item_groups.h"
 #include "pass_records.h"
 
 using namespace paos;
@@ -27,6 +28,9 @@
 template <typename T, int N>
 constexpr int block_rows() { return (sizeof(T) == 4 && N >= 2048) ? PAOS_F32_BR : PAOS_BR; }
 inline constexpr int kNormSlots = PAOS_NORM_SLOTS;
+#ifndef PAOS_FRONT_FORK_DEFAULT
+#define PAOS_FRONT_FORK_DEFAULT false
+#endif
 template <typename T>
 struct Lay {
   static constexpr int BC = 2;
@@ -49,6 +53,10 @@
   int br = PAOS_BR;
   unsigned pitch = 0, item_stride = 0;
   hipStream_t stream = nullptr;
+  hipStream_t side = nullptr;
+  hipEvent_t fork_ev = nullptr, join_ev = nullptr;
+  bool front_fork = PAOS_FRONT_FORK_DEFAULT;
+  unsigned long long front_forked = 0, front_inline = 0;
   double* psf = nullptr;
   void* focus_spec = nullptr;
   bool focus_open = false;
@@ -261,9 +269,10 @@
   return f(std::integral_constant<int, B>{});
 }
 
+struct StartDesc;
 int run_passes(paos_ctx* c, const paos_pass* passes, int n_passes, const double* blocks, int n_blocks,
                const double* entry_rows = nullptr, bool entry_stale = false, int* final_ticket = nullptr, int final_mode = 1,
-               const double* entry_cols = nullptr);
+               const double* entry_cols = nullptr, const StartDesc* start = nullptr);
 int mask_render_mode();
 bool mask_rect_blocks();
 
@@ -271,12 +280,35 @@
 
 template <typename T, int N>
 int frugal_family(paos_ctx* c, const FrugalBuild& b, const FrugalArgs& a, bool narrow);
+
+struct StartDesc {
+  double re = 0.0, im = 0.0;
+  int shape = 0;
+  const double *aperture = nullptr, *stop = nullptr, *write_rows = nullptr, *write_cols = nullptr;
+  bool zernike = false;
+  int nmax = 0, kdim = 0, param_stride = 0;
+  const double *table = nullptr, *params = nullptr;
+  int* power_ticket = nullptr;
+};
+struct StartPlan {
+  StartDesc d;
+  std::vector<double> flags, power_of, compute, wc, lead, same, subs;
+  ItemGroups groups;
+  bool any_stop = false, want_power = false;
+  size_t zt_count = 0, zp_count = 0, total = 0;
+  const double *dp = nullptr, *ds = nullptr, *dcompute = nullptr, *dpower_of = nullptr, *drows = nullptr, *dcols = nullptr, *dzt = nullptr,
+               *dzp = nullptr, *dsubs = nullptr, *dlead = nullptr, *dsame = nullptr, *dgoff = nullptr, *dglen = nullptr, *dmembers = nullptr;
+};
+int start_plan(paos_ctx* c, const StartDesc& d, StartPlan& p);
+int start_add(paos_ctx* c, StartPlan& p, ArenaBatch& ab);
+int start_launch(paos_ctx* c, StartPlan& p);
+void start_forget(paos_ctx* c);
 
 int settle_scale(paos_ctx* c, bool field_is_overwritten = false);
 int dyn_scale_reset(paos_ctx* c);
 int zero_outside_rows(paos_ctx* c, const double* live_rows);
 int zero_outside_box(paos_ctx* c, const double* live_rows, const double* live_cols);
-int power_ring_full(paos_ctx* c);
+int power_ring_full(paos_ctx* c, int tickets = 1);
 int take_power_ticket(paos_ctx* c, const double* partial, int nparts, const double* source, int* ticket);
 int psf_keep_power_impl(paos_ctx* c, int* ticket);
 struct MaskRender {
diff --git a/paos_amd/csrc/paos_hip.hip b/paos_amd/csrc/paos_hip.hip
--- a/paos_amd/csrc/paos_hip.hip
+++ b/paos_amd/csrc/paos_hip.hip
@@ -137,8 +137,10 @@
 
 }
 
-int power_ring_full(paos_ctx* c) {
-  if (c->norm_busy[next_norm_slot(c)])
+int power_ring_full(paos_ctx* c, int tickets) {
+  int free_slots = 0;
+  for (int k = 0; k < kNormSlots; ++k) free_slots += c->norm_busy[k] ? 0 : 1;
+  if (free_slots < tickets)
     return fail(c, PAOS_EINVAL, "64 power reductions outstanding: fetch earlier tickets (paos_norm2_fetch) first");
   return PAOS_OK;
 }
@@ -171,11 +173,6 @@
   return PAOS_OK;
 }
 
-struct StartZernike {
-  int nmax, kdim, param_stride;
-  const double *table, *params;
-  int* power_ticket;
-};
 static int zernike_check(paos_ctx* c, int nmax, int kdim, const double* table, const double* params, int param_stride);
 
 static bool start_memo_on() {
@@ -185,37 +182,40 @@
 static bool same_key(const std::vector<double>& a, const std::vector<double>& b) {
   return a.size() == b.size() && !std::memcmp(a.data(), b.data(), a.size() * sizeof(double));
 }
-static void start_forget(paos_ctx* c) {
+
+}
+
+void start_forget(paos_ctx* c) {
   c->start_key.clear();
   c->start_partial_key.clear();
 }
 
-static int start_body(paos_ctx* c, double re, double im, int shape, const double* aperture, const double* stop,
-                      const double* write_rows, const double* write_cols, const StartZernike* zk) {
-  if (c) (void)hipSetDevice(c->device);
-  if (!c || !aperture) return fail(c, PAOS_EINVAL, "null argument");
-  if (shape != PAOS_SHAPE_ELLIPSE && shape != PAOS_SHAPE_RECT) return fail(c, PAOS_EINVAL, "unknown aperture shape");
+int start_plan(paos_ctx* c, const StartDesc& d, StartPlan& p) {
+  if (c) (void)hipSetDevice(c->device);
+  if (!c || !d.aperture) return fail(c, PAOS_EINVAL, "null argument");
+  if (d.shape != PAOS_SHAPE_ELLIPSE && d.shape != PAOS_SHAPE_RECT) return fail(c, PAOS_EINVAL, "unknown aperture shape");
   int rc;
-  if (zk) {
-    if ((rc = zernike_check(c, zk->nmax, zk->kdim, zk->table, zk->params, zk->param_stride))) return rc;
-    if (zk->power_ticket && (rc = power_ring_full(c))) return rc;
-  }
+  if (d.zernike) {
+    if ((rc = zernike_check(c, d.nmax, d.kdim, d.table, d.params, d.param_stride))) return rc;
+    if (d.power_ticket && (rc = power_ring_full(c))) return rc;
+  }
+  p.d = d;
   const int batch = c->batch;
-  std::vector<double> flags(batch, 0.0);
-  bool any_stop = false;
-  if (stop)
-    for (int i = 0; i < batch; ++i) { flags[i] = stop[i] != 0.0 ? 1.0 : 0.0; any_stop |= flags[i] != 0.0; }
-  std::vector<double> power_of, compute;
-  power_representatives(batch, aperture, AP_STRIDE, flags.data(), power_of, compute);
+  const double *aperture = d.aperture, *write_rows = d.write_rows, *write_cols = d.write_cols;
+  p.flags.assign(batch, 0.0);
+  p.any_stop = false;
+  if (d.stop)
+    for (int i = 0; i < batch; ++i) { p.flags[i] = d.stop[i] != 0.0 ? 1.0 : 0.0; p.any_stop |= p.flags[i] != 0.0; }
+  power_representatives(batch, aperture, AP_STRIDE, p.flags.data(), p.power_of, p.compute);
   if (write_rows && (rc = check_rows(c, write_rows))) return rc;
-  std::vector<double> wc;
   if (write_cols) {
     if (!write_rows) return fail(c, PAOS_EINVAL, "a column window needs a row window");
     if ((rc = check_rows(c, write_cols))) return rc;
-    wc = rounded_cols(c, write_cols);
+    p.wc = rounded_cols(c, write_cols);
   }
   static const bool share_start = !env_is("PAOS_SHARE_START", '0');
-  ItemGroups groups = group_items(
+  const std::vector<double>& flags = p.flags;
+  p.groups = group_items(
       batch,
       [&](int j, int i) {
         return share_start && flags[j] == flags[i] && same_record(aperture + (size_t)j * AP_STRIDE, aperture + (size_t)i * AP_STRIDE, AP_STRIDE) &&
@@ -223,65 +223,71 @@
                (!write_cols || same_record(write_cols + 2 * j, write_cols + 2 * i, 2));
       },
       [](int) { return true; });
-  std::vector<double> lead, same, subs;
-  const bool want_power = zk && zk->power_ticket;
-  if (zk) {
-    group_leaders(groups, lead, same);
-    subs = split_by_map(groups, zk->params, zk->param_stride, ZP_ENABLE, ZP_INV_WL, share_wfe_maps());
-  }
-  const size_t zt_count = zk ? (size_t)(zk->nmax + 1) * zk->kdim * 3 : 0, zp_count = zk ? (size_t)batch * zk->param_stride : 0;
-  size_t total = arena_rounded((size_t)batch * AP_STRIDE) + 3 * arena_rounded(batch) + arena_rounded(groups.goff.size()) +
-                 arena_rounded(groups.glen.size()) + arena_rounded(groups.members.size());
-  if (write_rows) total += arena_rounded((size_t)2 * batch);
-  if (write_cols) total += arena_rounded(wc.size());
-  if (zk) total += arena_rounded(zt_count) + arena_rounded(zp_count) + arena_rounded(subs.size());
-  if (want_power) total += 2 * arena_rounded(batch);
-  ArenaBatch ab(c);
-  if ((rc = ab.begin(total))) return rc;
-  const double *dp = nullptr, *ds = nullptr, *dcompute = nullptr, *dpower_of = nullptr, *drows = nullptr, *dcols = nullptr;
-  if ((rc = ab.add(aperture, (size_t)batch * AP_STRIDE, &dp))) return rc;
-  if ((rc = ab.add(flags.data(), flags.size(), &ds))) return rc;
-  if ((rc = ab.add(compute.data(), compute.size(), &dcompute))) return rc;
-  if ((rc = ab.add(power_of.data(), power_of.size(), &dpower_of))) return rc;
-  if (write_rows && (rc = ab.add(write_rows, (size_t)2 * batch, &drows))) return rc;
-  if (write_cols && (rc = ab.add(wc.data(), wc.size(), &dcols))) return rc;
-  const double *dzt = nullptr, *dzp = nullptr, *dsubs = nullptr, *dlead = nullptr, *dsame = nullptr;
-  if (zk) {
-    if ((rc = ab.add(zk->table, zt_count, &dzt))) return rc;
-    if ((rc = ab.add(zk->params, zp_count, &dzp))) return rc;
-    if ((rc = ab.add(subs.data(), subs.size(), &dsubs))) return rc;
-    if (want_power) {
-      if ((rc = ab.add(lead.data(), lead.size(), &dlead))) return rc;
-      if ((rc = ab.add(same.data(), same.size(), &dsame))) return rc;
+  p.want_power = d.zernike && d.power_ticket;
+  if (d.zernike) {
+    group_leaders(p.groups, p.lead, p.same);
+    p.subs = split_by_map(p.groups, d.params, d.param_stride, ZP_ENABLE, ZP_INV_WL, share_wfe_maps());
+  }
+  p.zt_count = d.zernike ? (size_t)(d.nmax + 1) * d.kdim * 3 : 0;
+  p.zp_count = d.zernike ? (size_t)batch * d.param_stride : 0;
+  const size_t counts[] = {(size_t)batch * AP_STRIDE, (size_t)batch, (size_t)batch, (size_t)batch, p.groups.goff.size(), p.groups.glen.size(),
+                           p.groups.members.size(), write_rows ? (size_t)2 * batch : 0, p.wc.size(), p.zt_count, p.zp_count, p.subs.size(),
+                           p.want_power ? (size_t)batch : 0, p.want_power ? (size_t)batch : 0};
+  p.total = arena_blocks_total(counts, sizeof(counts) / sizeof(counts[0]));
+  return PAOS_OK;
+}
+
+int start_add(paos_ctx* c, StartPlan& p, ArenaBatch& ab) {
+  const StartDesc& d = p.d;
+  const int batch = c->batch;
+  int rc;
+  if ((rc = ab.add(d.aperture, (size_t)batch * AP_STRIDE, &p.dp))) return rc;
+  if ((rc = ab.add(p.flags.data(), p.flags.size(), &p.ds))) return rc;
+  if ((rc = ab.add(p.compute.data(), p.compute.size(), &p.dcompute))) return rc;
+  if ((rc = ab.add(p.power_of.data(), p.power_of.size(), &p.dpower_of))) return rc;
+  if (d.write_rows && (rc = ab.add(d.write_rows, (size_t)2 * batch, &p.drows))) return rc;
+  if (d.write_cols && (rc = ab.add(p.wc.data(), p.wc.size(), &p.dcols))) return rc;
+  if (d.zernike) {
+    if ((rc = ab.add(d.table, p.zt_count, &p.dzt))) return rc;
+    if ((rc = ab.add(d.params, p.zp_count, &p.dzp))) return rc;
+    if ((rc = ab.add(p.subs.data(), p.subs.size(), &p.dsubs))) return rc;
+    if (p.want_power) {
+      if ((rc = ab.add(p.lead.data(), p.lead.size(), &p.dlead))) return rc;
+      if ((rc = ab.add(p.same.data(), p.same.size(), &p.dsame))) return rc;
     }
   }
-  const double *dgoff = nullptr, *dglen = nullptr, *dmembers = nullptr;
-  if ((rc = ab.add(groups.goff.data(), groups.goff.size(), &dgoff))) return rc;
-  if ((rc = ab.add(groups.glen.data(), groups.glen.size(), &dglen))) return rc;
-  if ((rc = ab.add(groups.members.data(), groups.members.size(), &dmembers))) return rc;
-  if ((rc = ab.commit())) return rc;
+  if ((rc = ab.add(p.groups.goff.data(), p.groups.goff.size(), &p.dgoff))) return rc;
+  if ((rc = ab.add(p.groups.glen.data(), p.groups.glen.size(), &p.dglen))) return rc;
+  return ab.add(p.groups.members.data(), p.groups.members.size(), &p.dmembers);
+}
+
+int start_launch(paos_ctx* c, StartPlan& p) {
+  const StartDesc& d = p.d;
+  const int batch = c->batch, shape = d.shape;
+  const double re = d.re, im = d.im;
+  const bool any_stop = p.any_stop, want_power = p.want_power;
   const bool memo = start_memo_on();
   std::vector<double> key, pkey;
   if (memo && (any_stop || want_power)) {
     key.reserve(3 + (size_t)batch * (AP_STRIDE + 1));
     key.push_back((double)shape); key.push_back(re); key.push_back(im);
-    key.insert(key.end(), aperture, aperture + (size_t)batch * AP_STRIDE);
-    key.insert(key.end(), flags.begin(), flags.end());
+    key.insert(key.end(), d.aperture, d.aperture + (size_t)batch * AP_STRIDE);
+    key.insert(key.end(), p.flags.begin(), p.flags.end());
   }
   bool power_found = false;
   if (any_stop) {
     power_found = memo && c->start_norm2 && same_key(key, c->start_key);
-    if (power_found) HIPCHK(c, hipMemcpyAsync(c->norm2, c->start_norm2, (size_t)batch * sizeof(double), hipMemcpyDeviceToDevice, c->stream));
-    else c->start_key.clear();
-  }
+    if (!power_found) c->start_key.clear();
+  }
+  const double* stop_sums = power_found ? c->start_norm2 : c->norm2;
   bool partial_found = false;
   double* partial = c->partial;
   if (want_power && memo) {
     pkey = key;
-    pkey.insert(pkey.end(), write_rows, write_rows + (size_t)2 * batch);
-    pkey.insert(pkey.end(), wc.begin(), wc.end());
-    pkey.insert(pkey.end(), lead.begin(), lead.end());
-    pkey.insert(pkey.end(), same.begin(), same.end());
+    pkey.insert(pkey.end(), d.write_rows, d.write_rows + (size_t)2 * batch);
+    pkey.insert(pkey.end(), p.wc.begin(), p.wc.end());
+    pkey.insert(pkey.end(), p.lead.begin(), p.lead.end());
+    pkey.insert(pkey.end(), p.same.begin(), p.same.end());
     partial_found = c->start_partial && same_key(pkey, c->start_partial_key);
     if (!partial_found) c->start_partial_key.clear();
     if (!c->start_partial) HIPCHK(c, hipMalloc(&c->start_partial, (size_t)batch * c->nparts * sizeof(double)));
@@ -294,23 +300,23 @@
     dispatch_either<0, 1>(shape == PAOS_SHAPE_ELLIPSE, [&](auto s) {
       constexpr int S = decltype(s)::value;
       if (any_stop && !power_found) {
-        hipLaunchKernelGGL((start_power_kernel<T, BRV, BC, S>), parts, block, 0, c->stream, dp, c->n, c->pitch, c->item_stride, re, im,
-                           c->partial, dcompute);
-        hipLaunchKernelGGL(norm2_final_kernel, dim3(batch), block, 0, c->stream, c->partial, c->norm2, c->nparts, ds, 1, dpower_of);
+        hipLaunchKernelGGL((start_power_kernel<T, BRV, BC, S>), parts, block, 0, c->stream, p.dp, c->n, c->pitch, c->item_stride, re, im,
+                           c->partial, p.dcompute);
+        hipLaunchKernelGGL(norm2_final_kernel, dim3(batch), block, 0, c->stream, c->partial, c->norm2, c->nparts, p.ds, 1, p.dpower_of);
       }
-      if (!zk) {
-        hipLaunchKernelGGL((start_write_kernel<T, BRV, BC, S>), sweep, block, 0, c->stream, (cx<T>*)c->field, dp, c->n, c->pitch,
-                           c->item_stride, re, im, (const double*)c->norm2, ds, drows, dgoff, dglen, dmembers, dcols);
+      if (!d.zernike) {
+        hipLaunchKernelGGL((start_write_kernel<T, BRV, BC, S>), sweep, block, 0, c->stream, (cx<T>*)c->field, p.dp, c->n, c->pitch,
+                           c->item_stride, re, im, stop_sums, p.ds, p.drows, p.dgoff, p.dglen, p.dmembers, p.dcols);
         return;
       }
-      dispatch_either<8, 0>(zk->nmax <= 8, [&](auto nc) {
+      dispatch_either<8, 0>(d.nmax <= 8, [&](auto nc) {
         hipLaunchKernelGGL((zernike_start_write_kernel<T, BRV, BC, S, decltype(nc)::value>), sweep, block, 0, c->stream, (cx<T>*)c->field,
-                           dp, c->n, c->pitch, c->item_stride, re, im, (const double*)c->norm2, ds, drows, dcols, dgoff, dglen, dsubs,
-                           dmembers, dzt, dzp, zk->param_stride, zk->nmax, zk->kdim);
+                           p.dp, c->n, c->pitch, c->item_stride, re, im, stop_sums, p.ds, p.drows, p.dcols, p.dgoff, p.dglen, p.dsubs,
+                           p.dmembers, p.dzt, p.dzp, d.param_stride, d.nmax, d.kdim);
       });
       if (want_power && !partial_found)
-        hipLaunchKernelGGL((start_norm2_partial_kernel<T, BRV, BC, S>), parts, block, 0, c->stream, partial, dp, c->n, c->pitch,
-                           c->item_stride, re, im, (const double*)c->norm2, ds, dlead, drows, dcols);
+        hipLaunchKernelGGL((start_norm2_partial_kernel<T, BRV, BC, S>), parts, block, 0, c->stream, partial, p.dp, c->n, c->pitch,
+                           c->item_stride, re, im, stop_sums, p.ds, p.dlead, p.drows, p.dcols);
     });
   });
   HIPCHK(c, hipGetLastError());
@@ -320,13 +326,26 @@
     c->start_key = std::move(key);
   }
   if (want_power && !partial_found && memo) c->start_partial_key = std::move(pkey);
-  if (want_power) return take_power_ticket(c, partial, c->nparts, dsame, zk->power_ticket);
-  return PAOS_OK;
+  if (want_power) return take_power_ticket(c, partial, c->nparts, p.dsame, d.power_ticket);
+  return PAOS_OK;
+}
+
+extern "C" {
+
+static int start_body(paos_ctx* c, const StartDesc& d) {
+  StartPlan p;
+  int rc = start_plan(c, d, p);
+  if (rc) return rc;
+  ArenaBatch ab(c);
+  if ((rc = ab.begin(p.total)) || (rc = start_add(c, p, ab)) || (rc = ab.commit())) return rc;
+  return start_launch(c, p);
 }
 
 static int start_impl(paos_ctx* c, double re, double im, int shape, const double* aperture, const double* stop,
-                      const double* write_rows, const double* write_cols = nullptr, const StartZernike* zk = nullptr) {
-  const int rc = arena_settled(c, start_body(c, re, im, shape, aperture, stop, write_rows, write_cols, zk));
+                      const double* write_rows, const double* write_cols = nullptr, const StartDesc* zk = nullptr) {
+  StartDesc d = zk ? *zk : StartDesc{};
+  d.re = re; d.im = im; d.shape = shape; d.aperture = aperture; d.stop = stop; d.write_rows = write_rows; d.write_cols = write_cols;
+  const int rc = arena_settled(c, start_body(c, d));
   if (rc != PAOS_OK && c) start_forget(c);
   return rc;
 }
@@ -351,7 +370,9 @@
                            const double* params, int param_stride, int* power_ticket) {
   DROP_SCALE(c);
   if (c && (!write_rows || !write_cols)) return fail(c, PAOS_EINVAL, "paos_start_zernike_box: null window");
-  const StartZernike zk{nmax, kdim, param_stride, table, params, power_ticket};
+  StartDesc zk{};
+  zk.zernike = true; zk.nmax = nmax; zk.kdim = kdim; zk.param_stride = param_stride; zk.table = table; zk.params = params;
+  zk.power_ticket = power_ticket;
   return start_impl(c, re, im, shape, aperture, stop, write_rows, write_cols, &zk);
 }
 
diff --git a/paos_amd/csrc/passes.hip b/paos_amd/csrc/passes.hip
--- a/paos_amd/csrc/passes.hip
+++ b/paos_amd/csrc/passes.hip
@@ -279,15 +279,16 @@
   std::vector<Launch> launches;
   std::vector<int> launch_of;
   StagedTables staged;
+  StartPlan* start = nullptr;
   ProgramRun(paos_ctx* c_, const paos_pass* passes_, int n_passes_, const double* blocks_, int n_blocks_)
       : c(c_), passes(passes_), n_passes(n_passes_), blocks(blocks_), n_blocks(n_blocks_), d(plan_dims(c_)), sw(plan_switches(c_)), ab(c_) {}
 };
 
-int validate_program(paos_ctx* c, const paos_pass* passes, int n_passes, const double* blocks, int n_blocks, const int* final_ticket) {
+int validate_program(paos_ctx* c, const paos_pass* passes, int n_passes, const double* blocks, int n_blocks, int tickets) {
   if (c) c->pass_builds.clear();
   if (!c || !passes || !blocks || n_passes < 0 || n_blocks < 1) return fail(c, PAOS_EINVAL, "bad pass program");
   c->norm2_of_field = false;
-  if (int rcr = final_ticket ? power_ring_full(c) : PAOS_OK) return rcr;
+  if (int rcr = tickets ? power_ring_full(c, tickets) : PAOS_OK) return rcr;
   switch (check_phase_args(plan_dims(c), passes, n_passes, blocks, n_blocks)) {
     case PHASE_BLOCK_OUT_OF_RANGE: return fail(c, PAOS_EINVAL, "operator block index out of range");
     case PHASE_TOO_LARGE: return fail(c, PAOS_EUNSUPPORTED, "quadratic phase exceeds 1e12 rad at the grid corner (or is not finite)");
@@ -297,10 +298,10 @@
 
 int open_batch(ProgramRun& r) {
   paos_ctx* c = r.c;
-  const size_t per_pass = (((size_t)c->batch * sizeof(FrugalItem) / sizeof(double) + 15) & ~size_t(15)) +
-                          (((size_t)c->batch + 15) & ~size_t(15)) + 16;
-  int rc = r.ab.begin((size_t)r.n_blocks * c->batch * FP_STRIDE + 16 + (size_t)r.n_passes * per_pass + 2 * arena_rounded((size_t)2 * c->batch));
+  int rc = r.ab.begin(arena_program_total((size_t)r.n_blocks, (size_t)r.n_passes, (size_t)c->batch, FP_STRIDE, sizeof(FrugalItem) / sizeof(double),
+                                          r.start ? r.start->total : 0));
   if (rc) return rc;
+  if (r.start && (rc = start_add(c, *r.start, r.ab))) return rc;
   return r.ab.add(r.blocks, (size_t)r.n_blocks * c->batch * FP_STRIDE, &r.dblocks);
 }
 
@@ -469,31 +470,90 @@
   return take_power_ticket(c, c->psf_partial, c->n / frugal_tile_lines(c, r.passes[r.n_passes - 1].axis), nullptr, final_ticket);
 }
 
+int launch_records_and_tables(ProgramRun& r) {
+  paos_ctx* c = r.c;
+  int rc;
+  for (size_t at = 0; at < r.renderings.size(); at += kMaskRenders)
+    if ((rc = render_mask_records(c, r.renderings.data() + at, (int)std::min<size_t>(kMaskRenders, r.renderings.size() - at)))) return rc;
+  return launch_staged_tables(c, r.staged);
+}
+
+struct SideLaunches {
+  paos_ctx* c;
+  hipStream_t main;
+  explicit SideLaunches(paos_ctx* c_) : c(c_), main(c_->stream) { c->stream = c->side; }
+  ~SideLaunches() { c->stream = main; }
+  SideLaunches(const SideLaunches&) = delete;
+  SideLaunches& operator=(const SideLaunches&) = delete;
+};
+
+int run_front(ProgramRun& r, const double* zero_rows, const double* zero_cols) {
+  paos_ctx* c = r.c;
+  auto on_main = [&]() {
+    int rc = start_launch(c, *r.start);
+    if (rc == PAOS_OK && zero_rows) rc = zero_cols ? zero_outside_box(c, zero_rows, zero_cols) : zero_outside_rows(c, zero_rows);
+    return rc;
+  };
+  const bool side_work = !r.renderings.empty() || r.staged.count > 0;
+  if (!c->front_fork || !r.staged.items || !r.sw.batched_records || !side_work) {
+    ++c->front_inline;
+    const int rc = on_main();
+    return rc ? rc : launch_records_and_tables(r);
+  }
+  ++c->front_forked;
+  HIPCHK(c, hipEventRecord(c->fork_ev, c->stream));
+  HIPCHK(c, hipStreamWaitEvent(c->side, c->fork_ev, 0));
+  const int rc_main = on_main();
+  int rc_side;
+  {
+    SideLaunches on(c);
+    rc_side = launch_records_and_tables(r);
+  }
+  const hipError_t ej = hipEventRecord(c->join_ev, c->side);
+  const hipError_t ew = ej == hipSuccess ? hipStreamWaitEvent(c->stream, c->join_ev, 0) : ej;
+  if (ew != hipSuccess) (void)hipStreamSynchronize(c->side);
+  if (rc_main || rc_side) return rc_main ? rc_main : rc_side;
+  HIPCHK(c, ew);
+  return PAOS_OK;
+}
+
 int run_passes_impl(paos_ctx* c, const paos_pass* passes, int n_passes, const double* blocks, int n_blocks,
-                    const double* entry_rows, bool entry_stale, int* final_ticket, int final_mode, const double* entry_cols) {
-  int rc = validate_program(c, passes, n_passes, blocks, n_blocks, final_ticket);
+                    const double* entry_rows, bool entry_stale, int* final_ticket, int final_mode, const double* entry_cols,
+                    const StartDesc* start) {
+  int rc = validate_program(c, passes, n_passes, blocks, n_blocks, (final_ticket ? 1 : 0) + (start && start->power_ticket ? 1 : 0));
   if (rc) return rc;
   final_mode = final_ticket ? (final_mode == 2 ? 2 : 1) : 0;
+  StartPlan sp;
+  if (start) {
+    if ((rc = start_plan(c, *start, sp))) return rc;
+    DROP_SCALE(c);
+  }
   ProgramRun r(c, passes, n_passes, blocks, n_blocks);
+  r.start = start ? &sp : nullptr;
   if ((rc = open_batch(r)) || (rc = lower_and_assign_sets(r)) || (rc = settle_stop(r))) return rc;
   plan_lines(r, entry_rows, entry_stale, entry_cols);
+  bool zero_behind_start = false;
   if (entry_stale && entry_rows && entry_zero_first(r.d, r.pruned, r.low, entry_rows, entry_cols)) {
-    if ((rc = entry_cols ? zero_outside_box(c, entry_rows, entry_cols) : zero_outside_rows(c, entry_rows))) return rc;
+    if (start) zero_behind_start = true;
+    else if ((rc = entry_cols ? zero_outside_box(c, entry_rows, entry_cols) : zero_outside_rows(c, entry_rows))) return rc;
   }
   if ((rc = prepare_store(r, final_mode)) || (rc = batch_renderings(r)) || (rc = plan_and_stage_launches(r))) return rc;
   if ((rc = r.ab.commit())) return rc;
-  for (size_t at = 0; at < r.renderings.size(); at += kMaskRenders)
-    if ((rc = render_mask_records(c, r.renderings.data() + at, (int)std::min<size_t>(kMaskRenders, r.renderings.size() - at)))) return rc;
-  if ((rc = launch_staged_tables(c, r.staged)) || (rc = launch_chunks(r))) return rc;
+  if ((rc = start ? run_front(r, zero_behind_start ? entry_rows : nullptr, entry_cols) : launch_records_and_tables(r))) return rc;
+  if ((rc = launch_chunks(r))) return rc;
   return final_mode ? hand_out_ticket(r, final_mode, final_ticket) : PAOS_OK;
 }
 
 }
 
 int run_passes(paos_ctx* c, const paos_pass* passes, int n_passes, const double* blocks, int n_blocks, const double* entry_rows,
-               bool entry_stale, int* final_ticket, int final_mode, const double* entry_cols) {
-  const int rc = arena_settled(c, run_passes_impl(c, passes, n_passes, blocks, n_blocks, entry_rows, entry_stale, final_ticket, final_mode, entry_cols));
-  if (rc != PAOS_OK && c) forget_mask_sets(c);
+               bool entry_stale, int* final_ticket, int final_mode, const double* entry_cols, const StartDesc* start) {
+  const int rc = arena_settled(c, run_passes_impl(c, passes, n_passes, blocks, n_blocks, entry_rows, entry_stale, final_ticket, final_mode,
+                                                  entry_cols, start));
+  if (rc != PAOS_OK && c) {
+    forget_mask_sets(c);
+    if (start) start_forget(c);
+  }
   return rc;
 }
 
@@ -563,10 +623,10 @@
 
 extern "C" {
 
-int paos_run_program(paos_ctx* c, const paos_pass* passes, int n_passes, const double* blocks, int n_blocks,
-                     const paos_program_opts* opts) {
-  if (c) (void)hipSetDevice(c->device);
-  if (!opts) return run_passes(c, passes, n_passes, blocks, n_blocks);
+static int run_program(paos_ctx* c, const StartDesc* start, const paos_pass* passes, int n_passes, const double* blocks, int n_blocks,
+                       const paos_program_opts* opts) {
+  if (c) (void)hipSetDevice(c->device);
+  if (!opts) return run_passes(c, passes, n_passes, blocks, n_blocks, nullptr, false, nullptr, 1, nullptr, start);
   if (c && opts->live_rows) {
     int rc = check_rows(c, opts->live_rows);
     if (rc) return rc;
@@ -580,7 +640,54 @@
   }
   return run_passes(c, passes, n_passes, blocks, n_blocks, opts->live_rows, stale,
                     opts->final_intensity ? opts->power_ticket : nullptr, opts->final_intensity == 2 ? 2 : 1,
-                    stale ? opts->live_cols : nullptr);
+                    stale ? opts->live_cols : nullptr, start);
+}
+
+int paos_run_program(paos_ctx* c, const paos_pass* passes, int n_passes, const double* blocks, int n_blocks,
+                     const paos_program_opts* opts) {
+  return run_program(c, nullptr, passes, n_passes, blocks, n_blocks, opts);
+}
+
+int paos_run_started_program(paos_ctx* c, const paos_start_desc* st, const paos_pass* passes, int n_passes, const double* blocks,
+                             int n_blocks, const paos_program_opts* opts) {
+  if (!st) return fail(c, PAOS_EINVAL, "paos_run_started_program: null start");
+  if (c && (!st->write_rows || !st->write_cols)) return fail(c, PAOS_EINVAL, "paos_run_started_program: null window");
+  StartDesc d;
+  d.re = st->re; d.im = st->im; d.shape = st->shape; d.aperture = st->aperture; d.stop = st->stop;
+  d.write_rows = st->write_rows; d.write_cols = st->write_cols;
+  d.zernike = true; d.nmax = st->nmax; d.kdim = st->kdim; d.param_stride = st->param_stride; d.table = st->table; d.params = st->params;
+  d.power_ticket = st->power_ticket;
+  return run_program(c, &d, passes, n_passes, blocks, n_blocks, opts);
+}
+
+int paos_record_sets_poison(paos_ctx* c) {
+  if (c) (void)hipSetDevice(c->device);
+  if (!c) return fail(c, PAOS_EINVAL, "null context");
+  const size_t lines = (size_t)c->batch * c->n * sizeof(MaskLine), vals = (size_t)c->batch * c->n * 2 * kMaskW * sizeof(double);
+  for (paos_ctx::MaskSet& ms : c->mask_sets) {
+    if (!ms.lines) {
+      HIPCHK(c, hipMalloc(&ms.lines, lines));
+      HIPCHK(c, hipMalloc(&ms.vals, vals));
+    }
+    ms.key.clear();
+    ms.line_lo = ms.line_hi = 0;
+    HIPCHK(c, hipMemsetAsync(ms.lines, 0xff, lines, c->stream));
+    HIPCHK(c, hipMemsetAsync(ms.vals, 0xff, vals, c->stream));
+  }
+  return PAOS_OK;
+}
+
+int paos_record_set_fetch(paos_ctx* c, int set, void* lines_out, double* vals_out, unsigned long long* bytes) {
+  if (c) (void)hipSetDevice(c->device);
+  if (!c || !bytes || set < 0 || set >= paos_ctx::kMaskSets) return fail(c, PAOS_EINVAL, "bad record-set request");
+  const paos_ctx::MaskSet& ms = c->mask_sets[set];
+  bytes[0] = ms.lines ? (unsigned long long)c->batch * c->n * sizeof(MaskLine) : 0ull;
+  bytes[1] = ms.lines ? (unsigned long long)c->batch * c->n * 2 * kMaskW * sizeof(double) : 0ull;
+  if (!ms.lines || (!lines_out && !vals_out)) return PAOS_OK;
+  HIPCHK(c, hipStreamSynchronize(c->stream));
+  if (lines_out) HIPCHK(c, hipMemcpy(lines_out, ms.lines, (size_t)bytes[0], hipMemcpyDeviceToHost));
+  if (vals_out) HIPCHK(c, hipMemcpy(vals_out, ms.vals, (size_t)bytes[1], hipMemcpyDeviceToHost));
+  return PAOS_OK;
 }
 
 int paos_frugal_built(int precision, int n, const int* record) {
diff --git a/paos_amd/passes.py b/paos_amd/passes.py
--- a/paos_amd/passes.py
+++ b/paos_amd/passes.py
@@ -265,12 +265,19 @@
         self._reset()
         return passes, blocks
 
-    def flush(self, dev, live_rows=None, rows_stale=False, final_intensity=False, live_cols=None):
+    def flush(self, dev, live_rows=None, rows_stale=False, final_intensity=False, live_cols=None, start=None):
         if not self.pending():
             return (0, None) if final_intensity else 0
         passes, blocks = self.program()
         ticket = None
-        if passes:
+        if start is not None and not passes:
+            start.launch(dev)
+            start = None
+        if start is not None:
+            slot, ticket = dev.run_started_program(start.args, passes, blocks, live_rows=live_rows, rows_stale=rows_stale,
+                                                   final_intensity=final_intensity, live_cols=live_cols)
+            start.launched(slot)
+        elif passes:
             if rows_stale and live_cols is not None:
                 ticket = dev.run_passes(passes, blocks, live_rows=live_rows, rows_stale=True, final_intensity=final_intensity,
                                         live_cols=live_cols)
diff --git a/paos_amd/run.py b/paos_amd/run.py
--- a/paos_amd/run.py
+++ b/paos_amd/run.py
@@ -31,6 +31,7 @@
 START_BOX = _os.environ.get("PAOS_START_BOX", "1") != "0"
 TWIN_FIELDS = _os.environ.get("PAOS_TWIN_FIELDS", "1") != "0"
 FUSE_START = _os.environ.get("PAOS_FUSE_START", "1") != "0"
+HOLD_START = _os.environ.get("PAOS_HOLD_START", "1") != "0"
 _MASK_RUN = 192
 
 
@@ -669,6 +670,7 @@
         self.cols = None
         self.final_ticket = None
         self.deferred_start = None
+        self.held_start = None
 
 
 class _FieldState:
@@ -701,8 +703,11 @@
         store = True if final_intensity else (2 if final_power else False)
         if store == 2 and ledger is not None:
             ledger.make_room()
+        held = None
+        if lean is not None and lean.held_start is not None:
+            held, lean.held_start = lean.held_start, None
         out = comp.flush(dev, live_rows=rows, rows_stale=self.stale and rows is not None, final_intensity=store,
-                         live_cols=self.stale_cols_for(rows))
+                         live_cols=self.stale_cols_for(rows), **_given(start=held))
         done, ticket = out if store else (out, None)
         if final_intensity:
             lean.psf_ticket = lean.final_ticket = ticket
@@ -731,15 +736,36 @@
     return True
 
 
-def _launch_start(dev, lean, plans=None, items=None, pending=True):
+class _HeldStart:
+
+    def __init__(self, args, power):
+        self.args, self.power = args, power
+
+    def launched(self, slot):
+        if self.power is not None:
+            self.power.slot = int(slot)
+
+    def launch(self, dev):
+        self.launched(dev.start_zernike(*self.args[:-1], power=self.args[-1]))
+
+
+def _release_start(dev, lean):
+    if lean is not None and lean.held_start is not None:
+        held, lean.held_start = lean.held_start, None
+        held.launch(dev)
+
+
+def _launch_start(dev, lean, plans=None, items=None, pending=True, hold=False):
     d, lean.deferred_start = lean.deferred_start, None
     power = d.get("power")
     if plans is not None and _zernike_rides(d, plans, items, dev.n, pending):
         zs, nmax, kdim, table, build = _zernike_tables(plans)
-        slot = dev.start_zernike(d["value"], d["code"], d["blocks"], d["stops"], d["rows"], d["cols"], nmax, kdim, table,
-                                 build([z["Z"] for z in zs]), power=power is not None)
-        if power is not None:
-            power.slot = int(slot)
+        held = _HeldStart((d["value"], d["code"], d["blocks"], d["stops"], d["rows"], d["cols"], nmax, kdim, table,
+                           build([z["Z"] for z in zs]), power is not None), power)
+        if hold and hasattr(dev, "run_started_program"):
+            lean.held_start = held
+        else:
+            held.launch(dev)
         return True
     dev.start(d["value"], d["code"], d["blocks"], d["stops"], write_rows=d["rows"], write_cols=d["cols"])
     if power is not None:
@@ -798,7 +824,8 @@
         lens, stw, ptp, wts, inv_stw, inv_wts = beams.surface(*_gate_arrays(col_t, col_s))
         rays.advance(col_t, col_s)
         zernike_done = (lean is not None and lean.deferred_start is not None
-                        and _launch_start(dev, lean, plans, items, comp.pending()))
+                        and _launch_start(dev, lean, plans, items, comp.pending(),
+                                          hold=HOLD_START and not saved and not plans.summary()[2]))
         fused_start += zernike_done
         if fresh is not None and not saved and all(_inert(it) for it in items):
             continue
@@ -833,6 +860,8 @@
                 npass += fs.flush(dev, comp, lean, ledger, final_intensity=as_psf,
                                   final_power=(not as_psf and comp.pending() and not fs.dead and
                                                (stop_rides or (ledger is not None and only_saved))))
+            if (any_ap and not fuse_ap) or any_stop:
+                _release_start(dev, lean)
             if not fuse_ap and any_ap:
                 _launch_apertures(dev, plans)
                 if not comp.pending():
@@ -854,6 +883,8 @@
                 fs.power = None
             if fs.twins is not None and (comp.pending() or fuse_ap or any_ap or any_stop):
                 fs.twins = None
+        if (any_zern and not zernike_done) or any_map or saved:
+            _release_start(dev, lean)
         wfe = None if zernike_done else _launch_zernike(dev, plans, want_wfe=len(plans) == 1 and bool(items[0]["save"]),
                                                         same_as=fs.twins)
         if any_zern or any_map:
@@ -882,6 +913,7 @@
     if fresh is not None:
         dev.fill(fresh)
     npass += fs.flush(dev, comp, lean, ledger)
+    _release_start(dev, lean)
     fs.settle(dev)
     if stats is not None:
         stats["fused_passes"] = npass
```

New measurement: 2532 wavefronts/s (median of 4 runs). No clear change (+0.1%).
